# ahsouri/OI-SAT-GMI

Hardware: AMD Instinct MI355X
Metric: analysed grid-cells/s (dense Gaussian-B OI: B build + Kalman-gain solve + increment) and Kalman-gain solve TFLOP/s vs MI355X fp32 MFMA roofline (higher is better)
Workload: dtype f32; 1 GPU; config3_720x1440_1e5obs; species=NO2, obs_per_month=99898, refine=2, parallelism=one month per GPU; RCCL broadcast of the grid, gather of the fields to rank 0

## Files before the change

### include/oisat.h

```cpp
#ifndef OISAT_H
#define OISAT_H

#include <stddef.h>
#include <stdint.h>

#ifdef __cplusplus
extern "C" {
#endif

#define OISAT_F32 0
#define OISAT_F64 1

#define OISAT_OK 0
#define OISAT_EINVAL (-1)
#define OISAT_EHIP (-2)
#define OISAT_ENOMEM (-3)
#define OISAT_ENOTPD (-4)
#define OISAT_ENODEV (-5)

#define OISAT_MAX_SCALES 128

typedef struct oisat_ctx oisat_ctx;

int oisat_init(int device_id, oisat_ctx** out);
void oisat_shutdown(oisat_ctx* h);
const char* oisat_last_error(void);
const char* oisat_version(void);
int oisat_device_info(oisat_ctx* h, char* name_out, int name_cap, int* cu_count, int64_t* hbm_bytes);

int oisat_set_stream(oisat_ctx* h, void* hip_stream);
int oisat_stream_create(oisat_ctx* h);
int oisat_stream_create_masked(oisat_ctx* h, int reserve_per_xcd);
int oisat_bind_thread(oisat_ctx* h);
int oisat_wait_for(oisat_ctx* waiter, oisat_ctx* signaler);
int oisat_sync(oisat_ctx* h);
int oisat_query(oisat_ctx* h, int* busy);
int oisat_dmalloc(oisat_ctx* h, size_t bytes, void** dev_out);
int oisat_dfree(oisat_ctx* h, void* dev);
int oisat_h2d(oisat_ctx* h, void* dev_dst, const void* host_src, size_t bytes);
int oisat_d2h(oisat_ctx* h, void* host_dst, const void* dev_src, size_t bytes);
int oisat_memset(oisat_ctx* h, void* dev, int byte_value, size_t bytes);

int oisat_prof_enable(oisat_ctx* h, int on);
int oisat_prof_reset(oisat_ctx* h);
int oisat_prof_collect(oisat_ctx* h, int cap, char (*names)[64], double* total_ms, int64_t* launches);

int oisat_oi_curve(oisat_ctx* h, int dtype, const void* Sa, const void* So, int64_t n,
                   const double* scales, int nscales, double* mean_out, int64_t* count_out);

int oisat_oi_apply(oisat_ctx* h, int dtype, const void* Xa, void* Y_inout, const void* Sa,
                   const void* So, int64_t n, double scale, void* Xb, void* AK, void* inc, void* err);

int oisat_oi_fused(oisat_ctx* h, int dtype, const void* Xa, void* Y_inout, const void* Sa,
                   const void* So, int64_t n, const double* scales, int nscales, int forced_index,
                   void* Xb, void* AK, void* inc, void* err, int32_t* index_dev, double* curve_dev);

int oisat_nanmean_stack(oisat_ctx* h, int dtype, const void* stack, int k, int64_t n, int inf_to_nan, void* out);

int oisat_error_average(oisat_ctx* h, int dtype, const void* stack, int k, int64_t n, int square_input, void* out);

int oisat_month_accumulate(oisat_ctx* h, int acc_dtype, const void* vcd, const void* uncertainty, const void* ctm_vcd,
                           const void* new_amf, const void* old_amf, int f32_mask, int64_t n, const int32_t* kept, void* acc);
int oisat_month_finish(oisat_ctx* h, int acc_dtype, const void* acc, int64_t n, void* out);
int oisat_all_nan(oisat_ctx* h, int dtype, const void* x, int64_t n, int32_t* kept);
int oisat_widen(oisat_ctx* h, const float* x, int64_t n, double* out);

int oisat_affine(oisat_ctx* h, int dtype, const void* x, int64_t n, double offset, double slope, void* out);

int oisat_oi_variances(oisat_ctx* h, int dtype, const void* Xa, const void* sat_err, int64_t n,
                       double error_ctm, void* Sa_out, void* So_out);

int oisat_scaling_factor(oisat_ctx* h, int dtype, const void* posterior, const void* prior, int64_t n, void* out);

int oisat_partial_column(oisat_ctx* h, int dtype, const void* deltap, const void* profile, int64_t n, void* out);

int oisat_amf_recal(oisat_ctx* h, const double* sat_pmid, const double* sat_sw, int nzs, int ctm_dtype,
                    const void* ctm_pmid, const void* ctm_partial, int nzc, const double* tropopause, const double* vcd,
                    const double* amf, int64_t n, double* new_amf, double* vcd_out, double* ctm_vcd);

int oisat_column_sum(oisat_ctx* h, int dtype, const void* ctm_pmid, const void* ctm_partial, int nzc,
                     const double* tropopause, const double* vcd, int64_t n, void* ctm_vcd);

int oisat_ak_conv_mopitt(oisat_ctx* h, int ctm_dtype, const void* ctm_pmid, const void* ctm_profile,
                         const void* ctm_air_partial, int nzc, const double* sat_pmid,
                         const double* averaging_kernels, const double* apriori_profile, int nzs,
                         const double* aprior_column, const double* apriori_surface, const double* vcd,
                         int64_t n, double* model_vcd, double* model_xcol);
int oisat_ak_conv_gosat(oisat_ctx* h, int ctm_dtype, const void* ctm_pmid, const void* ctm_profile, int nzc,
                        const double* sat_pmid, const double* averaging_kernels,
                        const double* apriori_profile, const double* pressure_weight, int nzs,
                        const double* x_col, int64_t n, double* model_xcol);

int oisat_water_column(oisat_ctx* h, int dtype, const void* deltap, const void* profile, int64_t n, void* out);
int oisat_pwv_sum(oisat_ctx* h, int dtype, const void* partial, int nz, const double* vcd, int64_t n, void* out);

int oisat_boxfilter_symm(oisat_ctx* h, int dtype, const void* Z, int64_t Ny, int64_t Nx, int ky, int kx,
                         int variance, void* out);

int oisat_nn_query(oisat_ctx* h, const double* plon, const double* plat, int64_t P,
                   const double* tlon, const double* tlat, int64_t T, double max_dist,
                   int32_t* idx_out, double* dist_out );

int oisat_nn_query_ties(oisat_ctx* h, const double* plon, const double* plat, int64_t P,
                        const double* tlon, const double* tlat, int64_t T, double max_dist,
                        int32_t* idx_out, double* dist_out ,
                        int32_t* tie_list, int64_t* n_ties);

int oisat_gather_mask(oisat_ctx* h, int dtype, const void* values, int64_t P, int nfields,
                      const int32_t* idx, int64_t T, void* out);

int oisat_linear_interp(oisat_ctx* h, int dtype, const double* tlon, const double* tlat, int64_t T,
                        const int32_t* nn_idx, const int32_t* vertex_to_simplex, const int32_t* simplices,
                        const int32_t* neighbors, const double* transform, int64_t nsimplex,
                        const void* values, int64_t P, int nfields, void* out, const double* bounds_host);

int oisat_tri_transform(oisat_ctx* h, const double* points, int64_t P, const int32_t* simplices, int64_t nsimplex,
                        double* transform_out, int32_t* suspects, int64_t* n_suspect);

int oisat_linear_locate(oisat_ctx* h, const double* tlon, const double* tlat, int64_t T, const int32_t* nn_idx,
                        const int32_t* vertex_to_simplex, const int32_t* simplices, const int32_t* neighbors,
                        const double* transform, int64_t nsimplex, int64_t P, const double* bounds_host,
                        int32_t* amb_list, int64_t* n_amb);

int oisat_linear_interp_forced(oisat_ctx* h, int dtype, const double* tlon, const double* tlat, int64_t T,
                               const int32_t* nn_idx, const int32_t* vertex_to_simplex, const int32_t* simplices,
                               const int32_t* neighbors, const double* transform, int64_t nsimplex,
                               const void* values, int64_t P, int nfields, void* out, const double* bounds_host,
                               const int32_t* forced);

int oisat_rbf_interp(oisat_ctx* h, int dtype, const double* plon, const double* plat, int64_t P,
                     const double* tlon, const double* tlat, int64_t T, const int32_t* nn_idx, double cell,
                     int neighbors, const void* values, int nfields, void* out, int64_t* n_singular);

int oisat_rbf_interp_ties(oisat_ctx* h, int dtype, const double* plon, const double* plat, int64_t P,
                          const double* tlon, const double* tlat, int64_t T, const int32_t* nn_idx, double cell,
                          int neighbors, const void* values, int nfields, void* out, int64_t* n_singular,
                          int32_t* tie_list, int64_t* n_ties);

int oisat_rbf_interp_forced(oisat_ctx* h, int dtype, const double* plon, const double* plat, int64_t P,
                            const double* tlon, const double* tlat, int64_t T, const int32_t* targets,
                            const int32_t* ids, int64_t n, int neighbors, const void* values, int nfields, void* out,
                            int64_t* n_singular);

int oisat_rbf_check_masked(oisat_ctx* h, const double* plon, const double* plat, int64_t P, const double* tlon,
                           const double* tlat, int64_t T, const int32_t* nn_idx, double cell, int neighbors,
                           int64_t* n_singular);

int oisat_boxfilter_pick(oisat_ctx* h, int dtype, const void* Z, int64_t Ny, int64_t Nx, int nfields,
                         int ky, int kx, int variance, const int32_t* idx, int64_t T, void* out);

int oisat_flag_mask(oisat_ctx* h, int dtype, const void* x, const void* flag, int64_t n, double thresh,
                    int square, void* out);

int oisat_sqrt(oisat_ctx* h, int dtype, const void* x, int64_t n, void* out);


int oisat_cov_build(oisat_ctx* h, const double* oxyz, const double* osig, const double* ovar, int64_t m,
                    double g, float* S, int64_t ld);

int oisat_innovation(oisat_ctx* h, int dtype, const void* xb, const int64_t* cell, const double* y,
                     int64_t m, double* d_out);

int oisat_gemm_nt(oisat_ctx* h, float* C, int64_t ldc, const float* A, int64_t lda, const float* B, int64_t ldb,
                  int64_t M, int64_t N, int64_t K, int mode, int lower);

int oisat_potrf(oisat_ctx* h, float* S, int64_t m, int64_t ld, int* info_host);

int oisat_envelope(const double* lat_sorted, int64_t m, double g, int32_t* env_out);
int oisat_factor_envelope(const double* lat_sorted, int64_t m, double g, int32_t* env_out);
int oisat_factor_far(const double* lat_sorted, int64_t m, double g, const int32_t* first, int32_t* far_out);
int oisat_factor_mid(const double* lat_sorted, int64_t m, double g, const int32_t* first, const int32_t* far, int32_t* mid_out);

#define OISAT_CORR_GAUSSIAN 0
#define OISAT_CORR_GASPARI_COHN 1
int oisat_set_correlation(oisat_ctx* h, int kind);
int oisat_corr_eval(int kind, double g, const double* d2, int64_t n, double* out);
int oisat_corr_cut_chord(int kind, double g, double bits, double* chord_out);
int oisat_envelope_corr(int kind, const double* lat_sorted, int64_t m, double g, int32_t* env_out);
int oisat_factor_envelope_corr(int kind, const double* lat_sorted, int64_t m, double g, int32_t* env_out);
int oisat_factor_far_corr(int kind, const double* lat_sorted, int64_t m, double g, const int32_t* first, int32_t* far_out);
int oisat_set_factor_far(oisat_ctx* h, const int32_t* far, int64_t nb);
int oisat_factor_mid_corr(int kind, const double* lat_sorted, int64_t m, double g, const int32_t* first, const int32_t* far,
                          int32_t* mid_out);
int oisat_set_factor_mid(oisat_ctx* h, const int32_t* mid, int64_t nb);
int oisat_cov_build_env(oisat_ctx* h, const double* oxyz, const double* osig, const double* ovar, int64_t m,
                        double g, float* S, int64_t ld, const int32_t* env_dev);
int oisat_potrf_env(oisat_ctx* h, float* S, int64_t m, int64_t ld, const int32_t* first, const int32_t* env_dev,
                    int* info_host);

#define OISAT_SCHEDULE_OTHER 0
#define OISAT_SCHEDULE_ENV_DAG 1
#define OISAT_SCHEDULE_ENV_DAG_FWD 2
int oisat_cov_build_env_zeroed(oisat_ctx* h, const double* oxyz, const double* osig, const double* ovar, int64_t m,
                               double g, float* S, int64_t ld, const int32_t* first, const int32_t* env_dev,
                               const int32_t* zero_first, const int32_t* zero_first_dev, int* enveloped_out);
int oisat_cov_build_cover(const int32_t* first, const int32_t* zero_first, int64_t nb, int32_t* from_out,
                          int64_t* width_out, int64_t* zero_tiles_out);
int oisat_potrf_env_fwd(oisat_ctx* h, float* S, int64_t m, int64_t ld, const int32_t* first, const int32_t* env_dev,
                        const double* d, int* info_host, int* schedule_out);

int oisat_trsv_plan(int64_t nb, int band, int cu_count, int32_t* two_tiles_out, int32_t* grid_out);

int oisat_potrs(oisat_ctx* h, const float* L, int64_t m, int64_t ld, double* z_inout);

int oisat_cov_residual(oisat_ctx* h, const double* oxyz, const double* osig, const double* ovar, int64_t m,
                       double g, const double* d, const double* z, double* r_out, const double* olat_sorted);

int oisat_gain_solve(oisat_ctx* h, const float* L, const double* oxyz, const double* osig, const double* ovar,
                     int64_t m, int64_t ld, double g, const double* d, int refine, double* z_out,
                     double* resid_host, const double* olat_sorted );

int oisat_apply_increment(oisat_ctx* h, int dtype, const double* gxyz, const double* gsig, int64_t n,
                          const double* oxyz, const double* osig, const double* z, int64_t m, double g,
                          const void* xb, void* xa, void* inc, const double* glat, const double* olat_sorted);

int oisat_apply_increment_grid(oisat_ctx* h, int dtype, const double* gxyz, const double* gsig, int64_t ny, int64_t nx,
                               const double* oxyz, const double* osig, const double* z, int64_t m, double g,
                               const void* xb, void* xa, void* inc, const double* glat, const double* olat_sorted);

int oisat_set_obs_blocks(oisat_ctx* h, const int32_t* perm, int64_t m);

int oisat_trsm_rows(oisat_ctx* h, const float* L, int64_t m, int64_t ld, float* X, int64_t nrows, int64_t ldx);

int oisat_posterior_error(oisat_ctx* h, const float* L, int64_t m, int64_t ld, const double* gxyz,
                          const double* gsig, int64_t n, int64_t i0, int64_t i1, const double* oxyz,
                          const double* osig, double g, int64_t chunk_rows, float* err);

int oisat_gain_diag(oisat_ctx* h, const float* L, int64_t m, int64_t ld, const double* ovar, int64_t chunk_rows,
                    double* ak_out);

int oisat_dag_task_order(int nsys, const int32_t* block_rows, int wave, int32_t* tasks_out, int64_t capacity,
                         int64_t* ntasks_out, int32_t* reserve_out, int32_t* max_wave_chains_out);
int oisat_dag_task_order_env(int nb, const int32_t* first, const int32_t* far, int32_t* tasks_out, int64_t capacity,
                             int64_t* ntasks_out);

int oisat_set_task_graph(oisat_ctx* h, int mode);

int oisat_set_share(oisat_ctx* h, int wave_prio, int gemm_wg_per_cu);

int oisat_set_refine_tol(oisat_ctx* h, double tol);

int oisat_batch_create(oisat_ctx* h, int nmat, float* const* S, const int64_t* m, const int64_t* ld, float* const* tinv,
                       int* batch_id_out);
int oisat_batch_potrf(oisat_ctx* h, int batch_id, int* info_host);

int oisat_batch_set_solve(oisat_ctx* h, int batch_id, int nmat, const double* const* oxyz, const double* const* osig,
                          const double* const* ovar, const double* const* d, const double* const* olat, double* const* z,
                          double* const* work, void* const* state, const double* const* gxyz, const double* const* gsig,
                          const double* const* glat, const int64_t* n, const void* const* xb, void* const* xa,
                          void* const* inc);
int oisat_batch_set_grid(oisat_ctx* h, int batch_id, int nmat, const int64_t* nx, const int32_t* const* perm);
int oisat_batch_solve(oisat_ctx* h, int batch_id, int dtype, double g, int refine);
int oisat_batch_analyse(oisat_ctx* h, int batch_id, int dtype, double g, int refine, int* info_host);
int oisat_batch_is_task_graph(oisat_ctx* h, int batch_id, int* yes_out);
int oisat_batch_destroy(oisat_ctx* h, int batch_id);
int oisat_factor_adopt(oisat_ctx* h, const float* L, int64_t m, int64_t ld, float* tinv);

int oisat_comm_unique_id(char* id_out, int cap );
int oisat_comm_init(oisat_ctx* h, int rank, int nranks, const char* unique_id);
int oisat_comm_bcast(oisat_ctx* h, void* dev_buf, size_t bytes, int root);
int oisat_comm_gather(oisat_ctx* h, const void* send_dev, size_t bytes, void* recv_dev, int root);
int oisat_comm_destroy(oisat_ctx* h);

enum { OISAT_STATUS_NOTPD_COL = 0, OISAT_STATUS_NOTPD_BLOCKS = 1, OISAT_STATUS_TRSV_TIMEOUTS = 2, OISAT_STATUS_UNCONVERGED = 3,
       OISAT_STATUS_UNCONVERGED_MEMBER = 4, OISAT_STATUS_DAG_TIMEOUTS = 5, OISAT_STATUS_WORDS = 6 };
int oisat_solve_status_ex(oisat_ctx* h, int32_t* out, int nwords, int clear);
int oisat_solve_status(oisat_ctx* h, int* first_notpd_col, int* n_notpd_blocks, int* trsv_timeouts, int clear);

int oisat_dense_reserve(oisat_ctx* h, int64_t max_obs, int64_t diag_chunk_rows);

#ifdef __cplusplus
}
#endif
#endif
```

### oi-sat-gmi_amd/csrc/dense_chol.hip

```cpp
#include "oisat_common.h"

#include <algorithm>

namespace {

typedef float f32x16 __attribute__((ext_vector_type(16)));

constexpr int NB = 128;
constexpr int BK = 32;
constexpr int LDSW = 36;

struct BatchArgs {
    const BatchMat* mats;
    int kind;
    int b0, mid, b1;
    const int* cum = nullptr;
    int cnt = 0, total = 0;
    int prio = 0;
};

__device__ __forceinline__ void group_prio(int p) {
    if (p == 3) __builtin_amdgcn_s_setprio(3);
    else if (p == 2) __builtin_amdgcn_s_setprio(2);
    else if (p == 1) __builtin_amdgcn_s_setprio(1);
// ... 1591 lines not shown
        OISAT_LAUNCH(h, "potrf_diag", potrf_diag3_kernel, dim3(1), dim3(D3_THREADS), 0, S, ld, k0, tinv, info_dev, (int)b0,
                     (const BatchMat*)nullptr, 0);
        const int64_t rows = (mpb - b0 - 1) * NB;
        if (rows > 0) {
            float* P = S + (k0 + NB) * ld + k0;
            const int rc = launch_gemm(h, "trsm_gemm", P, ld, P, ld, tinv + b0 * NB * NB, NB, rows, NB, NB, 1, 0);
            if (rc) return rc;
        }
        return OISAT_OK;
    }
    if (b1 - b0 == 2 && kSinglePairs) {
        OISAT_LAUNCH(h, "potrf_diag", potrf_diag3_kernel, dim3(1), dim3(D3_THREADS), 0, S, ld, b0 * NB, tinv, info_dev, (int)b0,
                     (const BatchMat*)nullptr, 0);
        OISAT_LAUNCH(h, "pair_mid", pair_mid_kernel<false>, dim3(1), dim3(256), 0, S, ld, (int)mpb, (const float*)tinv, (int)b0,
                     (const BatchMat*)nullptr, 0);
        OISAT_LAUNCH(h, "potrf_diag", potrf_diag3_kernel, dim3(1), dim3(D3_THREADS), 0, S, ld, (b0 + 1) * NB, tinv, info_dev,
                     (int)(b0 + 1), (const BatchMat*)nullptr, 0);
        const int64_t rows = mpb - b0 - 2;
        if (rows > 0) {
            OISAT_LAUNCH(h, "pair_panel", pair_panel_kernel<false>, dim3((unsigned)(rows * 2)), dim3(256), 0, S, ld, (int)mpb,
                         (const float*)tinv, (int)b0, (const BatchMat*)nullptr, 0);
        }
        return OISAT_OK;
    }
    const int64_t mid = split_mid(b0, b1, kSinglePairs);
    int rc = potrf_rec(h, S, ld, mpb, b0, mid, tinv, info_dev);
    if (rc) return rc;
    {
        float* Cc = S + mid * NB * ld + mid * NB;
        const float* Aa = S + mid * NB * ld + b0 * NB;
        rc = launch_gemm(h, "syrk_gemm", Cc, ld, Aa, ld, Aa, ld, (mpb - mid) * NB, (b1 - mid) * NB, (int)((mid - b0) * NB), 0, 1);
        if (rc) return rc;
    }
    return potrf_rec(h, S, ld, mpb, mid, b1, tinv, info_dev);
}

int potrf_lookahead(oisat_ctx* h, float* S, int64_t ld, int64_t nb, float* tinv, int* info_dev, int64_t pw) {
    const int64_t np = cdiv(nb, pw);
    if (!h->aux_stream) {
        int prio_low = 0, prio_high = 0;
        HIP_TRY(hipDeviceGetStreamPriorityRange(&prio_low, &prio_high));
        const int prio = prio_low;
        HIP_TRY(hipStreamCreateWithPriority(&h->aux_stream, hipStreamNonBlocking, prio));
    }
    while ((int64_t)h->sync_events.size() < 2 * np + 2) {
        hipEvent_t ev;
        HIP_TRY(hipEventCreateWithFlags(&ev, hipEventDisableTiming));
        h->sync_events.push_back(ev);
    }
    hipStream_t s1 = h->stream, s2 = h->aux_stream;
    auto E1 = [&](int64_t q) { return h->sync_events[2 * q]; };
    auto E2 = [&](int64_t q) { return h->sync_events[2 * q + 1]; };
    hipEvent_t ev_edge = h->sync_events[2 * np];
    HIP_TRY(hipEventRecord(ev_edge, s1));
    HIP_TRY(hipStreamWaitEvent(s2, ev_edge, 0));
    auto c0 = [&](int64_t q) { return (q * pw < nb ? q * pw : nb); };
    int rc = OISAT_OK;
    auto update = [&](int64_t cb0, int64_t cb1, int64_t kb0, int64_t kb1) {
        if (cb1 <= cb0) return (int)OISAT_OK;
        float* Cc = S + cb0 * NB * ld + cb0 * NB;
        const float* Aa = S + cb0 * NB * ld + kb0 * NB;
        return launch_gemm(h, "syrk_gemm", Cc, ld, Aa, ld, Aa, ld, (nb - cb0) * NB, (cb1 - cb0) * NB, (int)((kb1 - kb0) * NB), 0, 1);
    };
    for (int64_t q = 0; q < np && rc == OISAT_OK; ++q) {
        if (q >= 2) HIP_TRY(hipStreamWaitEvent(s1, E2(q - 2), 0));
        rc = potrf_rec(h, S, ld, nb, c0(q), c0(q + 1), tinv, info_dev);
        if (rc || q + 1 == np) break;
        HIP_TRY(hipEventRecord(E1(q), s1));
        if (q >= 1) HIP_TRY(hipStreamWaitEvent(s1, E2(q - 1), 0));
        rc = update(c0(q + 1), c0(q + 2), c0(q), c0(q + 1));
        if (rc) break;
        if (q + 2 < np) {
            HIP_TRY(hipStreamWaitEvent(s2, E1(q), 0));
            h->stream = s2;
            rc = update(c0(q + 2), c0(q + 3), c0(q), c0(q + 1));
            if (rc == OISAT_OK && hipEventRecord(E2(q), s2) != hipSuccess) rc = OISAT_EHIP;
            if (rc == OISAT_OK) rc = update(c0(q + 3), nb, c0(q), c0(q + 1));
            h->stream = s1;
        }
    }
    h->stream = s1;
    if (rc) return rc;
    HIP_TRY(hipEventRecord(ev_edge, s2));
    HIP_TRY(hipStreamWaitEvent(s1, ev_edge, 0));
    return OISAT_OK;
}

constexpr size_t kCtlBytes = ((sizeof(TrsvCtl) + 15) / 16) * 16;
int status_ws(oisat_ctx* h, int** info_dev, char** trsv_base) {
    const bool fresh4 = h->ws[4] == nullptr, fresh7 = h->ws[7] == nullptr;
    int* info = (int*)oisat_ws(h, 4, 256);
    char* base = (char*)oisat_ws(h, 7, 16 + 2 * kCtlBytes);
    if (!info || !base) return OISAT_ENOMEM;
    if (fresh4) HIP_TRY(hipMemsetAsync(info, 0, 256, h->stream));
    if (fresh7) HIP_TRY(hipMemsetAsync(base, 0, 16 + 2 * kCtlBytes, h->stream));
    if (info_dev) *info_dev = info;
    if (trsv_base) *trsv_base = base;
    return OISAT_OK;
}

__global__ __launch_bounds__(256) void solve_prep_batched_kernel(const SolveMember* __restrict__ mem) {
    const SolveMember* mb = mem + blockIdx.y;
    const int64_t m = mb->m, mp = (int64_t)mb->mpb * NB;
    const int64_t stride = (int64_t)gridDim.x * blockDim.x;
    const int64_t g0 = (int64_t)blockIdx.x * blockDim.x + threadIdx.x;
    const double* src = mb->d;
    double* rhs = mb->rhs;
    unsigned long long* fwd = reinterpret_cast<unsigned long long*>(mb->fwd);
    for (int64_t i = g0; i < mp; i += stride) {
        rhs[i] = i < m ? src[i] : 0.0;
        fwd[i] = kTrsvEmpty;
    }
    if (g0 == 0) {
        mb->st->conv = 0;
        mb->st->computed = 0;
    }
}

__global__ __launch_bounds__(1024) void resid_check_batched_kernel(const SolveMember* __restrict__ mem, int k, double tol2, int final,
                                                                    int* __restrict__ info) {
    __shared__ double sr[1024], sd[1024];
    const SolveMember* mb = mem + blockIdx.x;
    SolveState* st = mb->st;
    if (st->conv != 0) return;
    const double* r = mb->rhs;
    const double* d = mb->d;
    const int64_t m = mb->m;
    double a = 0.0, b = 0.0;
    for (int64_t i = threadIdx.x; i < m; i += 1024) {
        a += r[i] * r[i];
        if (k == 0) b += d[i] * d[i];
    }
    sr[threadIdx.x] = a;
    sd[threadIdx.x] = b;
    __syncthreads();
    for (int q = 512; q > 0; q >>= 1) {
        if ((int)threadIdx.x < q) {
            sr[threadIdx.x] += sr[threadIdx.x + q];
            sd[threadIdx.x] += sd[threadIdx.x + q];
        }
        __syncthreads();
    }
    if (threadIdx.x == 0) {
        if (k == 0) st->dd = sd[0];
        st->norm[k] = sr[0];
        st->computed = k + 1;
        if (sr[0] <= tol2 * st->dd) st->conv = 1;
        else if (final && tol2 > 0.0) {
            atomicAdd(&info[kInfoUnconverged], 1);
            atomicCAS(&info[kInfoUnconvergedMember], 0, mb->which + 1);
        }
    }
}

extern "C" int oisat_trsv_plan(int64_t nb, int band, int cu_count, int32_t* two_tiles_out, int32_t* grid_out) {
    ARG_CHECK(nb >= 1 && nb <= INT32_MAX && band >= 0 && cu_count >= 0);
    const bool two = nb <= cu_count || (band > 0 && band <= cu_count / 2);
    if (two_tiles_out) *two_tiles_out = two ? 1 : 0;
    if (grid_out) *grid_out = (int32_t)(two ? std::min<int64_t>(nb, cu_count) : nb);
    return OISAT_OK;
}

static int trsv_launch_shape(const oisat_ctx* h, const ChFactor& f, int nb, int* two_out, int* grid_out) {
    int32_t two = 0, grid = 0;
    if (int rc = oisat_trsv_plan(nb, f.env != nullptr ? f.band : 0, h->cu_count, &two, &grid)) return rc;
    const char* e = getenv("OISAT_TRSV_TWO_TILES");
    if (e && *e) {
        ARG_CHECK((e[0] == '0' || e[0] == '1') && e[1] == '\0');
        two = e[0] == '1';
        grid = two && h->cu_count > 0 ? std::min(nb, h->cu_count) : nb;
    }
    e = getenv("OISAT_TRSV_MAX_WGS");
    if (e && *e) {
        char* end = nullptr;
        const long cap = strtol(e, &end, 10);
        ARG_CHECK(end != e && *end == '\0' && cap >= 1);
        if (cap < grid) grid = (int32_t)cap;
    }
    *two_out = two;
    *grid_out = grid;
    return OISAT_OK;
}

int trsv_solve(oisat_ctx* h, const ChFactor& f, double* rhs_pad, double* fwd, const SolveState* st, double* zout, int accumulate,
               bool fwd_done = false) {
    const int nb = (int)(f.mp / NB);
    const size_t ctl_bytes = kCtlBytes;
    char* base = nullptr;
    if (int rc = status_ws(h, nullptr, &base)) return rc;
    unsigned* err_total = (unsigned*)base;
    char* ctl = base + 16;
    int two = 0, grid = 0;
    if (int rc = trsv_launch_shape(h, f, nb, &two, &grid)) return rc;
    const size_t shm = sizeof(float) * NB * TLD * (two ? 2 : 1);
    if (!fwd_done) {
        OISAT_LAUNCH(h, "trsv_fwd", (trsv_pipe_kernel<0>), dim3(grid), dim3(256), shm, f.S, f.ld, (const float*)f.tinv, nb, rhs_pad, fwd,
                     (TrsvCtl*)ctl, err_total, two, st, (double*)nullptr, (int64_t)0, 0, f.env);
    }
    OISAT_LAUNCH(h, "trsv_bwd", (trsv_pipe_kernel<1>), dim3(grid), dim3(256), shm, f.S, f.ld, (const float*)f.tinv, nb, fwd, rhs_pad,
                 (TrsvCtl*)(ctl + ctl_bytes), err_total, two, st, zout, f.m, accumulate, f.env);
    return OISAT_OK;
}

SolveState* solve_state(oisat_ctx* h) {
    const bool fresh = h->ws[9] == nullptr;
    SolveState* st = (SolveState*)oisat_ws(h, 9, 256);
    if (st && fresh && hipMemsetAsync(st, 0, 256, h->stream) != hipSuccess) return nullptr;
    return st;
}

int trsm_rows_rec(oisat_ctx* h, const ChFactor& f, float* X, int64_t nrows, int64_t ldx, int64_t b0, int64_t b1) {
    if (b1 - b0 == 1) {
        float* Xb = X + b0 * NB;
        return launch_gemm(h, "trsm_rows_diag", Xb, ldx, Xb, ldx, f.tinv + b0 * NB * NB, NB, nrows, NB, NB, 1, 0);
    }
    const int64_t mid = b0 + (b1 - b0 + 1) / 2;
    int rc = trsm_rows_rec(h, f, X, nrows, ldx, b0, mid);
    if (rc) return rc;
    rc = launch_gemm(h, "trsm_rows_gemm", X + mid * NB, ldx, X + b0 * NB, ldx, f.S + mid * NB * f.ld + b0 * NB, f.ld, nrows,
                     (b1 - mid) * NB, (int)((mid - b0) * NB), 0, 0);
    if (rc) return rc;
    return trsm_rows_rec(h, f, X, nrows, ldx, mid, b1);
}

hipError_t dense_kernel_attributes() {
    static const hipError_t attr_rc = []() {
        hipError_t e = hipFuncSetAttribute((const void*)trsv_pipe_kernel<0>, hipFuncAttributeMaxDynamicSharedMemorySize,
                                    (int)(sizeof(float) * NB * TLD * 2));
        if (e == hipSuccess)
            e = hipFuncSetAttribute((const void*)trsv_pipe_kernel<1>, hipFuncAttributeMaxDynamicSharedMemorySize,
                                    (int)(sizeof(float) * NB * TLD * 2));
        if (e == hipSuccess)
            e = hipFuncSetAttribute((const void*)trsv_batched_kernel<0>, hipFuncAttributeMaxDynamicSharedMemorySize,
                                    (int)(sizeof(float) * NB * TLD));
        if (e == hipSuccess)
            e = hipFuncSetAttribute((const void*)trsv_batched_kernel<1>, hipFuncAttributeMaxDynamicSharedMemorySize,
                                    (int)(sizeof(float) * NB * TLD));
        return e;
    }();
    return attr_rc;
}

#include "dense_dag.inc"

static inline bool dag_wanted(const oisat_ctx* h, int64_t max_blocks, int nsys) {
    const int mode = h->dag_mode >= 0 ? h->dag_mode : (getenv("OISAT_DAG") ? atoi(getenv("OISAT_DAG")) : -1);
    if (mode == 0 || nsys > 1024) return false;
    return max_blocks >= (mode == 1 ? 2 : 3);
}

}

void oisat_dag_plan_release(void* plan) { dag_plan_free((DagPlan*)plan); }

extern "C" int oisat_dag_task_order(int nsys, const int32_t* block_rows, int wave, int32_t* tasks_out, int64_t capacity,
                                    int64_t* ntasks_out, int32_t* reserve_out, int32_t* max_wave_chains_out) {
    ARG_CHECK(nsys > 0 && block_rows && ntasks_out && (tasks_out || capacity == 0));
    std::vector<int> nb_of(block_rows, block_rows + nsys);
    for (int s = 0; s < nsys; ++s) ARG_CHECK(nb_of[s] >= 1 && (s == 0 || nb_of[s] <= nb_of[s - 1]));
    DagOrder order;
    dag_task_order(nb_of, wave, order);
    *ntasks_out = (int64_t)order.tasks.size();
    if (reserve_out) *reserve_out = order.reserve_chains;
    if (max_wave_chains_out) *max_wave_chains_out = order.max_wave_chains;
    if ((int64_t)order.tasks.size() > capacity) return capacity == 0 ? OISAT_OK : OISAT_EINVAL;
    memcpy(tasks_out, order.tasks.data(), sizeof(int4) * order.tasks.size());
    return OISAT_OK;
}

extern "C" int oisat_set_refine_tol(oisat_ctx* h, double tol) {
    ARG_CHECK(h != nullptr && tol >= 0.0 && tol < 1.0);
    h->refine_tol = tol;
    return OISAT_OK;
}

extern "C" int oisat_set_task_graph(oisat_ctx* h, int mode) {
    ARG_CHECK(h != nullptr && mode >= -1 && mode <= 1);
    h->dag_mode = mode;
    return OISAT_OK;
}

extern "C" int oisat_set_share(oisat_ctx* h, int wave_prio, int gemm_wg_per_cu) {
    ARG_CHECK(h != nullptr && wave_prio >= 0 && wave_prio <= 3 && gemm_wg_per_cu >= 0 && gemm_wg_per_cu <= 2);
    h->wave_prio = wave_prio;
    h->gemm_wg_per_cu = gemm_wg_per_cu;
    return OISAT_OK;
}

extern "C" int oisat_gemm_nt(oisat_ctx* h, float* C, int64_t ldc, const float* A, int64_t lda, const float* B, int64_t ldb,
                             int64_t M, int64_t N, int64_t K, int mode, int lower) {
    ARG_CHECK(h && C && A && B && M > 0 && N > 0 && K > 0);
    ARG_CHECK(M % NB == 0 && N % NB == 0 && K % BK == 0 && K < (int64_t)INT32_MAX);
    ARG_CHECK(ldc % 4 == 0 && lda % 4 == 0 && ldb % 4 == 0 && ldc >= N && lda >= K && ldb >= K);
    ARG_CHECK(((uintptr_t)C % 16) == 0 && ((uintptr_t)A % 16) == 0 && ((uintptr_t)B % 16) == 0);
    ARG_CHECK((mode == 0 || mode == 1) && (!lower || M >= N));
    return launch_gemm(h, "gemm_nt", C, ldc, A, lda, B, ldb, M, N, (int)K, mode, lower);
}

static bool fwd_in_launch_off() {
    const char* e = getenv("OISAT_FWD_IN_LAUNCH");
    return e != nullptr && atoi(e) == 0;
}

static int potrf_impl(oisat_ctx* h, float* S, int64_t m, int64_t ld, int* info_host, const int32_t* first, const int32_t* env_dev,
                      const double* fwd_d = nullptr, int* schedule_out = nullptr, const int32_t* far = nullptr, const int32_t* mid = nullptr) {
    ARG_CHECK(h && S && m > 0);
    h->factor.fwd_d = nullptr;
    if (schedule_out) *schedule_out = OISAT_SCHEDULE_OTHER;
    const int64_t mp = cdiv(m, NB) * NB;
    ARG_CHECK(ld >= mp && (ld % 4) == 0 && ((uintptr_t)S % 16) == 0);
    const int64_t mpb = mp / NB;
    float* tinv = (float*)oisat_ws(h, 3, sizeof(float) * mpb * NB * NB);
    int* info_dev = nullptr;
    if (!tinv) return OISAT_ENOMEM;
    if (int rc = status_ws(h, &info_dev, nullptr)) return rc;
    HIP_TRY(dense_kernel_attributes());
    HIP_TRY(hipMemsetAsync(info_dev, 0, sizeof(int), h->stream));
    if (mp > m) {
        OISAT_LAUNCH(h, "pad_identity", pad_identity_kernel, dim3(stream_grid((mp - m) * mp, 256)), dim3(256), 0, S, ld, m, mp);
    }
    bool lookahead = false;
    int64_t pw = 4;
    if (const char* env = getenv("OISAT_POTRF")) {
        if (strcmp(env, "recursive") == 0) lookahead = false;
        else if (strncmp(env, "lookahead", 9) == 0) {
            lookahead = mpb >= 2;
            if (env[9] == ':' && atoi(env + 10) > 0) pw = atoi(env + 10);
        }
    }
    int rc;
    if (!lookahead && !getenv("OISAT_POTRF") && dag_wanted(h, mpb, 1) && dag_fits(1, dag_slots(h)) && (!first || mpb <= kDagEnvMaxBlocks)) {
        const bool ride = fwd_d != nullptr && !fwd_in_launch_off();
        DagSingle* hit = nullptr;
        for (DagSingle& c : h->dag_cache)
            if (c.plan && c.S == S && c.tinv == tinv && c.ld == ld && c.mpb == mpb && c.enveloped == (first != nullptr) && c.fwd == ride) hit = &c;
        if (hit && first) {
            DagPlan& pl = *(DagPlan*)hit->plan;
            if (memcmp(pl.first.data(), first, sizeof(int) * (size_t)mpb) != 0 ||
                memcmp(pl.far.data(), far ? far : first, sizeof(int) * (size_t)mpb) != 0 ||
                memcmp(pl.mid.data(), mid ? mid : far ? far : first, sizeof(int) * (size_t)mpb) != 0)
                if (int rf = dag_plan_refill(pl, first, far, mid, h->stream)) return rf;
        }
        if (!hit) {
            DagSingle* slot = nullptr;
            for (DagSingle& c : h->dag_cache)
                if (!c.plan) { slot = &c; break; }
            if (!slot) {
                slot = &h->dag_cache[0];
                for (DagSingle& c : h->dag_cache)
                    if (c.stamp < slot->stamp) slot = &c;
                HIP_TRY(hipStreamSynchronize(h->stream));
                oisat_dag_plan_release(slot->plan);
                slot->plan = nullptr;
            }
            DagSolveShape shape;
            if (ride) {
                shape.refine = 0;
                shape.fwd_only = true;
            }
            slot->plan = dag_plan_create(std::vector<BatchMat>{BatchMat{S, tinv, ld, m, (int)mpb, 0}}, h->stream, shape, first, first ? far : nullptr,
                                         first ? mid : nullptr);
            if (!slot->plan) return OISAT_ENOMEM;
            slot->S = S; slot->tinv = tinv; slot->ld = ld; slot->mpb = mpb; slot->enveloped = first != nullptr; slot->fwd = ride;
            hit = slot;
        }
        hit->stamp = ++h->dag_clock;
        DagPlan& pl = *(DagPlan*)hit->plan;
        if (ride) {
            double* w = (double*)oisat_ws(h, 5, sizeof(double) * (2 + 8) * mp);
            SolveState* st = solve_state(h);
            char* base = nullptr;
            if (!w || !st) return OISAT_ENOMEM;
            if (int rs = status_ws(h, nullptr, &base)) return rs;
            OISAT_LAUNCH(h, "copy_pad", solve_prep_kernel, dim3(stream_grid(mp, 256)), dim3(256), 0, fwd_d, m, mp, w, w + mp, st);
            DagSolve sv{};
            sv.queue = pl.queue_dev;
            sv.qcap = (int)pl.qcap;
            sv.qcap0 = (int)pl.qcap0;
            sv.nsys = 1;
            sv.trsv_timeouts = (unsigned*)base;
            sv.fwd_rhs = w;
            sv.fwd_sol = w + mp;
            sv.env = first ? env_dev : nullptr;
            rc = dag_launch(h, pl, info_dev, (unsigned*)(info_dev + kInfoDagTimeouts), &sv);
            if (rc == OISAT_OK) h->factor.fwd_d = fwd_d;
        } else {
            rc = dag_launch(h, pl, info_dev, (unsigned*)(info_dev + kInfoDagTimeouts));
        }
        if (schedule_out) *schedule_out = !first ? OISAT_SCHEDULE_OTHER : ride ? OISAT_SCHEDULE_ENV_DAG_FWD : OISAT_SCHEDULE_ENV_DAG;
    } else {
        rc = lookahead ? potrf_lookahead(h, S, ld, mpb, tinv, info_dev, pw) : potrf_rec(h, S, ld, mpb, 0, mpb, tinv, info_dev);
    }
    if (rc) {
        h->factor.fwd_d = nullptr;
        return rc;
    }
    h->factor.S = S;
    h->factor.m = m;
    h->factor.mp = mp;
    h->factor.ld = ld;
    h->factor.tinv = tinv;
    h->factor.env = env_dev;
    h->factor.band = 0;
    if (first && env_dev)
        for (int64_t b = 0; b < mpb; ++b) h->factor.band = std::max(h->factor.band, (int)(b - first[b]) + 1);
    if (info_host) {
        int* pin = (int*)oisat_pinned(h, 64);
        if (!pin) return OISAT_ENOMEM;
        HIP_TRY(hipMemcpyAsync(pin, info_dev, 8 * sizeof(int), hipMemcpyDeviceToHost, h->stream));
        HIP_TRY(hipStreamSynchronize(h->stream));
        *info_host = *pin;
        if (pin[kInfoDagTimeouts] != 0) {
            HIP_TRY(hipMemsetAsync(info_dev + kInfoDagTimeouts, 0, sizeof(int), h->stream));
            oisat_set_error("potrf: the task-graph factorization timed out (a workgroup gave up waiting): the factor is incomplete");
            return OISAT_EHIP;
        }
        if (*pin != 0) {
            HIP_TRY(hipMemsetAsync(info_dev + 1, 0, 2 * sizeof(int), h->stream));
            oisat_set_error("potrf: matrix not positive definite at column %d", *pin);
            return OISAT_ENOTPD;
        }
    }
    return OISAT_OK;
}

extern "C" int oisat_potrf(oisat_ctx* h, float* S, int64_t m, int64_t ld, int* info_host) {
    return potrf_impl(h, S, m, ld, info_host, nullptr, nullptr);
}

bool oisat_envelope_off() {
    const char* e = getenv("OISAT_ENVELOPE");
    return e != nullptr && atoi(e) == 0;
}

static bool envelope_table_ok(const int32_t* first, int64_t nb) {
    for (int64_t i = 0; i < nb; ++i)
        if (first[i] < 0 || first[i] > (i > 0 ? i - 1 : 0) || (i > 0 && first[i] < first[i - 1])) return false;
    return true;
}

constexpr double kFactorCutBits = 28.0;
constexpr double kFactorMinKstepsPerRow = 1500.0;

static void envelope_table(int kind, const double* lat_sorted, int64_t m, double g, double bits, int32_t* env_out) {
    const int64_t nb = cdiv(m, NB);
    const double angle = g > 0.0 ? lat_window_deg(kind, g, bits) : 1e9;
    int64_t k = 0;
    for (int64_t i = 0; i < nb; ++i) {
        const double lo = lat_sorted[i * NB] - angle;
        while (k < i && lat_sorted[std::min((k + 1) * NB, m) - 1] < lo) ++k;
        env_out[i] = (int32_t)std::min<int64_t>(k, i > 0 ? i - 1 : 0);
    }
    for (int64_t b = 0, j = 0; b < nb; ++b) {
        while (j + 1 < nb && env_out[j + 1] <= b) ++j;
        env_out[nb + b] = (int32_t)j;
    }
}

static int64_t envelope_ksteps(const int32_t* first, int64_t nb) {
    int64_t k = 0;
    for (int64_t i = 0; i < nb; ++i)
        for (int64_t j = first[i]; j <= i; ++j) k += j - std::max(first[i], first[j]);
    return k;
}

static bool corr_kind_ok(int kind) { return kind == OISAT_CORR_GAUSSIAN || kind == OISAT_CORR_GASPARI_COHN; }

extern "C" int oisat_envelope_corr(int kind, const double* lat_sorted, int64_t m, double g, int32_t* env_out) {
    ARG_CHECK(corr_kind_ok(kind) && lat_sorted && env_out && m > 0 && g >= 0.0);
    for (int64_t i = 1; i < m; ++i) ARG_CHECK(lat_sorted[i] >= lat_sorted[i - 1]);
    envelope_table(kind, lat_sorted, m, g, kCutBits, env_out);
    return OISAT_OK;
}

extern "C" int oisat_envelope(const double* lat_sorted, int64_t m, double g, int32_t* env_out) {
    return oisat_envelope_corr(OISAT_CORR_GAUSSIAN, lat_sorted, m, g, env_out);
}

extern "C" int oisat_factor_envelope_corr(int kind, const double* lat_sorted, int64_t m, double g, int32_t* env_out) {
    ARG_CHECK(corr_kind_ok(kind) && lat_sorted && env_out && m > 0 && g >= 0.0);
    for (int64_t i = 1; i < m; ++i) ARG_CHECK(lat_sorted[i] >= lat_sorted[i - 1]);
    double bits = kFactorCutBits;
    bool forced = false;
    const char* e = getenv("OISAT_FACTOR_CUT_BITS");
    if (e && *e) {
        char* end = nullptr;
        bits = strtod(e, &end);
        ARG_CHECK(end != e && *end == '\0' && bits >= 1.0 && bits <= kCutBits);
        forced = true;
    }
    const int64_t nb = cdiv(m, NB);
    if (kind == OISAT_CORR_GASPARI_COHN && !forced) bits = kCutBits;
    envelope_table(kind, lat_sorted, m, g, bits, env_out);
    if (kind == OISAT_CORR_GAUSSIAN && !forced && (double)envelope_ksteps(env_out, nb) <= kFactorMinKstepsPerRow * (double)nb)
        envelope_table(kind, lat_sorted, m, g, kCutBits, env_out);
    return OISAT_OK;
}

extern "C" int oisat_factor_envelope(const double* lat_sorted, int64_t m, double g, int32_t* env_out) {
    return oisat_factor_envelope_corr(OISAT_CORR_GAUSSIAN, lat_sorted, m, g, env_out);
}

constexpr double kFactorFarBits = 18.0;

extern "C" int oisat_factor_far_corr(int kind, const double* lat_sorted, int64_t m, double g, const int32_t* first, int32_t* far_out) {
    ARG_CHECK(corr_kind_ok(kind) && lat_sorted && first && far_out && m > 0 && g >= 0.0);
    for (int64_t i = 1; i < m; ++i) ARG_CHECK(lat_sorted[i] >= lat_sorted[i - 1]);
    const int64_t nb = cdiv(m, NB);
    ARG_CHECK(envelope_table_ok(first, nb));
    double bits = kFactorFarBits;
    bool on = false;
    const char* e = getenv("OISAT_FACTOR_FAR_BITS");
    if (e && *e) {
        char* end = nullptr;
        bits = strtod(e, &end);
        ARG_CHECK(end != e && *end == '\0' && bits >= 0.0 && bits <= kCutBits);
        on = bits >= 1.0;
        ARG_CHECK(on || bits == 0.0);
    } else {
        const char* c = getenv("OISAT_FACTOR_CUT_BITS");
        if (!(c && *c) && kind == OISAT_CORR_GAUSSIAN) {
            std::vector<int32_t> narrow(2 * (size_t)nb);
            envelope_table(kind, lat_sorted, m, g, kFactorCutBits, narrow.data());
            on = (double)envelope_ksteps(narrow.data(), nb) > kFactorMinKstepsPerRow * (double)nb;
        }
    }
    if (on && !oisat_envelope_off()) {
        std::vector<int32_t> t(2 * (size_t)nb);
        envelope_table(kind, lat_sorted, m, g, bits, t.data());
        for (int64_t i = 0; i < nb; ++i) far_out[i] = std::min<int32_t>(std::max(t[i], first[i]), (int32_t)i);
    } else {
        for (int64_t i = 0; i < nb; ++i) far_out[i] = first[i];
    }
    return OISAT_OK;
}

extern "C" int oisat_factor_far(const double* lat_sorted, int64_t m, double g, const int32_t* first, int32_t* far_out) {
    return oisat_factor_far_corr(OISAT_CORR_GAUSSIAN, lat_sorted, m, g, first, far_out);
}

extern "C" int oisat_set_factor_far(oisat_ctx* h, const int32_t* far, int64_t nb) {
    ARG_CHECK(h != nullptr && nb >= 0 && (far != nullptr || nb == 0));
    h->factor_far.assign(far, far + nb);
    return OISAT_OK;
}

static bool far_table_ok(const std::vector<int32_t>& far, const int32_t* first, int64_t nb) {
    if (far.empty()) return true;
    if ((int64_t)far.size() != nb) return false;
    for (int64_t i = 0; i < nb; ++i)
        if (far[i] < first[i] || far[i] > i) return false;
    return true;
}

constexpr double kFactorMidBits = 8.0;

extern "C" int oisat_factor_mid_corr(int kind, const double* lat_sorted, int64_t m, double g, const int32_t* first, const int32_t* far,
                                     int32_t* mid_out) {
    ARG_CHECK(corr_kind_ok(kind) && lat_sorted && first && far && mid_out && m > 0 && g >= 0.0);
    for (int64_t i = 1; i < m; ++i) ARG_CHECK(lat_sorted[i] >= lat_sorted[i - 1]);
    const int64_t nb = cdiv(m, NB);
    ARG_CHECK(envelope_table_ok(first, nb));
    for (int64_t i = 0; i < nb; ++i) ARG_CHECK(far[i] >= first[i] && far[i] <= i);
    double bits = kFactorMidBits;
    bool on = false;
    const char* e = getenv("OISAT_FACTOR_MID_BITS");
    if (e && *e) {
        char* end = nullptr;
        bits = strtod(e, &end);
        ARG_CHECK(end != e && *end == '\0' && bits >= 0.0 && bits <= kCutBits);
        on = bits >= 1.0;
        ARG_CHECK(on || bits == 0.0);
    } else {
        const char* c = getenv("OISAT_FACTOR_CUT_BITS");
        if (!(c && *c) && kind == OISAT_CORR_GAUSSIAN) {
            std::vector<int32_t> narrow(2 * (size_t)nb);
            envelope_table(kind, lat_sorted, m, g, kFactorCutBits, narrow.data());
            on = (double)envelope_ksteps(narrow.data(), nb) > kFactorMinKstepsPerRow * (double)nb;
        }
    }
    if (on && !oisat_envelope_off()) {
        std::vector<int32_t> t(2 * (size_t)nb);
        envelope_table(kind, lat_sorted, m, g, bits, t.data());
        for (int64_t i = 0; i < nb; ++i) mid_out[i] = std::min<int32_t>(std::max(t[i], far[i]), (int32_t)i);
    } else {
        for (int64_t i = 0; i < nb; ++i) mid_out[i] = far[i];
    }
    return OISAT_OK;
}

extern "C" int oisat_factor_mid(const double* lat_sorted, int64_t m, double g, const int32_t* first, const int32_t* far, int32_t* mid_out) {
    return oisat_factor_mid_corr(OISAT_CORR_GAUSSIAN, lat_sorted, m, g, first, far, mid_out);
}

extern "C" int oisat_set_factor_mid(oisat_ctx* h, const int32_t* mid, int64_t nb) {
    ARG_CHECK(h != nullptr && nb >= 0 && (mid != nullptr || nb == 0));
    h->factor_mid.assign(mid, mid + nb);
    return OISAT_OK;
}

static bool mid_table_ok(const std::vector<int32_t>& mid, const std::vector<int32_t>& far, const int32_t* first, int64_t nb) {
    if (mid.empty()) return true;
    if ((int64_t)mid.size() != nb || !far_table_ok(far, first, nb)) return false;
    for (int64_t i = 0; i < nb; ++i)
        if (mid[i] < (far.empty() ? first[i] : far[i]) || mid[i] > i) return false;
    return true;
}

extern "C" int oisat_dag_task_order_env(int nb, const int32_t* first, const int32_t* far, int32_t* tasks_out, int64_t capacity,
                                        int64_t* ntasks_out) {
    ARG_CHECK(nb >= 1 && nb <= kDagEnvMaxBlocks && first && ntasks_out && (tasks_out || capacity == 0));
    ARG_CHECK(envelope_table_ok(first, nb));
    if (far)
        for (int i = 0; i < nb; ++i) ARG_CHECK(far[i] >= first[i] && far[i] <= i);
    DagOrder order;
    dag_task_order(std::vector<int>{nb}, 0, order, first, far);
    *ntasks_out = (int64_t)order.tasks.size();
    if ((int64_t)order.tasks.size() > capacity) return capacity == 0 ? OISAT_OK : OISAT_EINVAL;
    memcpy(tasks_out, order.tasks.data(), sizeof(int4) * order.tasks.size());
    return OISAT_OK;
}

extern "C" int oisat_potrf_env(oisat_ctx* h, float* S, int64_t m, int64_t ld, const int32_t* first, const int32_t* env_dev,
                               int* info_host) {
    ARG_CHECK(h != nullptr);
    std::vector<int32_t> far, mid;
    far.swap(h->factor_far);
    mid.swap(h->factor_mid);
    ARG_CHECK(first && env_dev && m > 0);
    ARG_CHECK(envelope_table_ok(first, cdiv(m, NB)) && far_table_ok(far, first, cdiv(m, NB)) &&
              mid_table_ok(mid, far, first, cdiv(m, NB)));
    if (oisat_envelope_off()) return potrf_impl(h, S, m, ld, info_host, nullptr, nullptr);
    return potrf_impl(h, S, m, ld, info_host, first, env_dev, nullptr, nullptr, far.empty() ? nullptr : far.data(),
                      mid.empty() ? nullptr : mid.data());
}

extern "C" int oisat_potrf_env_fwd(oisat_ctx* h, float* S, int64_t m, int64_t ld, const int32_t* first, const int32_t* env_dev,
                                   const double* d, int* info_host, int* schedule_out) {
    ARG_CHECK(h != nullptr);
    std::vector<int32_t> far, mid;
    far.swap(h->factor_far);
    mid.swap(h->factor_mid);
    ARG_CHECK(first && env_dev && d && m > 0);
    ARG_CHECK(envelope_table_ok(first, cdiv(m, NB)) && far_table_ok(far, first, cdiv(m, NB)) &&
              mid_table_ok(mid, far, first, cdiv(m, NB)));
    if (oisat_envelope_off()) return potrf_impl(h, S, m, ld, info_host, nullptr, nullptr, d, schedule_out);
    return potrf_impl(h, S, m, ld, info_host, first, env_dev, d, schedule_out, far.empty() ? nullptr : far.data(),
                      mid.empty() ? nullptr : mid.data());
}

extern "C" int oisat_potrs(oisat_ctx* h, const float* L, int64_t m, int64_t ld, double* z_inout) {
    ARG_CHECK(h && L && z_inout && m > 0);
    ARG_CHECK(h->factor.S == L && h->factor.m == m && h->factor.ld == ld);
    h->factor.fwd_d = nullptr;
    double* w = (double*)oisat_ws(h, 5, sizeof(double) * (2 + 8) * h->factor.mp);
    if (!w) return OISAT_ENOMEM;
    double* rhs = w;
    double* fwd = w + h->factor.mp;
    OISAT_LAUNCH(h, "copy_pad", solve_prep_kernel, dim3(stream_grid(h->factor.mp, 256)), dim3(256), 0, (const double*)z_inout, m,
                 h->factor.mp, rhs, fwd, (SolveState*)nullptr);
    return trsv_solve(h, h->factor, rhs, fwd, nullptr, z_inout, 0);
}

int oisat_cov_residual_if(oisat_ctx* h, const double* oxyz, const double* osig, const double* ovar, int64_t m, double g,
                          const double* d, const double* z, double* r_out, const double* olat_sorted, const int* converged_dev,
                          const int* perm);
const int* oisat_take_obs_perm(oisat_ctx* h, int64_t m);

extern "C" int oisat_gain_solve(oisat_ctx* h, const float* L, const double* oxyz, const double* osig, const double* ovar, int64_t m,
                                int64_t ld, double g, const double* d, int refine, double* z_out, double* resid_host,
                                const double* olat_sorted) {
    ARG_CHECK(h != nullptr);
    const int* perm = oisat_take_obs_perm(h, m);
    const bool fwd_done = h->factor.fwd_d != nullptr && h->factor.fwd_d == d;
    h->factor.fwd_d = nullptr;
    ARG_CHECK(L && oxyz && osig && ovar && d && z_out && m > 0 && refine >= 0 && refine <= 8);
    ARG_CHECK(h->factor.S == L && h->factor.m == m && h->factor.ld == ld);
    const double tol = h->refine_tol;
    const int64_t mp = h->factor.mp;
    double* w = (double*)oisat_ws(h, 5, sizeof(double) * (2 + 8) * mp);
    SolveState* st = solve_state(h);
    if (!w || !st) return OISAT_ENOMEM;
    double* rhs = w;
    double* fwd = w + mp;
    if (!fwd_done) {
        OISAT_LAUNCH(h, "copy_pad", solve_prep_kernel, dim3(stream_grid(mp, 256)), dim3(256), 0, d, m, mp, rhs, fwd, st);
    }
    int rc = trsv_solve(h, h->factor, rhs, fwd, nullptr, z_out, 0, fwd_done);
    if (rc) return rc;
    int* info_dev = nullptr;
    if (int rs = status_ws(h, &info_dev, nullptr)) return rs;
    for (int it = 0; it <= refine && (refine > 0 || resid_host); ++it) {
        rc = oisat_cov_residual_if(h, oxyz, osig, ovar, m, g, d, z_out, rhs, olat_sorted, &st->conv, perm);
        if (rc) return rc;
        OISAT_LAUNCH(h, "resid_check", resid_check_kernel, dim3(1), dim3(1024), 0, (const double*)rhs, d, m, it, tol * tol, st,
                     it == refine && refine > 0 ? 1 : 0, info_dev);
        if (it == refine) break;
        rc = trsv_solve(h, h->factor, rhs, fwd, st, z_out, 1);
        if (rc) return rc;
    }
    if (resid_host) {
        char* pin = (char*)oisat_pinned(h, 512);
        if (!pin) return OISAT_ENOMEM;
        HIP_TRY(hipMemcpyAsync(pin, st, sizeof(SolveState), hipMemcpyDeviceToHost, h->stream));
        HIP_TRY(hipMemcpyAsync(pin + 256, h->ws[7], sizeof(unsigned), hipMemcpyDeviceToHost, h->stream));
        HIP_TRY(hipStreamSynchronize(h->stream));
        const SolveState* hs = (const SolveState*)pin;
        const double dn = hs->dd > 0.0 ? sqrt(hs->dd) : 1.0;
        for (int it = 0; it <= refine; ++it) {
            const int k = it < hs->computed ? it : hs->computed - 1;
            resid_host[it] = k >= 0 ? sqrt(hs->norm[k]) / dn : 0.0;
        }
        const unsigned gave_up = *(const unsigned*)(pin + 256);
        if (gave_up != 0) {
            HIP_TRY(hipMemsetAsync(h->ws[7], 0, 16, h->stream));
            oisat_set_error("triangular solve: %u workgroup(s) gave up waiting for a predecessor (bounded spin)", gave_up);
            return OISAT_EHIP;
        }
    }
    return OISAT_OK;
}

extern "C" int oisat_trsm_rows(oisat_ctx* h, const float* L, int64_t m, int64_t ld, float* X, int64_t nrows, int64_t ldx) {
    ARG_CHECK(h && L && X && m > 0 && nrows > 0);
    ARG_CHECK(h->factor.S == L && h->factor.m == m && h->factor.ld == ld);
    ARG_CHECK(nrows % NB == 0 && ldx >= h->factor.mp && ldx % 4 == 0 && ((uintptr_t)X % 16) == 0);
    return trsm_rows_rec(h, h->factor, X, nrows, ldx, 0, h->factor.mp / NB);
}

extern "C" int oisat_posterior_error(oisat_ctx* h, const float* L, int64_t m, int64_t ld, const double* gxyz, const double* gsig,
                                     int64_t n, int64_t i0, int64_t i1, const double* oxyz, const double* osig, double g,
                                     int64_t chunk_rows, float* err) {
    ARG_CHECK(h && L && gxyz && gsig && oxyz && osig && err && m > 0 && n > 0 && 0 <= i0 && i0 < i1 && i1 <= n);
    ARG_CHECK(h->factor.S == L && h->factor.m == m && h->factor.ld == ld);
    const int64_t mp = h->factor.mp;
    if (chunk_rows <= 0) chunk_rows = 4096;
    chunk_rows = cdiv(chunk_rows, NB) * NB;
    float* X = (float*)oisat_ws(h, 6, sizeof(float) * chunk_rows * mp + sizeof(double) * chunk_rows);
    if (!X) return OISAT_ENOMEM;
    double* ss = (double*)(X + chunk_rows * mp);
    const float g2 = h->corr == OISAT_CORR_GASPARI_COHN ? (float)(kGcZ2PerG * g) : (float)(g * 1.4426950408889634);
    for (int64_t c0 = i0; c0 < i1; c0 += chunk_rows) {
        const int64_t live = (i1 - c0 < chunk_rows) ? i1 - c0 : chunk_rows;
        const int64_t nrows = cdiv(live, NB) * NB;
        if (h->corr == OISAT_CORR_GASPARI_COHN) {
            OISAT_LAUNCH(h, "cross_cov_rows", cross_cov_rows_kernel<OISAT_CORR_GASPARI_COHN>, dim3((unsigned)(mp / 64), (unsigned)(nrows / 64)),
                         dim3(256), 0, gxyz, gsig, n, c0, live, oxyz, osig, m, mp, g2, X, mp);
        } else {
            OISAT_LAUNCH(h, "cross_cov_rows", cross_cov_rows_kernel<OISAT_CORR_GAUSSIAN>, dim3((unsigned)(mp / 64), (unsigned)(nrows / 64)),
                         dim3(256), 0, gxyz, gsig, n, c0, live, oxyz, osig, m, mp, g2, X, mp);
        }
        if (nrows > live) HIP_TRY(hipMemsetAsync(X + live * mp, 0, sizeof(float) * (nrows - live) * mp, h->stream));
        const int rc = trsm_rows_rec(h, h->factor, X, nrows, mp, 0, mp / NB);
        if (rc) return rc;
        OISAT_LAUNCH(h, "row_sumsq", row_sumsq_kernel, dim3((unsigned)cdiv(nrows * 64, 256)), dim3(256), 0, (const float*)X, nrows, mp,
                     mp, ss);
        OISAT_LAUNCH(h, "post_err", post_err_kernel, dim3((unsigned)cdiv(live, 256)), dim3(256), 0, gsig, c0, live, n,
                     (const double*)ss, err + (c0 - i0));
    }
    return OISAT_OK;
}

extern "C" int oisat_gain_diag(oisat_ctx* h, const float* L, int64_t m, int64_t ld, const double* ovar, int64_t chunk_rows,
                               double* ak_out) {
    ARG_CHECK(h && L && ovar && ak_out && m > 0);
    ARG_CHECK(h->factor.S == L && h->factor.m == m && h->factor.ld == ld);
    const int64_t mp = h->factor.mp;
    if (chunk_rows <= 0) chunk_rows = 4096;
    chunk_rows = cdiv(chunk_rows, NB) * NB;
    float* X = (float*)oisat_ws(h, 6, sizeof(float) * chunk_rows * mp + sizeof(double) * chunk_rows);
    if (!X) return OISAT_ENOMEM;
    double* ss = (double*)(X + chunk_rows * mp);
    for (int64_t a0 = 0; a0 < m; a0 += chunk_rows) {
        const int64_t live = (m - a0 < chunk_rows) ? m - a0 : chunk_rows;
        const int64_t nrows = cdiv(live, NB) * NB;
        OISAT_LAUNCH(h, "identity_rows", identity_rows_kernel, dim3(stream_grid(nrows * mp, 256)), dim3(256), 0, X, mp, a0, nrows, mp);
        const int rc = trsm_rows_rec(h, h->factor, X, nrows, mp, 0, mp / NB);
        if (rc) return rc;
        OISAT_LAUNCH(h, "row_sumsq", row_sumsq_kernel, dim3((unsigned)cdiv(nrows * 64, 256)), dim3(256), 0, (const float*)X, nrows, mp,
                     mp, ss);
        OISAT_LAUNCH(h, "gain_diag", gain_diag_kernel, dim3((unsigned)cdiv(live, 256)), dim3(256), 0, ovar, a0, live, m,
                     (const double*)ss, ak_out);
    }
    return OISAT_OK;
}

extern "C" int oisat_solve_status_ex(oisat_ctx* h, int32_t* out, int nwords, int clear) {
    ARG_CHECK(h != nullptr && (out != nullptr || nwords == 0) && nwords >= 0 && nwords <= OISAT_STATUS_WORDS);
    int* info = nullptr;
    char* base = nullptr;
    if (int rc = status_ws(h, &info, &base)) return rc;
    int* pin = (int*)oisat_pinned(h, 256);
    if (!pin) return OISAT_ENOMEM;
    HIP_TRY(hipMemcpyAsync(pin, info, 8 * sizeof(int), hipMemcpyDeviceToHost, h->stream));
    HIP_TRY(hipMemcpyAsync(pin + 8, base, sizeof(int), hipMemcpyDeviceToHost, h->stream));
    if (clear) {
        HIP_TRY(hipMemsetAsync(info + 1, 0, 2 * sizeof(int), h->stream));
        HIP_TRY(hipMemsetAsync(info + kInfoUnconverged, 0, 3 * sizeof(int), h->stream));
        HIP_TRY(hipMemsetAsync(base, 0, 16, h->stream));
    }
    HIP_TRY(hipStreamSynchronize(h->stream));
    const int32_t words[OISAT_STATUS_WORDS] = {pin[1], pin[2], pin[8], pin[kInfoUnconverged], pin[kInfoUnconvergedMember] - 1,
                                               pin[kInfoDagTimeouts]};
    for (int i = 0; i < nwords; ++i) out[i] = words[i];
    return OISAT_OK;
}

extern "C" int oisat_solve_status(oisat_ctx* h, int* first_notpd_col, int* n_notpd_blocks, int* trsv_timeouts, int clear) {
    int32_t w[OISAT_STATUS_WORDS];
    if (int rc = oisat_solve_status_ex(h, w, OISAT_STATUS_WORDS, clear)) return rc;
    if (first_notpd_col) *first_notpd_col = w[OISAT_STATUS_NOTPD_COL];
    if (n_notpd_blocks) *n_notpd_blocks = w[OISAT_STATUS_NOTPD_BLOCKS];
    if (trsv_timeouts) *trsv_timeouts = w[OISAT_STATUS_TRSV_TIMEOUTS] + w[OISAT_STATUS_DAG_TIMEOUTS] + w[OISAT_STATUS_UNCONVERGED];
    return OISAT_OK;
}

extern "C" int oisat_dense_reserve(oisat_ctx* h, int64_t max_obs, int64_t diag_chunk_rows) {
    ARG_CHECK(h != nullptr && max_obs > 0 && diag_chunk_rows >= 0);
    const int64_t mp = cdiv(max_obs, NB) * NB;
    if (!oisat_ws(h, 3, sizeof(float) * mp * NB)) return OISAT_ENOMEM;
    if (int rc = status_ws(h, nullptr, nullptr)) return rc;
    if (!oisat_ws(h, 5, sizeof(double) * (2 + 8) * mp)) return OISAT_ENOMEM;
    if (!solve_state(h)) return OISAT_ENOMEM;
    size_t s6 = sizeof(double) * (max_obs + 16);
    if (diag_chunk_rows > 0) {
        const int64_t ch = cdiv(diag_chunk_rows, NB) * NB;
        const size_t x = sizeof(float) * ch * mp + sizeof(double) * ch;
        if (x > s6) s6 = x;
    }
    if (!oisat_ws(h, 6, s6)) return OISAT_ENOMEM;
    if (!oisat_pinned(h, 4096)) return OISAT_ENOMEM;
    return OISAT_OK;
}

extern "C" int oisat_batch_create(oisat_ctx* h, int nmat, float* const* S, const int64_t* m, const int64_t* ld, float* const* tinv,
                                  int* batch_id_out) {
    ARG_CHECK(h && S && m && ld && tinv && batch_id_out && nmat > 0 && nmat <= 65535);
    ChBatch* bt = new ChBatch();
    bt->order.resize(nmat);
    for (int i = 0; i < nmat; ++i) bt->order[i] = i;
    for (int i = 0; i < nmat; ++i) {
        const int64_t mp = cdiv(m[i], NB) * NB;
        if (!(S[i] && tinv[i] && m[i] > 0 && ld[i] >= mp && (ld[i] % 4) == 0 && ((uintptr_t)S[i] % 16) == 0 && ((uintptr_t)tinv[i] % 16) == 0 &&
              mp / NB < (int64_t)INT32_MAX)) {
            delete bt;
            oisat_set_error("oisat_batch_create: matrix %d: bad pointer, size or leading dimension", i);
            return OISAT_EINVAL;
        }
    }
    std::stable_sort(bt->order.begin(), bt->order.end(), [&](int a, int b) { return cdiv(m[a], NB) > cdiv(m[b], NB); });
    bt->table.resize(nmat);
    for (int i = 0; i < nmat; ++i) {
        const int k = bt->order[i];
        bt->table[i] = BatchMat{S[k], tinv[k], ld[k], m[k], (int)cdiv(m[k], NB), 0};
    }
    bt->max_mpb = bt->table[0].mpb;
    bt->pairs = kLeafPairsMin > 0 && nmat >= kLeafPairsMin;
    if (hipMalloc(&bt->table_dev, sizeof(BatchMat) * nmat) != hipSuccess) {
        delete bt;
        oisat_set_error("oisat_batch_create: hipMalloc of the table failed");
        return OISAT_ENOMEM;
    }
    if (hipMemcpy(bt->table_dev, bt->table.data(), sizeof(BatchMat) * nmat, hipMemcpyHostToDevice) != hipSuccess) {
        (void)hipFree(bt->table_dev);
        delete bt;
        oisat_set_error("oisat_batch_create: upload of the table failed");
        return OISAT_EHIP;
    }
    {
        std::vector<int> host;
        build_cum_tables(bt, host);
        if (hipMalloc(&bt->cum_dev, sizeof(int) * host.size()) != hipSuccess ||
            hipMemcpy(bt->cum_dev, host.data(), sizeof(int) * host.size(), hipMemcpyHostToDevice) != hipSuccess) {
            if (bt->cum_dev) (void)hipFree(bt->cum_dev);
            (void)hipFree(bt->table_dev);
            delete bt;
            oisat_set_error("oisat_batch_create: tile-enumeration tables failed");
            return OISAT_ENOMEM;
        }
    }
    bool want_dag = dag_wanted(h, bt->max_mpb, nmat);
    if (want_dag) {
        std::vector<int> nb_of(nmat);
        for (int i = 0; i < nmat; ++i) nb_of[i] = bt->table[i].mpb;
        DagOrder probe;
        dag_task_order(nb_of, 0, probe);
        want_dag = dag_fits(probe.max_wave_chains, dag_slots(h));
    }
    if (want_dag) {
        bt->dag = dag_plan_create(bt->table, h->stream);
        if (bt->dag && hipStreamSynchronize(h->stream) != hipSuccess) {
            oisat_dag_plan_release(bt->dag);
            bt->dag = nullptr;
        }
        if (!bt->dag) {
            (void)hipFree(bt->cum_dev);
            (void)hipFree(bt->table_dev);
            delete bt;
            return OISAT_ENOMEM;
        }
    }
    int id = -1;
    for (size_t i = 0; i < h->batches.size(); ++i)
        if (!h->batches[i]) { id = (int)i; break; }
    if (id < 0) { h->batches.push_back(nullptr); id = (int)h->batches.size() - 1; }
    h->batches[id] = bt;
    *batch_id_out = id;
    return OISAT_OK;
}
// ... 271 lines not shown
```

### oi-sat-gmi_amd/csrc/dense_dag.inc

```
constexpr int DAG_CHAIN = 0, DAG_TILE = 1, DAG_SUB = 2, DAG_PRE = 3;
constexpr int DAG_FWD = 5, DAG_BWD = 6, DAG_RES = 7, DAG_INC = 8;
constexpr int DAG_STATE_HDR = 64;
constexpr int DAG_ST_FWD = 2;
constexpr int DAG_ST_BWD = 11;
constexpr int DAG_ST_RES = 20;
constexpr int DAG_ST_INC = 29;
constexpr int DAG_INC_DECIDED = 1 << 20;
constexpr int DAG_MAX_REFINE = 8;
constexpr unsigned kDagSpinMax = 1u << 24;
constexpr int DAG_CU_KEYS = 16 * 256;

struct DagSys {
    float* S;
    float* tinv;
    int64_t ld;
    int* state;
    int nb;
    int which;
    const int* mid;
};

struct DagCtl {
    int ticket, error, gone, pad;
    int sys_done, pad2[3];
    struct { int head, tail, avail, pad; } q[2];
    int cu_arrivals[DAG_CU_KEYS];
    int cu_role[DAG_CU_KEYS];
};

struct DagLane {
    int lane, wid, wr, wc, rl, lc, frow, fh, sw, arow, brow;
    int flags;
    unsigned spin;
};

__device__ __forceinline__ bool dag_wait_ge(const int* p, int v, DagCtl* ctl, unsigned spin_max) {
    unsigned spins = 0;
    while (__hip_atomic_load(p, __ATOMIC_RELAXED, __HIP_MEMORY_SCOPE_AGENT) < v) {
        __builtin_amdgcn_s_sleep(2);
        if ((++spins & 255u) == 0u &&
            (spins > spin_max || __hip_atomic_load(&ctl->error, __ATOMIC_RELAXED, __HIP_MEMORY_SCOPE_AGENT) != 0)) {
            __hip_atomic_store(&ctl->error, 1, __ATOMIC_RELAXED, __HIP_MEMORY_SCOPE_AGENT);
            return false;
        }
    }
    return true;
}

__device__ __forceinline__ void dag_drop_l1() { asm volatile("buffer_inv sc1" ::: "memory"); }

__device__ __forceinline__ bool dag_join(bool ok_thread0, int* s_flag) {
    if (threadIdx.x == 0) {
        *s_flag = ok_thread0 ? 1 : 0;
        asm volatile("buffer_inv sc1\n\ts_waitcnt vmcnt(0)" ::: "memory");
    }
    __syncthreads();
    return *s_flag != 0;
}

__device__ __forceinline__ void dag_publish(int* p, int v) {
    asm volatile("s_waitcnt vmcnt(0)" ::: "memory");
    __syncthreads();
    if (threadIdx.x == 0) __hip_atomic_store(p, v, __ATOMIC_RELAXED, __HIP_MEMORY_SCOPE_AGENT);
}

#define DAG_MFMA4(A0, A1, B0, B1, c)                                                            \
    acc00 = __builtin_amdgcn_mfma_f32_32x32x2f32(A0.c, B0.c, acc00, 0, 0, 0);                   \
    acc01 = __builtin_amdgcn_mfma_f32_32x32x2f32(A0.c, B1.c, acc01, 0, 0, 0);                   \
    acc10 = __builtin_amdgcn_mfma_f32_32x32x2f32(A1.c, B0.c, acc10, 0, 0, 0);                   \
    acc11 = __builtin_amdgcn_mfma_f32_32x32x2f32(A1.c, B1.c, acc11, 0, 0, 0);
#define DAG_MFMA16(A0, A1, B0, B1)                                                              \
    DAG_MFMA4(A0, A1, B0, B1, x) DAG_MFMA4(A0, A1, B0, B1, y) DAG_MFMA4(A0, A1, B0, B1, z) DAG_MFMA4(A0, A1, B0, B1, w)

__device__ __forceinline__ void dag_seg(float* __restrict__ lds, const DagLane& L, const float* Ad, int64_t lda, const float* Bd, int64_t ldb,
                                        int nkt, f32x16& acc00, f32x16& acc01, f32x16& acc10, f32x16& acc11) {
    typedef __attribute__((address_space(1))) const void* gptr_t;
    typedef __attribute__((address_space(3))) void* lptr_t;
    constexpr int IMG = NB * BK;
#define DAG_DMA(buf, k0)                                                                                           \
    do {                                                                                                           \
        _Pragma("unroll") for (int i = 0; i < 4; ++i) {                                                            \
            __builtin_amdgcn_global_load_lds((gptr_t)(Ad + (int64_t)(8 * i) * lda + (k0)),                         \
                                             (lptr_t)(lds + ((buf) * 2 + 0) * IMG + (L.wid * 32 + 8 * i) * BK), 16, 0, 0); \
            __builtin_amdgcn_global_load_lds((gptr_t)(Bd + (int64_t)(8 * i) * ldb + (k0)),                         \
                                             (lptr_t)(lds + ((buf) * 2 + 1) * IMG + (L.wid * 32 + 8 * i) * BK), 16, 0, 0); \
        }                                                                                                          \
    } while (0)
#define DAG_FRAG(A0, A1, B0, B1, buf, s)                                                                               \
    do {                                                                                                           \
        A0 = *reinterpret_cast<const float4*>(lds + ((buf) * 2 + 0) * IMG + L.arow + 4 * ((2 * (s) + L.fh) ^ L.sw));            \
        A1 = *reinterpret_cast<const float4*>(lds + ((buf) * 2 + 0) * IMG + L.arow + 32 * BK + 4 * ((2 * (s) + L.fh) ^ L.sw));  \
        B0 = *reinterpret_cast<const float4*>(lds + ((buf) * 2 + 1) * IMG + L.brow + 4 * ((2 * (s) + L.fh) ^ L.sw));            \
        B1 = *reinterpret_cast<const float4*>(lds + ((buf) * 2 + 1) * IMG + L.brow + 32 * BK + 4 * ((2 * (s) + L.fh) ^ L.sw));  \
    } while (0)
    float4 fa0, fa1, fb0, fb1, ga0, ga1, gb0, gb1;
    DAG_DMA(0, 0);
    asm volatile("s_waitcnt vmcnt(0)" ::: "memory");
    __syncthreads();
    DAG_FRAG(fa0, fa1, fb0, fb1, 0, 0);
    for (int kt = 0; kt < nkt; ++kt) {
        const int cur = kt & 1;
        const bool more = kt + 1 < nkt;
        if (more) DAG_DMA(cur ^ 1, (kt + 1) * BK);
        DAG_FRAG(ga0, ga1, gb0, gb1, cur, 1);
        DAG_MFMA16(fa0, fa1, fb0, fb1)
        DAG_FRAG(fa0, fa1, fb0, fb1, cur, 2);
        DAG_MFMA16(ga0, ga1, gb0, gb1)
        DAG_FRAG(ga0, ga1, gb0, gb1, cur, 3);
        DAG_MFMA16(fa0, fa1, fb0, fb1)
        asm volatile("s_waitcnt vmcnt(0)" ::: "memory");
        __syncthreads();
        if (more) DAG_FRAG(fa0, fa1, fb0, fb1, cur ^ 1, 0);
        DAG_MFMA16(ga0, ga1, gb0, gb1)
    }
#undef DAG_DMA
#undef DAG_FRAG
}

typedef __attribute__((ext_vector_type(8))) __bf16 dag_bf16x8;
typedef __attribute__((ext_vector_type(4))) unsigned dag_u32x4;
__device__ __forceinline__ unsigned dag_pk_bf16(float lo, float hi) {
    unsigned r;
    asm("v_cvt_pk_bf16_f32 %0, %1, %2" : "=v"(r) : "v"(lo), "v"(hi));
    return r;
}
__device__ __forceinline__ dag_bf16x8 dag_pack8(const float4& a, const float4& b) {
    const dag_u32x4 u = {dag_pk_bf16(a.x, a.y), dag_pk_bf16(a.z, a.w), dag_pk_bf16(b.x, b.y), dag_pk_bf16(b.z, b.w)};
    return __builtin_bit_cast(dag_bf16x8, u);
}
__device__ __forceinline__ void dag_seg_bf16(float* __restrict__ lds, const DagLane& L, const float* Ad, int64_t lda, const float* Bd, int64_t ldb,
                                             int nkt, f32x16& acc00, f32x16& acc01, f32x16& acc10, f32x16& acc11) {
    typedef __attribute__((address_space(1))) const void* gptr_t;
    typedef __attribute__((address_space(3))) void* lptr_t;
    constexpr int IMG = NB * BK;
#define DAG_DMA(buf, k0)                                                                                           \
    do {                                                                                                           \
        _Pragma("unroll") for (int i = 0; i < 4; ++i) {                                                            \
            __builtin_amdgcn_global_load_lds((gptr_t)(Ad + (int64_t)(8 * i) * lda + (k0)),                         \
                                             (lptr_t)(lds + ((buf) * 2 + 0) * IMG + (L.wid * 32 + 8 * i) * BK), 16, 0, 0); \
            __builtin_amdgcn_global_load_lds((gptr_t)(Bd + (int64_t)(8 * i) * ldb + (k0)),                         \
                                             (lptr_t)(lds + ((buf) * 2 + 1) * IMG + (L.wid * 32 + 8 * i) * BK), 16, 0, 0); \
        }                                                                                                          \
    } while (0)
#define DAG_RD8(lo, hi, buf, op, row, c)                                                                                              \
    do {                                                                                                                              \
        lo = *reinterpret_cast<const float4*>(lds + ((buf) * 2 + (op)) * IMG + (row) + 4 * ((4 * (c) + 2 * L.fh) ^ L.sw));            \
        hi = *reinterpret_cast<const float4*>(lds + ((buf) * 2 + (op)) * IMG + (row) + 4 * ((4 * (c) + 2 * L.fh + 1) ^ L.sw));        \
    } while (0)
#define DAG_CHUNK(buf, c)                                                                                          \
    do {                                                                                                           \
        float4 a0l, a0h, a1l, a1h, b0l, b0h, b1l, b1h;                                                             \
        DAG_RD8(a0l, a0h, buf, 0, L.arow, c);                                                                      \
        DAG_RD8(a1l, a1h, buf, 0, L.arow + 32 * BK, c);                                                            \
        DAG_RD8(b0l, b0h, buf, 1, L.brow, c);                                                                      \
        DAG_RD8(b1l, b1h, buf, 1, L.brow + 32 * BK, c);                                                            \
        const dag_bf16x8 a0 = dag_pack8(a0l, a0h), a1 = dag_pack8(a1l, a1h);                                       \
        const dag_bf16x8 b0 = dag_pack8(b0l, b0h), b1 = dag_pack8(b1l, b1h);                                       \
        acc00 = __builtin_amdgcn_mfma_f32_32x32x16_bf16(a0, b0, acc00, 0, 0, 0);                                   \
        acc01 = __builtin_amdgcn_mfma_f32_32x32x16_bf16(a0, b1, acc01, 0, 0, 0);                                   \
        acc10 = __builtin_amdgcn_mfma_f32_32x32x16_bf16(a1, b0, acc10, 0, 0, 0);                                   \
        acc11 = __builtin_amdgcn_mfma_f32_32x32x16_bf16(a1, b1, acc11, 0, 0, 0);                                   \
    } while (0)
    DAG_DMA(0, 0);
    asm volatile("s_waitcnt vmcnt(0)" ::: "memory");
    __syncthreads();
    for (int kt = 0; kt < nkt; ++kt) {
        const int cur = kt & 1;
        if (kt + 1 < nkt) DAG_DMA(cur ^ 1, (kt + 1) * BK);
        DAG_CHUNK(cur, 0);
        DAG_CHUNK(cur, 1);
        asm volatile("s_waitcnt vmcnt(0)" ::: "memory");
        __syncthreads();
    }
#undef DAG_CHUNK
}

__device__ __forceinline__ unsigned dag_pk_bf16_lo(float x, float y, unsigned hi ) {
    return dag_pk_bf16(x - __builtin_bit_cast(float, hi << 16), y - __builtin_bit_cast(float, hi & 0xffff0000u));
}
__device__ __forceinline__ void dag_split8(const float4& a, const float4& b, dag_bf16x8& hi, dag_bf16x8& lo) {
    const dag_u32x4 h = {dag_pk_bf16(a.x, a.y), dag_pk_bf16(a.z, a.w), dag_pk_bf16(b.x, b.y), dag_pk_bf16(b.z, b.w)};
    const dag_u32x4 l = {dag_pk_bf16_lo(a.x, a.y, h.x), dag_pk_bf16_lo(a.z, a.w, h.y), dag_pk_bf16_lo(b.x, b.y, h.z), dag_pk_bf16_lo(b.z, b.w, h.w)};
    hi = __builtin_bit_cast(dag_bf16x8, h);
    lo = __builtin_bit_cast(dag_bf16x8, l);
}
__device__ __forceinline__ void dag_seg_bf16x2(float* __restrict__ lds, const DagLane& L, const float* Ad, int64_t lda, const float* Bd, int64_t ldb,
                                               int nkt, f32x16& acc00, f32x16& acc01, f32x16& acc10, f32x16& acc11) {
    typedef __attribute__((address_space(1))) const void* gptr_t;
    typedef __attribute__((address_space(3))) void* lptr_t;
    constexpr int IMG = NB * BK;
#define DAG_SPLIT(H, LO, buf, op, row, c)                                                                          \
    do {                                                                                                           \
        float4 rl, rh;                                                                                             \
        DAG_RD8(rl, rh, buf, op, row, c);                                                                          \
        dag_split8(rl, rh, H, LO);                                                                                 \
    } while (0)
#define DAG_CHUNK(buf, c)                                                                                          \
    do {                                                                                                           \
        dag_bf16x8 a0, a0l, a1, a1l, b0, b0l, b1, b1l;                                                             \
        DAG_SPLIT(a0, a0l, buf, 0, L.arow, c);                                                                     \
        DAG_SPLIT(a1, a1l, buf, 0, L.arow + 32 * BK, c);                                                           \
        DAG_SPLIT(b0, b0l, buf, 1, L.brow, c);                                                                     \
        DAG_SPLIT(b1, b1l, buf, 1, L.brow + 32 * BK, c);                                                           \
        acc00 = __builtin_amdgcn_mfma_f32_32x32x16_bf16(a0l, b0, acc00, 0, 0, 0);                                  \
        acc01 = __builtin_amdgcn_mfma_f32_32x32x16_bf16(a0l, b1, acc01, 0, 0, 0);                                  \
        acc10 = __builtin_amdgcn_mfma_f32_32x32x16_bf16(a1l, b0, acc10, 0, 0, 0);                                  \
        acc11 = __builtin_amdgcn_mfma_f32_32x32x16_bf16(a1l, b1, acc11, 0, 0, 0);                                  \
        acc00 = __builtin_amdgcn_mfma_f32_32x32x16_bf16(a0, b0l, acc00, 0, 0, 0);                                  \
        acc01 = __builtin_amdgcn_mfma_f32_32x32x16_bf16(a0, b1l, acc01, 0, 0, 0);                                  \
        acc10 = __builtin_amdgcn_mfma_f32_32x32x16_bf16(a1, b0l, acc10, 0, 0, 0);                                  \
        acc11 = __builtin_amdgcn_mfma_f32_32x32x16_bf16(a1, b1l, acc11, 0, 0, 0);                                  \
        acc00 = __builtin_amdgcn_mfma_f32_32x32x16_bf16(a0, b0, acc00, 0, 0, 0);                                   \
        acc01 = __builtin_amdgcn_mfma_f32_32x32x16_bf16(a0, b1, acc01, 0, 0, 0);                                   \
        acc10 = __builtin_amdgcn_mfma_f32_32x32x16_bf16(a1, b0, acc10, 0, 0, 0);                                   \
        acc11 = __builtin_amdgcn_mfma_f32_32x32x16_bf16(a1, b1, acc11, 0, 0, 0);                                   \
    } while (0)
    DAG_DMA(0, 0);
    asm volatile("s_waitcnt vmcnt(0)" ::: "memory");
    __syncthreads();
    for (int kt = 0; kt < nkt; ++kt) {
        const int cur = kt & 1;
        if (kt + 1 < nkt) DAG_DMA(cur ^ 1, (kt + 1) * BK);
        DAG_CHUNK(cur, 0);
        DAG_CHUNK(cur, 1);
        asm volatile("s_waitcnt vmcnt(0)" ::: "memory");
        __syncthreads();
    }
#undef DAG_DMA
#undef DAG_RD8
#undef DAG_SPLIT
#undef DAG_CHUNK
}

__device__ __forceinline__ void dag_acc_to_image(float* __restrict__ lds, const DagLane& L, const f32x16& acc00, const f32x16& acc01,
                                                 const f32x16& acc10, const f32x16& acc11) {
    constexpr int IMG = NB * BK;
    const int ch = L.frow >> 2, w = L.frow & 3;
#define DAG_PUT(ACC, i, j)                                                                              \
    _Pragma("unroll") for (int e = 0; e < 16; ++e) {                                                    \
        const int r = L.wr * 64 + (i) * 32 + (e & 3) + 8 * (e >> 2) + 4 * L.fh;                         \
        lds[(L.wc * 2 + (j)) * IMG + r * BK + 4 * (ch ^ (r & 7)) + w] = ACC[e];                         \
    }
    DAG_PUT(acc00, 0, 0)
    DAG_PUT(acc01, 0, 1)
    DAG_PUT(acc10, 1, 0)
    DAG_PUT(acc11, 1, 1)
#undef DAG_PUT
}

__device__ __forceinline__ void dag_self_product(const float* __restrict__ lds, const DagLane& L, f32x16& acc00, f32x16& acc01, f32x16& acc10,
                                                 f32x16& acc11) {
    constexpr int IMG = NB * BK;
#pragma unroll
    for (int s = 0; s < 4; ++s) {
#pragma unroll
        for (int g = 0; g < 4; ++g) {
            const float* img = lds + s * IMG;
            const float4 a0 = *reinterpret_cast<const float4*>(img + L.arow + 4 * ((2 * g + L.fh) ^ L.sw));
            const float4 a1 = *reinterpret_cast<const float4*>(img + L.arow + 32 * BK + 4 * ((2 * g + L.fh) ^ L.sw));
            const float4 b0 = *reinterpret_cast<const float4*>(img + L.brow + 4 * ((2 * g + L.fh) ^ L.sw));
            const float4 b1 = *reinterpret_cast<const float4*>(img + L.brow + 32 * BK + 4 * ((2 * g + L.fh) ^ L.sw));
            DAG_MFMA16(a0, a1, b0, b1)
        }
    }
}

template <bool SUB>
__device__ __forceinline__ void dag_epilogue(float* Cg , int64_t ldc, const DagLane& L, const f32x16& acc00,
                                             const f32x16& acc01, const f32x16& acc10, const f32x16& acc11) {
    const __amdgpu_buffer_rsrc_t crs = __builtin_amdgcn_make_buffer_rsrc((void*)Cg, (short)0, (int)(64 * ldc * 4), 0x00020000);
    const int cvoff = (int)(((4 * L.fh) * ldc + L.frow) * 4);
#define DAG_SOFF(i, j, e) (int)((((i) * 32 + ((e) & 3) + 8 * ((e) >> 2)) * ldc + (j) * 32) * 4)
#define DAG_EPI(ACC, i, j)                                                                                              \
    do {                                                                                                                \
        float pre[16];                                                                                                  \
        if (SUB) {                                                                                                      \
            _Pragma("unroll") for (int e = 0; e < 16; ++e)                                                              \
                pre[e] = __builtin_bit_cast(float, __builtin_amdgcn_raw_buffer_load_b32(crs, cvoff, DAG_SOFF(i, j, e), 16)); \
        }                                                                                                               \
        _Pragma("unroll") for (int e = 0; e < 16; ++e) {                                                                \
            const float o = SUB ? pre[e] - ACC[e] : ACC[e];                                                             \
            __builtin_amdgcn_raw_buffer_store_b32(__builtin_bit_cast(unsigned, o), crs, cvoff, DAG_SOFF(i, j, e), 16);  \
        }                                                                                                               \
    } while (0)
    DAG_EPI(acc00, 0, 0);
    DAG_EPI(acc01, 0, 1);
    DAG_EPI(acc10, 1, 0);
    DAG_EPI(acc11, 1, 1);
#undef DAG_EPI
#undef DAG_SOFF
}

__device__ __forceinline__ const float* dag_src(const float* tile0, int64_t ld, const DagLane& L) {
    return tile0 + (int64_t)(L.wid * 32 + L.rl) * ld + 4 * L.lc;
}

template <bool FAR>
__device__ __forceinline__ bool dag_tile_task(const DagSys& sy, int kind, int k0, int kfar, int i, int j, DagCtl* ctl, float* lds, const DagLane& L,
                                              int* s_flag, int* s_kav, long long* tr ) {
    const int t = threadIdx.x;
    const int kend = kind == DAG_PRE ? j - 1 : j;
    int* const st = sy.state;
    const int* rowfin_i = st + DAG_STATE_HDR + i;
    const int* rowfin_j = st + DAG_STATE_HDR + j;
    const float* Arow = sy.S + (int64_t)i * NB * sy.ld;
    const float* Brow = sy.S + (int64_t)j * NB * sy.ld;
    f32x16 acc00 = {0}, acc01 = {0}, acc10 = {0}, acc11 = {0};
    int kmid = kfar;
    if (FAR && sy.mid) {
        kmid = sy.mid[i];
        kmid = kmid < kfar ? kfar : kmid;
        kmid = kmid > kend ? (kend > kfar ? kend : kfar) : kmid;
    }
    int k = k0;
    while (k < kend) {
        bool ok = true;
        if (t == 0) {
            const long long w0 = tr ? wall_clock64() : 0;
            ok = dag_wait_ge(rowfin_i, k + 1, ctl, L.spin) && (i == j || dag_wait_ge(rowfin_j, k + 1, ctl, L.spin));
            if (tr) tr[2] += wall_clock64() - w0;
            int a = __hip_atomic_load(rowfin_i, __ATOMIC_RELAXED, __HIP_MEMORY_SCOPE_AGENT);
            const int b = i == j ? a : __hip_atomic_load(rowfin_j, __ATOMIC_RELAXED, __HIP_MEMORY_SCOPE_AGENT);
            a = a < b ? a : b;
            *s_kav = a < kend ? a : kend;
        }
        if (!dag_join(ok, s_flag)) return false;
        int kav = *s_kav;
        if (FAR && k < kfar) {
            kav = kav < kfar ? kav : kfar;
            dag_seg_bf16(lds, L, dag_src(Arow + (int64_t)k * NB, sy.ld, L), sy.ld, dag_src(Brow + (int64_t)k * NB, sy.ld, L), sy.ld,
                         (kav - k) * (NB / BK), acc00, acc01, acc10, acc11);
        } else if (FAR && k < kmid) {
            kav = kav < kmid ? kav : kmid;
            dag_seg_bf16x2(lds, L, dag_src(Arow + (int64_t)k * NB, sy.ld, L), sy.ld, dag_src(Brow + (int64_t)k * NB, sy.ld, L), sy.ld,
                           (kav - k) * (NB / BK), acc00, acc01, acc10, acc11);
        } else {
            dag_seg(lds, L, dag_src(Arow + (int64_t)k * NB, sy.ld, L), sy.ld, dag_src(Brow + (int64_t)k * NB, sy.ld, L), sy.ld, (kav - k) * (NB / BK),
                    acc00, acc01, acc10, acc11);
        }
        k = kav;
        __syncthreads();
    }
    float* Ct = sy.S + (int64_t)i * NB * sy.ld + (int64_t)j * NB;
    float* Cq = Ct + (int64_t)(L.wr * 64) * sy.ld + L.wc * 64;
    if (kind != DAG_TILE) {
        dag_epilogue<true>(Cq, sy.ld, L, acc00, acc01, acc10, acc11);
        asm volatile("s_waitcnt vmcnt(0)" ::: "memory");
        __syncthreads();
        if (t == 0) {
            asm volatile("buffer_inv sc1\n\ts_waitcnt vmcnt(0)" ::: "memory");
            __hip_atomic_store(st + DAG_STATE_HDR + (kind == DAG_PRE ? sy.nb : 2 * sy.nb) + j, 1, __ATOMIC_RELAXED, __HIP_MEMORY_SCOPE_AGENT);
        }
        return true;
    }
    if (kend > k0) {
        dag_epilogue<true>(Cq, sy.ld, L, acc00, acc01, acc10, acc11);
        asm volatile("s_waitcnt vmcnt(0)" ::: "memory");
    }
    bool ok = true;
    if (t == 0) {
        const long long w0 = tr ? wall_clock64() : 0;
        ok = dag_wait_ge(st, j + 1, ctl, L.spin);
        if (tr) { tr[2] += wall_clock64() - w0; tr[3] = wall_clock64(); }
    }
    if (!dag_join(ok, s_flag)) return false;
    acc00 = f32x16{0}; acc01 = f32x16{0}; acc10 = f32x16{0}; acc11 = f32x16{0};
    dag_seg(lds, L, dag_src(Ct, sy.ld, L), sy.ld, dag_src(sy.tinv + (int64_t)j * NB * NB, NB, L), NB, NB / BK, acc00, acc01, acc10, acc11);
    if (t == 0) dag_drop_l1();
    dag_epilogue<false>(Cq, sy.ld, L, acc00, acc01, acc10, acc11);
    dag_publish(st + DAG_STATE_HDR + i, j + 1);
    return true;
}

__device__ __forceinline__ void dag_chain_diag(const DagSys& sy, int j, int* info, float* lds, const DagLane& L, const struct DagSolve* sv,
                                               struct DagCtl* ctl);
__device__ __forceinline__ void dag_chain_diag_body(const DagSys& sy, int j, int* info, float* lds, const DagLane& L, bool* announced) {
    float* Pp = lds;
    float* Xr = Pp + 2 * D3_PBUF;
    float* dinvb = Xr + 7 * D3_TILE;
    float* stage = dinvb + 2 * D3_TILE;
    int64_t ldj = sy.ld;
    int lrj = L.lane & 15, lgj = L.lane >> 4;
    asm volatile("" : "+s"(ldj), "+v"(lrj), "+v"(lgj));
    gfloat* Sb = (gfloat*)(sy.S + (int64_t)j * NB * sy.ld + (int64_t)j * NB);
    gfloat* Tg = (gfloat*)(sy.tinv + (int64_t)j * NB * NB);
    if (L.wid == 0) d3_diagonal_wave<true>(Sb, ldj, Pp, dinvb, stage, info, j * NB, L.lane, lrj, lgj, sy.which);
    else if (L.wid == 1) d3_worker_wave<1, true>(Sb, ldj, Tg, Pp, Xr, dinvb, stage, lrj, lgj);
    else if (L.wid == 2) d3_worker_wave<2, true>(Sb, ldj, Tg, Pp, Xr, dinvb, stage, lrj, lgj);
    else d3_worker_wave<3, true>(Sb, ldj, Tg, Pp, Xr, dinvb, stage, lrj, lgj);
    *announced = true;
#ifdef OISAT_TEST_HOOKS
    if ((L.flags & 128) && j >= 3) {
        asm volatile("s_waitcnt vmcnt(0)" ::: "memory");
        __syncthreads();
        *announced = false;
        return;
    }
#endif
    dag_publish(sy.state, j + 1);
}

__device__ __forceinline__ bool dag_chain_panel(const DagSys& sy, int j, DagCtl* ctl, float* lds, const DagLane& L, int* s_flag, long long* ctr) {
    const int t = threadIdx.x;
    int* const st = sy.state;
    float* Sjj = sy.S + (int64_t)j * NB * sy.ld + (int64_t)j * NB;
    f32x16 acc00 = {0}, acc01 = {0}, acc10 = {0}, acc11 = {0};
    float* Pt = Sjj + (int64_t)NB * sy.ld;
    dag_seg(lds, L, dag_src(Pt, sy.ld, L), sy.ld, dag_src(sy.tinv + (int64_t)j * NB * NB, NB, L), NB, NB / BK, acc00, acc01, acc10, acc11);
    if (t == 0) dag_drop_l1();
    dag_epilogue<false>(Pt + (int64_t)(L.wr * 64) * sy.ld + L.wc * 64, sy.ld, L, acc00, acc01, acc10, acc11);
    dag_acc_to_image(lds, L, acc00, acc01, acc10, acc11);
    dag_publish(st + DAG_STATE_HDR + j + 1, j + 1);
    if (ctr && t == 0) ctr[8 * j + 3] = wall_clock64();
    acc00 = f32x16{0}; acc01 = f32x16{0}; acc10 = f32x16{0}; acc11 = f32x16{0};
    dag_self_product(lds, L, acc00, acc01, acc10, acc11);
    if (ctr && t == 0) ctr[8 * j + 4] = wall_clock64();
    {
        bool ok = true;
        if (t == 0 && j >= 1) ok = dag_wait_ge(st + DAG_STATE_HDR + sy.nb + j + 1, 1, ctl, L.spin);
        if (ctr && t == 0) ctr[8 * j + 5] = wall_clock64();
        if (!dag_join(ok, s_flag)) return false;
    }
    dag_epilogue<true>(Sjj + (int64_t)NB * sy.ld + NB + (int64_t)(L.wr * 64) * sy.ld + L.wc * 64, sy.ld, L, acc00, acc01, acc10, acc11);
    asm volatile("s_waitcnt vmcnt(0)" ::: "memory");
    __syncthreads();
    return true;
}

__device__ __forceinline__ bool dag_chain_task(const DagSys& sy, DagCtl* ctl, int* info, float* lds, const DagLane& L, int* s_flag,
                                               long long* ctr , const struct DagSolve* sv) {
    const int t = threadIdx.x;
    __builtin_amdgcn_s_setprio(3);
    for (int j = 0; j < sy.nb; ++j) {
        if (ctr && t == 0) ctr[8 * j + 0] = wall_clock64();
        dag_chain_diag(sy, j, info, lds, L, sv, ctl);
        if (ctr && t == 0) ctr[8 * j + 1] = wall_clock64();
        if (j + 1 == sy.nb) break;
        bool ok = true;
        if (t == 0 && j >= 1) ok = dag_wait_ge(sy.state + DAG_STATE_HDR + 2 * sy.nb + j, 1, ctl, L.spin);
        if (ctr && t == 0) ctr[8 * j + 2] = wall_clock64();
        if (!dag_join(ok, s_flag)) return false;
        if (!dag_chain_panel(sy, j, ctl, lds, L, s_flag, ctr)) return false;
    }
    __builtin_amdgcn_s_setprio(0);
    return true;
}

struct DagSolve {
    const SolveMember* mem;
    unsigned long long* queue;
    double g, g2, win_deg, cut_chord, tol2;
    int refine, dtype, cells, blocks;
    int nsys, qcap, qcap0;
    unsigned* trsv_timeouts;
    double* fwd_rhs;
    double* fwd_sol;
    const int* env;
};

__device__ __forceinline__ int dag_ld(const int* p) { return __hip_atomic_load(p, __ATOMIC_RELAXED, __HIP_MEMORY_SCOPE_AGENT); }
__device__ __forceinline__ void dag_st(int* p, int v) { __hip_atomic_store(p, v, __ATOMIC_RELAXED, __HIP_MEMORY_SCOPE_AGENT); }

__device__ __forceinline__ int dag_queue_of(int kind) { return kind >= DAG_RES ? 1 : 0; }
__device__ __forceinline__ void dag_queue_write(const DagSolve& sv, DagCtl* ctl, int qi, int slot, int kind, int sys, int a, int b) {
    if (slot >= (qi ? sv.qcap - sv.qcap0 : sv.qcap0)) {
        dag_st(&ctl->error, 1);
        return;
    }
    unsigned long long* e = sv.queue + 2 * (int64_t)((qi ? sv.qcap0 : 0) + slot);
    __hip_atomic_store(e + 1, (unsigned long long)(unsigned)a | ((unsigned long long)(unsigned)b << 32), __ATOMIC_RELAXED, __HIP_MEMORY_SCOPE_AGENT);
    asm volatile("s_waitcnt vmcnt(0)" ::: "memory");
    __hip_atomic_store(e, (unsigned long long)(unsigned)kind | ((unsigned long long)(unsigned)sys << 32), __ATOMIC_RELAXED, __HIP_MEMORY_SCOPE_AGENT);
}
__device__ __forceinline__ void dag_push_one(const DagSolve& sv, DagCtl* ctl, int kind, int sys, int a, int b) {
    const int qi = dag_queue_of(kind);
    const int slot = __hip_atomic_fetch_add(&ctl->q[qi].tail, 1, __ATOMIC_RELAXED, __HIP_MEMORY_SCOPE_AGENT);
    dag_queue_write(sv, ctl, qi, slot, kind, sys, a, b);
    asm volatile("s_waitcnt vmcnt(0)" ::: "memory");
    __hip_atomic_fetch_add(&ctl->q[qi].avail, 1, __ATOMIC_RELAXED, __HIP_MEMORY_SCOPE_AGENT);
}
__device__ __forceinline__ void dag_push_many(const DagSolve& sv, DagCtl* ctl, int kind, int sys, int a0, int n, int b, int* s_base) {
    const int qi = dag_queue_of(kind);
    __syncthreads();
    if (threadIdx.x == 0) *s_base = __hip_atomic_fetch_add(&ctl->q[qi].tail, n, __ATOMIC_RELAXED, __HIP_MEMORY_SCOPE_AGENT);
    __syncthreads();
    const int base = *s_base;
    for (int i = threadIdx.x; i < n; i += 256) dag_queue_write(sv, ctl, qi, base + i, kind, sys, a0 + i, b);
    asm volatile("s_waitcnt vmcnt(0)" ::: "memory");
    __syncthreads();
    if (threadIdx.x == 0) __hip_atomic_fetch_add(&ctl->q[qi].avail, n, __ATOMIC_RELAXED, __HIP_MEMORY_SCOPE_AGENT);
}
__device__ __forceinline__ bool dag_queue_pop(const DagSolve& sv, DagCtl* ctl, int qi, int4* task_out, int* slot_out, long long* tm ) {
    const long long c0 = tm ? wall_clock64() : 0;
    bool some = __hip_atomic_fetch_add(&ctl->q[qi].avail, 0, __ATOMIC_RELAXED, __HIP_MEMORY_SCOPE_AGENT) > 0;
    if (some && __hip_atomic_fetch_add(&ctl->q[qi].avail, -1, __ATOMIC_RELAXED, __HIP_MEMORY_SCOPE_AGENT) <= 0) {
        __hip_atomic_fetch_add(&ctl->q[qi].avail, 1, __ATOMIC_RELAXED, __HIP_MEMORY_SCOPE_AGENT);
        some = false;
    }
    if (!some) {
        if (tm) tm[0] += wall_clock64() - c0;
        return false;
    }
    int h = __hip_atomic_fetch_add(&ctl->q[qi].head, 1, __ATOMIC_RELAXED, __HIP_MEMORY_SCOPE_AGENT);
    const long long c1 = tm ? wall_clock64() : 0;
    if (tm) tm[1] += c1 - c0;
    if (h >= (qi ? sv.qcap - sv.qcap0 : sv.qcap0)) return false;
    h += qi ? sv.qcap0 : 0;
    unsigned long long w0;
    unsigned spins = 0;
    while (((w0 = __hip_atomic_load(&sv.queue[2 * (int64_t)h], __ATOMIC_RELAXED, __HIP_MEMORY_SCOPE_AGENT)) & 0xffffffffull) == 0ull) {
        __builtin_amdgcn_s_sleep(1);
        if (++spins > (1u << 22)) {
            dag_st(&ctl->error, 1);
            return false;
        }
    }
    const unsigned long long w1 = __hip_atomic_load(&sv.queue[2 * (int64_t)h + 1], __ATOMIC_RELAXED, __HIP_MEMORY_SCOPE_AGENT);
    *task_out = int4{(int)(w0 & 0xffffffffull), (int)(w0 >> 32), (int)(w1 & 0xffffffffull), (int)(w1 >> 32)};
    *slot_out = h;
    if (tm) tm[2] += wall_clock64() - c1;
    return true;
}

__device__ __forceinline__ int dag_inc_patches(const SolveMember& mb, int cells) {
    if (mb.nx > 0) return (int)(((mb.nx + 31) / 32) * (((mb.n / mb.nx) + 8 * cells - 1) / (8 * cells)));
    return (int)((mb.n + 256 * cells - 1) / (256 * cells));
}

__device__ __forceinline__ void dag_chain_diag(const DagSys& sy, int j, int* info, float* lds, const DagLane& L, const DagSolve* sv, DagCtl* ctl) {
    bool announced = false;
    dag_chain_diag_body(sy, j, info, lds, L, &announced);
    if (sv != nullptr && announced && threadIdx.x == 0) dag_push_one(*sv, ctl, DAG_FWD, sy.which, j, 0);
}

__device__ __forceinline__ void dag_task_acquire() {
    if (threadIdx.x == 0) asm volatile("buffer_inv sc1\n\ts_waitcnt vmcnt(0)" ::: "memory");
    __syncthreads();
}

__device__ __forceinline__ void dag_inc_account(int* word, int add, int npatch, DagCtl* ctl) {
    const int v = __hip_atomic_fetch_add(word, add, __ATOMIC_RELAXED, __HIP_MEMORY_SCOPE_AGENT) + add;
    if (v == DAG_INC_DECIDED + npatch) __hip_atomic_fetch_add(&ctl->sys_done, 1, __ATOMIC_RELAXED, __HIP_MEMORY_SCOPE_AGENT);
}
__device__ __forceinline__ bool dag_push_increment(const DagSys& sy, const SolveMember& mb, int sys, int g, bool final, const DagSolve& sv, DagCtl* ctl,
                                                   int* s_base, unsigned spin_max) {
    const int npatch = dag_inc_patches(mb, sv.cells);
    if (g >= 2) {
        __syncthreads();
        if (threadIdx.x == 0) {
            unsigned spins = 0;
            int ok = 1;
            while ((__hip_atomic_fetch_add(sy.state + DAG_ST_INC + g - 1, 0, __ATOMIC_RELAXED, __HIP_MEMORY_SCOPE_AGENT) & (DAG_INC_DECIDED - 1)) < npatch) {
                __builtin_amdgcn_s_sleep(8);
                if (++spins > spin_max || dag_ld(&ctl->error) != 0) {
                    dag_st(&ctl->error, 1);
                    ok = 0;
                    break;
                }
            }
            *s_base = ok;
        }
        __syncthreads();
        const bool ok = *s_base != 0;
        __syncthreads();
        if (!ok) return false;
    }
    dag_push_many(sv, ctl, DAG_INC, sys, 0, npatch, g, s_base);
    if (final && threadIdx.x == 0) dag_inc_account(sy.state + DAG_ST_INC + g, DAG_INC_DECIDED, npatch, ctl);
    return true;
}

__device__ __forceinline__ bool dag_after_sweeps(const DagSys& sy, const SolveMember& mb, int sys, int round, const DagSolve& sv, DagCtl* ctl, int* s_base,
                                                 unsigned spin_max) {
    const bool final = sv.refine == 0 || round == sv.refine;
    if (final || round >= 1)
        if (!dag_push_increment(sy, mb, sys, round, final, sv, ctl, s_base, spin_max)) return false;
    if (sv.refine > 0) dag_push_many(sv, ctl, DAG_RES, sys, 0, (int)((mb.m + 63) / 64), round, s_base);
    return true;
}

template <int TRANSPOSE>
__device__ __forceinline__ bool dag_sweep_task(const DagSys& sy, const SolveMember& mb, int sys, int tk, int round, const DagSolve& sv, DagCtl* ctl,
                                               float* lds, int* s_kav, unsigned spin_max) {
    const int t = threadIdx.x;
    int* const st = sy.state;
    const int nb = sy.nb;
    dag_task_acquire();
    __builtin_amdgcn_s_setprio(2);
    float* tile = lds;
    double* vec = reinterpret_cast<double*>(lds + NB * TLD);
    double* part = vec + NB;
    unsigned* s_ok = reinterpret_cast<unsigned*>(part + NB);
    if (t == 0) *s_ok = 1u;
    __syncthreads();
    double* in = TRANSPOSE ? mb.fwd : mb.rhs;
    double* out = TRANSPOSE ? mb.rhs : mb.fwd;
    if (!trsv_row<TRANSPOSE, true>(mb.S, mb.ld, mb.tinv, nb, tk, 0, in, out, reinterpret_cast<TrsvCtl*>(ctl), sv.trsv_timeouts, 0,
                                   TRANSPOSE ? mb.z : (double*)nullptr, mb.m, round > 0 ? 1 : 0, tile, vec, part, s_ok)) {
        __builtin_amdgcn_s_setprio(0);
        return false;
    }
    __builtin_amdgcn_s_setprio(0);
    asm volatile("s_waitcnt vmcnt(0)" ::: "memory");
    __syncthreads();
    if (t == 0) {
        const int done = __hip_atomic_fetch_add(st + (TRANSPOSE ? DAG_ST_BWD : DAG_ST_FWD) + round, 1, __ATOMIC_RELAXED, __HIP_MEMORY_SCOPE_AGENT);
        *s_kav = done == nb - 1 ? 1 : 0;
    }
    __syncthreads();
    const bool last = *s_kav != 0;
    __syncthreads();
    if (last) {
        if (!TRANSPOSE) dag_push_many(sv, ctl, DAG_BWD, sys, 0, nb, round, s_kav);
        else if (!dag_after_sweeps(sy, mb, sys, round, sv, ctl, s_kav, spin_max)) return false;
    }
    return true;
}

__device__ __forceinline__ bool dag_fwd_row_task(const DagSys& sy, int row, const DagSolve& sv, DagCtl* ctl, float* lds) {
    dag_task_acquire();
    __builtin_amdgcn_s_setprio(2);
    float* tile = lds;
    double* vec = reinterpret_cast<double*>(lds + NB * TLD);
    double* part = vec + NB;
    unsigned* s_ok = reinterpret_cast<unsigned*>(part + NB);
    if (threadIdx.x == 0) *s_ok = 1u;
    __syncthreads();
    int step0 = 0;
    if (sv.env != nullptr) {
        step0 = sv.env[row];
        step0 = step0 < 0 ? 0 : (step0 > row ? row : step0);
    }
    const bool ok = trsv_row<0, true>(sy.S, sy.ld, sy.tinv, sy.nb, row, step0, sv.fwd_rhs, sv.fwd_sol, reinterpret_cast<TrsvCtl*>(ctl),
                                      sv.trsv_timeouts, 0, (double*)nullptr, (int64_t)0, 0, tile, vec, part, s_ok);
    __builtin_amdgcn_s_setprio(0);
    if (!ok) return false;
    asm volatile("s_waitcnt vmcnt(0)" ::: "memory");
    __syncthreads();
    if (threadIdx.x == 0 &&
        __hip_atomic_fetch_add(sy.state + DAG_ST_FWD, 1, __ATOMIC_RELAXED, __HIP_MEMORY_SCOPE_AGENT) == sy.nb - 1)
        __hip_atomic_fetch_add(&ctl->sys_done, 1, __ATOMIC_RELAXED, __HIP_MEMORY_SCOPE_AGENT);
    return true;
}

__device__ __forceinline__ bool dag_res_task(const DagSys& sy, const SolveMember& mb, int sys, int c, int e, const DagSolve& sv, DagCtl* ctl, int* info,
                                             float* lds, int* s_kav, unsigned spin_max) {
    const int t = threadIdx.x;
    int* const st = sy.state;
    dag_task_acquire();
    __builtin_amdgcn_s_setprio(1);
    const SolveLds W = solve_lds_carve(lds);
    if (sv.blocks)
        resid_compact_block<OISAT_CORR_GAUSSIAN, true>(mb.oxyz, mb.osig, mb.ovar, mb.m, sv.g, mb.d, mb.z, mb.rhs, mb.olat, sv.win_deg, mb.perm, sv.cut_chord, (int64_t)c, W);
    else
        resid_rows_block<OISAT_CORR_GAUSSIAN, true>(mb.oxyz, mb.osig, mb.ovar, mb.m, sv.g, mb.d, mb.z, mb.rhs, sv.win_deg < 180.0 ? mb.olat : (const double*)nullptr,
                               sv.win_deg, (double*)nullptr, 1, 0, (int64_t)c, W);
    __builtin_amdgcn_s_setprio(0);
    asm volatile("s_waitcnt vmcnt(0)" ::: "memory");
    __syncthreads();
    const int nres = (int)((mb.m + 63) / 64);
    if (t == 0) *s_kav = __hip_atomic_fetch_add(st + DAG_ST_RES + e, 1, __ATOMIC_RELAXED, __HIP_MEMORY_SCOPE_AGENT) == nres - 1 ? 1 : 0;
    __syncthreads();
    const bool last = *s_kav != 0;
    __syncthreads();
    if (!last) return true;
    dag_task_acquire();
    double* sr = reinterpret_cast<double*>(lds) + 4096;
    double* sd = sr + 1024;
    const double* r = mb.rhs;
    const double* d = mb.d;
    const int64_t m = mb.m;
#pragma unroll
    for (int q = 0; q < 4; ++q) {
        double a = 0.0, b = 0.0;
        for (int64_t i = t + 256 * q; i < m; i += 1024) {
            a += r[i] * r[i];
            if (e == 0) b += d[i] * d[i];
        }
        sr[t + 256 * q] = a;
        sd[t + 256 * q] = b;
    }
    __syncthreads();
    for (int w = 512; w > 0; w >>= 1) {
        for (int i = t; i < w; i += 256) {
            sr[i] += sr[i + w];
            sd[i] += sd[i + w];
        }
        __syncthreads();
    }
    if (t == 0) {
        SolveState* ss = mb.st;
        double dd;
        if (e == 0) {
            dd = sd[0];
            __hip_atomic_store(&ss->dd, dd, __ATOMIC_RELAXED, __HIP_MEMORY_SCOPE_AGENT);
        } else {
            dd = __hip_atomic_load(&ss->dd, __ATOMIC_RELAXED, __HIP_MEMORY_SCOPE_AGENT);
        }
        __hip_atomic_store(&ss->norm[e], sr[0], __ATOMIC_RELAXED, __HIP_MEMORY_SCOPE_AGENT);
        dag_st(&ss->computed, e + 1);
        const bool conv = sr[0] <= sv.tol2 * dd;
        if (conv) dag_st(&ss->conv, 1);
        else if (e == sv.refine && sv.tol2 > 0.0) {
            atomicAdd(&info[kInfoUnconverged], 1);
            atomicCAS(&info[kInfoUnconvergedMember], 0, mb.which + 1);
        }
        *s_kav = conv ? 1 : 0;
    }
    __syncthreads();
    const bool conv = *s_kav != 0;
    __syncthreads();
    if (e < sv.refine) {
        if (conv && e == 0) {
            if (!dag_push_increment(sy, mb, sys, 0, true, sv, ctl, s_kav, spin_max)) return false;
        } else if (conv) {
            if (t == 0) dag_inc_account(st + DAG_ST_INC + e, DAG_INC_DECIDED, dag_inc_patches(mb, sv.cells), ctl);
        } else {
            dag_push_many(sv, ctl, DAG_FWD, sys, 0, sy.nb, e + 1, s_kav);
        }
    }
    return true;
}

template <typename T>
__device__ __forceinline__ bool dag_inc_task(const DagSys& sy, const SolveMember& mb, int blk, int gen, const DagSolve& sv, DagCtl* ctl, float* lds) {
    dag_task_acquire();
    __builtin_amdgcn_s_setprio(1);
    const SolveLds W = solve_lds_carve(lds);
    const bool windowed = sv.win_deg < 180.0;
    const double* glat = windowed ? mb.glat : (const double*)nullptr;
    const double* olat = windowed ? mb.olat : (const double*)nullptr;
    if (sv.cells == 1)
        increment_patch<OISAT_CORR_GAUSSIAN, T, 1>(mb.gxyz, mb.gsig, mb.n, mb.oxyz, mb.osig, mb.z, mb.m, sv.g2, (const T*)mb.xb, (T*)mb.xa, (T*)mb.inc, glat, olat,
                              sv.win_deg, mb.nx, sv.cut_chord, (int64_t)blk, W);
    else
        increment_patch<OISAT_CORR_GAUSSIAN, T, 2>(mb.gxyz, mb.gsig, mb.n, mb.oxyz, mb.osig, mb.z, mb.m, sv.g2, (const T*)mb.xb, (T*)mb.xa, (T*)mb.inc, glat, olat,
                              sv.win_deg, mb.nx, sv.cut_chord, (int64_t)blk, W);
    __builtin_amdgcn_s_setprio(0);
    __syncthreads();
    asm volatile("s_waitcnt vmcnt(0)" ::: "memory");
    __syncthreads();
    if (threadIdx.x == 0) dag_inc_account(sy.state + DAG_ST_INC + gen, 1, dag_inc_patches(mb, sv.cells), ctl);
    return true;
}

__device__ __forceinline__ void dag_lane_coords(DagLane& L, int t) {
    L.lane = t & 63;
    L.wid = __builtin_amdgcn_readfirstlane(t >> 6);
    L.wr = L.wid >> 1;
    L.wc = L.wid & 1;
    L.rl = L.lane >> 3;
    L.lc = (L.lane & 7) ^ L.rl;
    L.frow = L.lane & 31;
    L.fh = L.lane >> 5;
    L.sw = L.frow & 7;
    L.arow = (L.wr * 64 + L.frow) * BK;
    L.brow = (L.wc * 64 + L.frow) * BK;
}

constexpr int DAG_SOLVE_NONE = 0, DAG_SOLVE_ALL = 1, DAG_SOLVE_FWD = 2;
constexpr unsigned kDagFwdStayers = 16;
constexpr int kDagLdsFloats = 2 * 2 * NB * BK;
constexpr int kDagSolveLdsFloats = NB * TLD + 4 * NB + 16;
static_assert(kDagSolveLdsFloats >= kDagLdsFloats && (size_t)kDagSolveLdsFloats * 4 >= 32768 + 2 * 1024 * sizeof(double) &&
              kSolveLdsBytes <= 32768, "solve tasks' LDS fits");
template <int SOLVE>
__global__ __launch_bounds__(256, 2) void potrf_dag_kernel(const DagSys* __restrict__ systems, const int4* __restrict__ tasks, int ntasks,
                                                           DagCtl* __restrict__ ctl, int* __restrict__ info, unsigned* __restrict__ err_total,
                                                           int* __restrict__ state_all, int state_words, int reserve_chains, int flags,
                                                           long long* __restrict__ trace, int chain_rows_total, const DagSolve sv) {
    __shared__ __attribute__((aligned(16))) float lds[SOLVE ? kDagSolveLdsFloats : kDagLdsFloats];
    __shared__ int s_ticket, s_flag, s_kav;
    static_assert(2 * D3_PBUF + 7 * D3_TILE + 2 * D3_TILE + 16 * D3_SLD <= 2 * 2 * NB * BK, "diagonal-block LDS fits into the GEMM image");
    const int t = threadIdx.x;
    DagLane L;
    L.lane = t & 63;
    L.wid = __builtin_amdgcn_readfirstlane(t >> 6);
    L.wr = L.wid >> 1;
    L.wc = L.wid & 1;
    L.rl = L.lane >> 3;
    L.lc = (L.lane & 7) ^ L.rl;
    L.frow = L.lane & 31;
    L.fh = L.lane >> 5;
    L.sw = L.frow & 7;
    L.arow = (L.wr * 64 + L.frow) * BK;
    L.brow = (L.wc * 64 + L.frow) * BK;
    L.flags = flags;
    L.spin = kDagSpinMax;
#ifdef OISAT_TEST_HOOKS
    if (flags & 256) L.spin = 4096u;
#endif
    int cu_key = -1, first_on_cu = 1;
    if (reserve_chains > 0 || SOLVE == DAG_SOLVE_ALL) {
        if (t == 0) {
            unsigned xcc, hw;
            asm volatile("s_getreg_b32 %0, hwreg(HW_REG_XCC_ID)" : "=s"(xcc));
            asm volatile("s_getreg_b32 %0, hwreg(HW_REG_HW_ID)" : "=s"(hw));
            const int key = (int)(((xcc & 15u) << 8) | ((hw >> 8) & 255u));
            const int arrived = __hip_atomic_fetch_add(&ctl->cu_arrivals[key], 1, __ATOMIC_RELAXED, __HIP_MEMORY_SCOPE_AGENT);
            s_ticket = key;
            s_flag = arrived;
            if (arrived >= 1 && reserve_chains > 0) {
                unsigned spins = 0;
                while (__hip_atomic_load(&ctl->cu_role[key], __ATOMIC_RELAXED, __HIP_MEMORY_SCOPE_AGENT) == 0 && ++spins < 4096u)
                    __builtin_amdgcn_s_sleep(2);
                spins = 0;
                while (__hip_atomic_load(&ctl->ticket, __ATOMIC_RELAXED, __HIP_MEMORY_SCOPE_AGENT) < reserve_chains && ++spins < 4096u)
                    __builtin_amdgcn_s_sleep(2);
                s_kav = __hip_atomic_load(&ctl->cu_role[key], __ATOMIC_RELAXED, __HIP_MEMORY_SCOPE_AGENT);
            } else {
                s_kav = 0;
            }
        }
        __syncthreads();
        cu_key = s_ticket;
        first_on_cu = s_flag == 0;
    }
    const bool second_on_cu = !first_on_cu;
    bool leave_now = reserve_chains > 0 && !first_on_cu && s_kav == 2;
    __syncthreads();
    __shared__ int4 s_task;
    bool tickets_gone = false;
    unsigned idle = 0;
    long long wg_claim = 0, wg_first = 0, wg_tasks = 0, wg_n = 0;
    long long wg_pop[3] = {0, 0, 0};
    while (!leave_now) {
        __syncthreads();
        if (t == 0) {
            const long long c0 = trace ? wall_clock64() : 0;
            if (trace && wg_first == 0) wg_first = c0;
            int slot = -1;
            s_flag = 0;
            if (SOLVE && (dag_queue_pop(sv, ctl, 0, &s_task, &slot, trace && SOLVE == DAG_SOLVE_ALL ? wg_pop : (long long*)nullptr) ||
                          (SOLVE == DAG_SOLVE_ALL && (second_on_cu || tickets_gone) && dag_queue_pop(sv, ctl, 1, &s_task, &slot, trace ? wg_pop : (long long*)nullptr)))) {
                s_flag = 1;
                s_ticket = ntasks + slot;
            } else if (!tickets_gone) {
                s_ticket = __hip_atomic_fetch_add(&ctl->ticket, 1, __ATOMIC_RELAXED, __HIP_MEMORY_SCOPE_AGENT);
            } else {
                s_ticket = ntasks;
            }
            if (trace) wg_claim += wall_clock64() - c0;
        }
        __syncthreads();
        const int tk = s_ticket;
        const bool ready_task = SOLVE && s_flag != 0;
        if (cu_key >= 0 && first_on_cu) {
            if (t == 0)
                __hip_atomic_store(&ctl->cu_role[cu_key], !ready_task && tk < reserve_chains ? 2 : 1, __ATOMIC_RELAXED, __HIP_MEMORY_SCOPE_AGENT);
            cu_key = -1;
        }
        if (!ready_task && tk >= ntasks) {
            if (!SOLVE) break;
            if (SOLVE == DAG_SOLVE_FWD && blockIdx.x >= kDagFwdStayers) break;
            tickets_gone = true;
            __syncthreads();
            if (t == 0) {
                const bool done = __hip_atomic_fetch_add(&ctl->sys_done, 0, __ATOMIC_RELAXED, __HIP_MEMORY_SCOPE_AGENT) >= sv.nsys;
                bool bad = dag_ld(&ctl->error) != 0;
                if (!done && !bad && ++idle > L.spin) {
                    dag_st(&ctl->error, 1);
                    bad = true;
                }
                s_flag = done || bad ? 1 : 0;
            }
            __syncthreads();
            if (s_flag != 0) break;
            __builtin_amdgcn_s_sleep(SOLVE == DAG_SOLVE_FWD ? 64 : 8);
            continue;
        }
        idle = 0;
        int4 task = ready_task ? s_task : tasks[tk];
        task.x = __builtin_amdgcn_readfirstlane(task.x);
        task.y = __builtin_amdgcn_readfirstlane(task.y);
        task.z = __builtin_amdgcn_readfirstlane(task.z);
        task.w = __builtin_amdgcn_readfirstlane(task.w);
        const DagSys sy = systems[task.y];
        long long* tr = trace ? trace + 4 * (int64_t)tk : nullptr;
        if (tr && t == 0) {
            tr[0] = wall_clock64();
            tr[2] = 0;
            tr[3] = ready_task ? ((long long)task.x | ((long long)task.w << 4) | ((long long)task.y << 8) | ((long long)task.z << 24)) : 0;
        }
        bool ok;
        if constexpr (SOLVE == DAG_SOLVE_FWD) {
            int tt = t;
            asm volatile("" : "+v"(tt));
            dag_lane_coords(L, tt);
            if (ready_task) ok = dag_fwd_row_task(sy, task.z, sv, ctl, lds);
            else if ((task.x & 255) == DAG_CHAIN)
                ok = dag_chain_task(sy, ctl, info, lds, L, &s_flag, trace ? trace + 4 * (int64_t)(ntasks + sv.qcap) + 8 * (int64_t)task.z : nullptr, &sv);
            else ok = dag_tile_task<true>(sy, task.x & 255, (task.x >> 8) & 1023, task.x >> 18, task.z, task.w, ctl, lds, L, &s_flag, &s_kav, tr);
        } else if (ready_task) {
            const SolveMember mb = sv.mem[task.y];
            if (task.x == DAG_FWD) ok = dag_sweep_task<0>(sy, mb, task.y, task.z, task.w, sv, ctl, lds, &s_kav, L.spin);
            else if (task.x == DAG_BWD) ok = dag_sweep_task<1>(sy, mb, task.y, task.z, task.w, sv, ctl, lds, &s_kav, L.spin);
            else if (task.x == DAG_RES) ok = dag_res_task(sy, mb, task.y, task.z, task.w, sv, ctl, info, lds, &s_kav, L.spin);
            else if (sv.dtype == OISAT_F32) ok = dag_inc_task<float>(sy, mb, task.z, task.w, sv, ctl, lds);
            else ok = dag_inc_task<double>(sy, mb, task.z, task.w, sv, ctl, lds);
        } else if ((task.x & 255) == DAG_CHAIN) {
            ok = dag_chain_task(sy, ctl, info, lds, L, &s_flag, trace ? trace + 4 * (int64_t)(ntasks + (SOLVE ? sv.qcap : 0)) + 8 * (int64_t)task.z : nullptr,
                                SOLVE ? &sv : (const DagSolve*)nullptr);
        } else {
            ok = dag_tile_task<SOLVE != DAG_SOLVE_ALL>(sy, task.x & 255, (task.x >> 8) & 1023, task.x >> 18, task.z, task.w, ctl, lds, L, &s_flag,
                                                       &s_kav, tr);
        }
        if (tr && t == 0) {
            tr[1] = wall_clock64();
            wg_tasks += tr[1] - tr[0];
            ++wg_n;
        }
        if (!ok) break;
    }
    if (trace && t == 0) {
        long long* w = trace + 4 * (int64_t)(ntasks + (SOLVE ? sv.qcap : 0)) + 8 * (int64_t)chain_rows_total + 8 * (int64_t)blockIdx.x;
        w[0] = wg_first; w[1] = wg_claim; w[2] = wg_tasks; w[3] = wg_n; w[4] = wall_clock64(); w[5] = 0; w[6] = wg_pop[0] + wg_pop[1]; w[7] = wg_pop[2];
    }
    __syncthreads();
    if (t == 0) {
        asm volatile("s_waitcnt vmcnt(0)" ::: "memory");
        const int gone = __hip_atomic_fetch_add(&ctl->gone, 1, __ATOMIC_RELAXED, __HIP_MEMORY_SCOPE_AGENT);
        s_flag = gone == (int)gridDim.x - 1 ? 1 : 0;
    }
    __syncthreads();
    if (s_flag) {
        for (int w = t; w < state_words; w += 256) __hip_atomic_store(&state_all[w], 0, __ATOMIC_RELAXED, __HIP_MEMORY_SCOPE_AGENT);
        if (reserve_chains > 0 || SOLVE == DAG_SOLVE_ALL)
            for (int w = t; w < DAG_CU_KEYS; w += 256) {
                __hip_atomic_store(&ctl->cu_arrivals[w], 0, __ATOMIC_RELAXED, __HIP_MEMORY_SCOPE_AGENT);
                __hip_atomic_store(&ctl->cu_role[w], 0, __ATOMIC_RELAXED, __HIP_MEMORY_SCOPE_AGENT);
            }
        if (SOLVE) {
            for (int w = t; w < 2 * sv.qcap; w += 256) __hip_atomic_store(&sv.queue[w], 0ull, __ATOMIC_RELAXED, __HIP_MEMORY_SCOPE_AGENT);
        }
        __syncthreads();
        if (t == 0) {
            if (__hip_atomic_load(&ctl->error, __ATOMIC_RELAXED, __HIP_MEMORY_SCOPE_AGENT) != 0) atomicAdd(err_total, 1u);
            for (int qi = 0; qi < 2; ++qi) {
                __hip_atomic_store(&ctl->q[qi].head, 0, __ATOMIC_RELAXED, __HIP_MEMORY_SCOPE_AGENT);
                __hip_atomic_store(&ctl->q[qi].tail, 0, __ATOMIC_RELAXED, __HIP_MEMORY_SCOPE_AGENT);
                __hip_atomic_store(&ctl->q[qi].avail, 0, __ATOMIC_RELAXED, __HIP_MEMORY_SCOPE_AGENT);
            }
            __hip_atomic_store(&ctl->sys_done, 0, __ATOMIC_RELAXED, __HIP_MEMORY_SCOPE_AGENT);
            __hip_atomic_store(&ctl->ticket, 0, __ATOMIC_RELAXED, __HIP_MEMORY_SCOPE_AGENT);
            __hip_atomic_store(&ctl->error, 0, __ATOMIC_RELAXED, __HIP_MEMORY_SCOPE_AGENT);
            __hip_atomic_store(&ctl->gone, 0, __ATOMIC_RELAXED, __HIP_MEMORY_SCOPE_AGENT);
        }
    }
}
#undef DAG_MFMA4
#undef DAG_MFMA16

struct DagPlan {
    DagSys* sys_dev = nullptr;
    int4* tasks_dev = nullptr;
    int* state_dev = nullptr;
    DagCtl* ctl_dev = nullptr;
    int ntasks = 0, nsys = 0, state_words = 0, chain_rows = 0;
    int reserve_chains = 0;
    int max_wave_chains = 0;
    int solve_refine = -1;
    bool fwd_only = false;
    int64_t qcap = 0, qcap0 = 0;
    unsigned long long* queue_dev = nullptr;
    std::vector<DagSys> sys_host;
    std::vector<int4> tasks_host;
    std::vector<int> first;
    std::vector<int> far;
    std::vector<int> mid;
    int* mid_dev = nullptr;
    size_t tasks_cap = 0;
    long long* trace_dev = nullptr;
};

void dag_plan_free(DagPlan* p) {
    if (!p) return;
    if (p->sys_dev) (void)hipFree(p->sys_dev);
    if (p->tasks_dev) (void)hipFree(p->tasks_dev);
    if (p->state_dev) (void)hipFree(p->state_dev);
    if (p->ctl_dev) (void)hipFree(p->ctl_dev);
    if (p->queue_dev) (void)hipFree(p->queue_dev);
    if (p->mid_dev) (void)hipFree(p->mid_dev);
    if (p->trace_dev) (void)hipFree(p->trace_dev);
    delete p;
}

struct DagOrder {
    std::vector<int4> tasks;
    int chain_rows = 0, reserve_chains = 0, max_wave_chains = 0;
};
constexpr int kDagWave = 8;
constexpr double kDagEnvLead = 0.15;
constexpr double kDagEnvLeadFar = 0.2;
constexpr int kDagWave0Max = 64;
constexpr int kDagEnvMaxBlocks = 1024;
void dag_task_order(const std::vector<int>& nb_of, int wave_arg, DagOrder& out, const int* first = nullptr, const int* far = nullptr) {
    const int nsys = (int)nb_of.size();
    const int wave = wave_arg > 0 ? wave_arg : kDagWave;
    int nbig = 0;
    while (nbig < nsys && nbig < kDagWave0Max && 2 * nb_of[nbig] >= nb_of[0]) ++nbig;
    std::vector<std::pair<int, int>> waves;
    if (nbig == nsys) {
        waves.push_back({0, nsys});
    } else {
        std::vector<std::pair<int, int>> small_waves, big_pairs;
        for (int w0 = nbig; w0 < nsys; w0 += wave) small_waves.push_back({w0, w0 + wave < nsys ? w0 + wave : nsys});
        for (int b0 = 0; b0 < nbig; b0 += 2) big_pairs.push_back({b0, b0 + 2 < nbig ? b0 + 2 : nbig});
        const int k = (int)small_waves.size(), G = (int)big_pairs.size();
        int g = 0;
        for (int w = 0; w <= k; ++w) {
            while (g < G) {
                int at = (int)((double)g * (double)k / (double)G + 0.5);
                if (at != w) break;
                waves.push_back(big_pairs[g++]);
            }
            if (w < k) waves.push_back(small_waves[w]);
        }
    }
    std::vector<int4>& tasks = out.tasks;
    tasks.clear();
    bool any_far = false;
    for (int i = 0; first && far && i < nb_of[0]; ++i) any_far = any_far || far[i] > first[i];
    const double env_lead = any_far ? kDagEnvLeadFar : kDagEnvLead;
    int chain_rows = 0;
    int max_wave_chains = 0, second = 0;
    struct Item { double key; int4 task; };
    std::vector<Item> items;
    for (const std::pair<int, int>& wv : waves) {
        const int w0 = wv.first, w1 = wv.second;
        for (int s = w0; s < w1; ++s) {
            tasks.push_back(int4{DAG_CHAIN, s, chain_rows, 0});
            chain_rows += nb_of[s];
        }
        if (w1 - w0 > max_wave_chains) { second = max_wave_chains; max_wave_chains = w1 - w0; }
        else if (w1 - w0 > second) second = w1 - w0;
        items.clear();
        for (int s = w0; s < w1; ++s) {
            const int nb = nb_of[s];
            for (int j = 0; j < nb; ++j) {
                const double key = (double)j / (double)nb;
                auto ekey = [&](int i, int jj) { return ((double)jj - env_lead * (double)(jj - first[i])) / (double)nb; };
                auto word = [&](int kind, int i, int kend) {
                    if (!first) return kind;
                    const int k0 = first[i];
                    int kfar = far ? far[i] : k0;
                    kfar = kfar < k0 ? k0 : kfar;
                    kfar = kfar > kend ? (kend > k0 ? kend : k0) : kfar;
                    return kind | k0 << 8 | kfar << 18;
                };
                if (j >= 2) items.push_back(Item{(first ? ekey(j, j - 1) : (double)(j - 1) / (double)nb) - 1e-9, int4{word(DAG_PRE, j, j - 1), s, j, j}});
                if (j >= 1 && j + 1 < nb) items.push_back(Item{first ? ekey(j + 1, j) : key, int4{word(DAG_SUB, j + 1, j), s, j + 1, j}});
                for (int i = j + 2; i < nb && (!first || first[i] <= j); ++i)
                    items.push_back(Item{first ? ekey(i, j) : key, int4{word(DAG_TILE, i, j), s, i, j}});
            }
        }
        std::stable_sort(items.begin(), items.end(), [](const Item& a, const Item& b) { return a.key < b.key; });
        for (const Item& it : items) tasks.push_back(it.task);
    }
    out.chain_rows = chain_rows;
    out.max_wave_chains = max_wave_chains + (waves.size() > 1 ? (second > 0 ? second : max_wave_chains) : 0);
    {
        int n = 0;
        const int first_w0 = waves[0].first, first_w1 = waves[0].second;
        while (first_w0 + n < first_w1 && n < 4 && nb_of[first_w0 + n] >= 8) ++n;
        out.reserve_chains = n;
    }
}

struct DagSolveShape {
    int refine = -1;
    std::vector<int> nres, ninc;
    bool fwd_only = false;
};
static inline void dag_queue_entries(const std::vector<int>& nb_of, const DagSolveShape& sh, int64_t* sweep_rows, int64_t* valu_tasks) {
    *sweep_rows = *valu_tasks = 0;
    for (size_t s = 0; s < nb_of.size(); ++s) {
        if (sh.fwd_only) {
            *sweep_rows += nb_of[s];
            continue;
        }
        *sweep_rows += (int64_t)(sh.refine + 1) * 2 * nb_of[s];
        *valu_tasks += (int64_t)(sh.refine + 1) * ((sh.refine > 0 ? sh.nres[s] : 0) + sh.ninc[s]);
    }
}

static inline bool dag_fits(int max_wave_chains, int slots) { return 4 * max_wave_chains <= slots; }
static inline int dag_slots(const oisat_ctx* h) { return 2 * (h->cu_count > 0 ? h->cu_count : 256); }

static hipError_t dag_plan_mid(DagPlan& p, const int* mid, hipStream_t stream) {
    const size_t nb = p.first.size();
    p.mid.assign(mid ? mid : p.far.data(), (mid ? mid : p.far.data()) + nb);
    bool any = false;
    for (size_t i = 0; i < nb; ++i) any = any || p.mid[i] > p.far[i];
    const int* want = any ? p.mid_dev : nullptr;
    if (any)
        if (hipError_t e = hipMemcpyAsync(p.mid_dev, p.mid.data(), sizeof(int) * nb, hipMemcpyHostToDevice, stream)) return e;
    if (p.sys_host[0].mid == want) return hipSuccess;
    p.sys_host[0].mid = want;
    return hipMemcpyAsync(p.sys_dev, p.sys_host.data(), sizeof(DagSys), hipMemcpyHostToDevice, stream);
}

DagPlan* dag_plan_create(const std::vector<BatchMat>& table, hipStream_t stream, const DagSolveShape& shape = DagSolveShape(),
                         const int* first = nullptr, const int* far = nullptr, const int* mid = nullptr) {
    DagPlan* p = new DagPlan();
    const int nsys = (int)table.size();
    p->nsys = nsys;
    p->sys_host.resize(nsys);
    std::vector<int> state_off(nsys);
    int words = 0;
    for (int s = 0; s < nsys; ++s) {
        state_off[s] = words;
        words += DAG_STATE_HDR + 3 * table[s].mpb;
        words = (words + 31) / 32 * 32;
    }
    p->state_words = words;
    DagOrder order;
    {
        std::vector<int> nb_of(nsys);
        for (int s = 0; s < nsys; ++s) nb_of[s] = table[s].mpb;
        dag_task_order(nb_of, 0, order, nsys == 1 ? first : nullptr, nsys == 1 && first ? far : nullptr);
        if (first && nsys == 1) {
            p->first.assign(first, first + nb_of[0]);
            p->far.assign(far ? far : first, (far ? far : first) + nb_of[0]);
        }
        if (shape.refine >= 0) {
            int64_t rows = 0, valu = 0;
            dag_queue_entries(nb_of, shape, &rows, &valu);
            p->qcap0 = rows;
            p->qcap = rows + valu;
        }
    }
    p->solve_refine = shape.refine;
    p->fwd_only = shape.fwd_only;
    std::vector<int4>& tasks = order.tasks;
    p->max_wave_chains = order.max_wave_chains;
    p->chain_rows = order.chain_rows;
    p->reserve_chains = order.reserve_chains;
    p->ntasks = (int)tasks.size();
    p->tasks_host = tasks;
    p->tasks_cap = tasks.size();
    if (!p->first.empty()) {
        const size_t nb = (size_t)table[0].mpb;
        p->tasks_cap = 1 + 2 * nb + nb * (nb + 1) / 2;
    }
    bool ok = hipMalloc((void**)&p->sys_dev, sizeof(DagSys) * nsys) == hipSuccess &&
              hipMalloc((void**)&p->tasks_dev, sizeof(int4) * p->tasks_cap) == hipSuccess &&
              hipMalloc((void**)&p->state_dev, sizeof(int) * words) == hipSuccess &&
              hipMalloc((void**)&p->ctl_dev, sizeof(DagCtl)) == hipSuccess &&
              (p->first.empty() || hipMalloc((void**)&p->mid_dev, sizeof(int) * p->first.size()) == hipSuccess) &&
              (p->qcap == 0 || (p->qcap < (int64_t)INT32_MAX / 4 && hipMalloc((void**)&p->queue_dev, 16 * (size_t)p->qcap) == hipSuccess));
    if (ok && p->qcap > 0) ok = hipMemsetAsync(p->queue_dev, 0, 16 * (size_t)p->qcap, stream) == hipSuccess;
    if (ok) {
        for (int s = 0; s < nsys; ++s)
            p->sys_host[s] = DagSys{table[s].S, table[s].tinv, table[s].ld, p->state_dev + state_off[s], table[s].mpb, s};
        ok = hipMemcpy(p->sys_dev, p->sys_host.data(), sizeof(DagSys) * nsys, hipMemcpyHostToDevice) == hipSuccess &&
             hipMemcpy(p->tasks_dev, tasks.data(), sizeof(int4) * tasks.size(), hipMemcpyHostToDevice) == hipSuccess &&
             hipMemsetAsync(p->state_dev, 0, sizeof(int) * words, stream) == hipSuccess &&
             hipMemsetAsync(p->ctl_dev, 0, sizeof(DagCtl), stream) == hipSuccess;
        if (ok && !p->first.empty()) ok = dag_plan_mid(*p, mid, stream) == hipSuccess;
    }
    if (!ok) {
        dag_plan_free(p);
        oisat_set_error("task-graph factorization: allocation or upload of the plan failed");
        return nullptr;
    }
    return p;
}

int dag_plan_refill(DagPlan& p, const int* first, const int* far, const int* mid, hipStream_t stream) {
    const int nb = p.sys_host[0].nb;
    DagOrder order;
    dag_task_order(std::vector<int>{nb}, 0, order, first, far);
    if (order.tasks.size() > p.tasks_cap) {
        oisat_set_error("task-graph factorization: %zu tickets do not fit the plan's %zu", order.tasks.size(), p.tasks_cap);
        return OISAT_EINVAL;
    }
    HIP_TRY(hipStreamSynchronize(stream));
    p.tasks_host = order.tasks;
    p.ntasks = (int)order.tasks.size();
    p.first.assign(first, first + nb);
    p.far.assign(far ? far : first, (far ? far : first) + nb);
    p.max_wave_chains = order.max_wave_chains;
    p.chain_rows = order.chain_rows;
    p.reserve_chains = order.reserve_chains;
    if (p.trace_dev) { (void)hipFree(p.trace_dev); p.trace_dev = nullptr; }
    HIP_TRY(hipMemcpyAsync(p.tasks_dev, p.tasks_host.data(), sizeof(int4) * p.tasks_host.size(), hipMemcpyHostToDevice, stream));
    HIP_TRY(dag_plan_mid(p, mid, stream));
    return OISAT_OK;
}

int dag_launch(oisat_ctx* h, DagPlan& p, int* info_dev, unsigned* dag_timeouts, const DagSolve* solve = nullptr) {
    const int slots = dag_slots(h);
    if (!dag_fits(p.max_wave_chains, slots)) {
        oisat_set_error("task-graph factorization: %d chains of one wave on %d resident workgroups would not drain", p.max_wave_chains, slots);
        return OISAT_EINVAL;
    }
    if ((solve != nullptr) != (p.solve_refine >= 0) || (solve && solve->refine != p.solve_refine)) {
        oisat_set_error("task-graph launch: plan and solve arguments do not belong together");
        return OISAT_EINVAL;
    }
    const int grid = p.ntasks < slots ? p.ntasks : slots;
    const char* trace_file = getenv("OISAT_DAG_TRACE");
    const size_t trace_words = 4 * ((size_t)p.ntasks + (size_t)p.qcap) + 8 * (size_t)p.chain_rows + 8 * (size_t)grid;
    if (trace_file && !p.trace_dev) HIP_TRY(hipMalloc((void**)&p.trace_dev, sizeof(long long) * trace_words));
    if (trace_file) HIP_TRY(hipMemsetAsync(p.trace_dev, 0, sizeof(long long) * trace_words, h->stream));
    int flags = 0;
#ifdef OISAT_TEST_HOOKS
    if (getenv("OISAT_DAG_FLAGS")) flags = atoi(getenv("OISAT_DAG_FLAGS"));
#endif
    if (p.fwd_only && (p.nsys != 1 || !solve || !solve->fwd_rhs || !solve->fwd_sol || solve->nsys != 1)) {
        oisat_set_error("task-graph launch: the forward-sweep plan takes one system and its two work vectors");
        return OISAT_EINVAL;
    }
    if (solve) {
        if (solve->queue != p.queue_dev || solve->qcap != (int)p.qcap || solve->qcap0 != (int)p.qcap0) {
            oisat_set_error("task-graph launch: the solve arguments carry another plan's ready queue");
            return OISAT_EINVAL;
        }
        if (p.fwd_only) {
            OISAT_LAUNCH(h, "potrf_dag", potrf_dag_kernel<DAG_SOLVE_FWD>, dim3((unsigned)grid), dim3(256), 0, (const DagSys*)p.sys_dev,
                         (const int4*)p.tasks_dev, p.ntasks, p.ctl_dev, info_dev, dag_timeouts, p.state_dev, p.state_words, p.reserve_chains, flags,
                         trace_file ? p.trace_dev : (long long*)nullptr, p.chain_rows, *solve);
        } else {
            OISAT_LAUNCH(h, "analyse_dag", potrf_dag_kernel<DAG_SOLVE_ALL>, dim3((unsigned)grid), dim3(256), 0, (const DagSys*)p.sys_dev,
                         (const int4*)p.tasks_dev, p.ntasks, p.ctl_dev, info_dev, dag_timeouts, p.state_dev, p.state_words, p.reserve_chains, flags,
                         trace_file ? p.trace_dev : (long long*)nullptr, p.chain_rows, *solve);
        }
    } else {
        OISAT_LAUNCH(h, "potrf_dag", potrf_dag_kernel<DAG_SOLVE_NONE>, dim3((unsigned)grid), dim3(256), 0, (const DagSys*)p.sys_dev,
                     (const int4*)p.tasks_dev, p.ntasks, p.ctl_dev, info_dev, dag_timeouts, p.state_dev, p.state_words, p.reserve_chains, flags,
                     trace_file ? p.trace_dev : (long long*)nullptr, p.chain_rows, DagSolve{});
    }
    if (trace_file) {
        std::vector<long long> host(trace_words);
        HIP_TRY(hipStreamSynchronize(h->stream));
        HIP_TRY(hipMemcpy(host.data(), p.trace_dev, sizeof(long long) * trace_words, hipMemcpyDeviceToHost));
        if (FILE* f = fopen(trace_file, "wb")) {
            const int hdr[2] = {p.ntasks + (int)p.qcap, p.chain_rows + grid};
            fwrite(hdr, sizeof(int), 2, f);
            fwrite(p.tasks_host.data(), sizeof(int4), p.tasks_host.size(), f);
            {
                const std::vector<int4> pad((size_t)p.qcap, int4{-1, 0, 0, 0});
                fwrite(pad.data(), sizeof(int4), pad.size(), f);
            }
            fwrite(host.data(), sizeof(long long), host.size(), f);
            fclose(f);
        }
    }
    return OISAT_OK;
}
```

### oi-sat-gmi_amd/csrc/oisat_common.h

```cpp
#pragma once

#include <hip/hip_runtime.h>

#include <cmath>
#include <cstdarg>
#include <cstdint>
#include <cstdio>
#include <cstring>
#include <string>
#include <vector>

#include "../../include/oisat.h"

constexpr int kWave = 64;

void oisat_set_error(const char* fmt, ...);

struct ProfRec {
    char name[64];
    double total_ms = 0.0;
    int64_t launches = 0;
};

struct ProfPending {
    int rec;
    hipEvent_t a, b;
};

struct ChFactor {
    const float* S = nullptr;
    int64_t m = 0, mp = 0, ld = 0;
    float* tinv = nullptr;
    const int* env = nullptr;
    int band = 0;
    const double* fwd_d = nullptr;
};

struct BatchMat {
    float* S;
    float* tinv;
    int64_t ld;
    int64_t m;
    int mpb;
    int pad;
};

struct SolveState {
    double dd;
    double norm[12];
    int conv;
    int computed;
};

struct SolveMember {
    const float* S;
    const float* tinv;
    int64_t ld, m;
    int mpb, nx;
    const double *oxyz, *osig, *ovar, *d, *olat;
    double *z, *rhs, *fwd;
    SolveState* st;
    const double *gxyz, *gsig, *glat;
    int64_t n;
    const void* xb;
    void* xa;
    void* inc;
    const int* perm;
    int which;
};

struct ChBatch {
    BatchMat* table_dev = nullptr;
    int* cum_dev = nullptr;
    std::vector<int> cum_off, cum_cnt, cum_total;
    std::vector<long long> cum_key;
    std::vector<BatchMat> table;
    std::vector<int> order;
    int max_mpb = 0;
    SolveMember* solve_dev = nullptr;
    std::vector<SolveMember> solve_host;
    int64_t max_patches = 0;
    int* ord_dev = nullptr;
    void* ctl_dev = nullptr;
    int ord_total = 0;
    int64_t max_m = 0, max_n = 0, max_mp = 0;
    bool pairs = false;
    void* dag = nullptr;
    void* dag_solve = nullptr;
    int dag_solve_refine = -1, dag_solve_cells = 0;
};

struct DagSingle {
    void* plan = nullptr;
    const float* S = nullptr;
    const float* tinv = nullptr;
    int64_t ld = 0, mpb = 0;
    bool enveloped = false;
    bool fwd = false;
    uint64_t stamp = 0;
};

struct oisat_ctx {
    int device = 0;
    hipStream_t stream = nullptr;
    int cu_count = 0;
    size_t hbm_bytes = 0;
    char name[128] = {0};
    bool prof = false;
    std::vector<ProfRec> recs;
    std::vector<ProfPending> pending;
    std::vector<hipEvent_t> free_events;
    void* ws[10] = {nullptr, nullptr, nullptr, nullptr, nullptr, nullptr, nullptr, nullptr, nullptr, nullptr};
    size_t ws_bytes[10] = {0, 0, 0, 0, 0, 0, 0, 0, 0, 0};
    double scales_host[OISAT_MAX_SCALES] = {0};
    int scales_n = 0;
    const void* scales_dev = nullptr;
    ChFactor factor;
    bool small_tiles = true;
    double refine_tol = 1e-6;
    int corr = 0;
    int wave_prio = 0;
    int gemm_wg_per_cu = 0;
    hipStream_t own_stream = nullptr;
    hipStream_t aux_stream = nullptr;
    std::vector<hipEvent_t> sync_events;
    void* comm = nullptr;
    int comm_rank = 0, comm_size = 1;
    hipEvent_t signal_event = nullptr;
    std::vector<ChBatch*> batches;
    const int* obs_perm = nullptr;
    int64_t obs_perm_m = 0;
    std::vector<int32_t> factor_far;
    std::vector<int32_t> factor_mid;
    int dag_mode = -1;
    DagSingle dag_cache[8];
    uint64_t dag_clock = 0;
    void* pinned = nullptr;
    size_t pinned_bytes = 0;
    hipStream_t xfer_streams[4] = {nullptr, nullptr, nullptr, nullptr};
};

#define HIP_TRY(expr)                                                                          \
    do {                                                                                       \
        hipError_t _e = (expr);                                                                \
        if (_e != hipSuccess) {                                                                \
            oisat_set_error("%s failed: %s (%s:%d)", #expr, hipGetErrorString(_e), __FILE__, __LINE__); \
            return OISAT_EHIP;                                                                 \
        }                                                                                      \
    } while (0)

#define ARG_CHECK(cond)                                                                        \
    do {                                                                                       \
        if (!(cond)) {                                                                         \
            oisat_set_error("invalid argument: %s (%s:%d)", #cond, __FILE__, __LINE__);        \
            return OISAT_EINVAL;                                                               \
        }                                                                                      \
    } while (0)

void* oisat_ws(oisat_ctx* h, int slot, size_t bytes);
void* oisat_pinned(oisat_ctx* h, size_t bytes);
bool oisat_envelope_off();
void oisat_dag_plan_release(void* plan);

int oisat_prof_begin(oisat_ctx* h, const char* name);
void oisat_prof_end(oisat_ctx* h, int pending);

#define OISAT_LAUNCH(h, NAME, kernel, grid, block, shmem, ...)                                 \
    do {                                                                                       \
        int _p = (h)->prof ? oisat_prof_begin((h), NAME) : -1;                                 \
        hipLaunchKernelGGL(kernel, grid, block, shmem, (h)->stream, __VA_ARGS__);              \
        if (_p >= 0) oisat_prof_end((h), _p);                                                  \
        hipError_t _le = hipGetLastError();                                                    \
        if (_le != hipSuccess) {                                                               \
            oisat_set_error("launch of %s failed: %s", NAME, hipGetErrorString(_le));          \
            return OISAT_EHIP;                                                                 \
        }                                                                                      \
    } while (0)

static inline int64_t cdiv(int64_t a, int64_t b) { return (a + b - 1) / b; }

static inline int stream_grid(int64_t work_items, int per_block) {
    int64_t g = cdiv(work_items, per_block);
    if (g < 1) g = 1;
    if (g > 2048) g = 2048;
    return (int)g;
}

template <typename T>
__device__ __forceinline__ T nan_of();
template <>
__device__ __forceinline__ float nan_of<float>() { return __builtin_nanf(""); }
template <>
__device__ __forceinline__ double nan_of<double>() { return __builtin_nan(""); }
```

### oi-sat-gmi_amd/csrc/oisat_core.hip

```cpp
#include "oisat_common.h"
#include <thread>

static thread_local char g_err[512] = "";

void oisat_set_error(const char* fmt, ...) {
    va_list ap;
    va_start(ap, fmt);
    vsnprintf(g_err, sizeof(g_err), fmt, ap);
    va_end(ap);
}

extern "C" const char* oisat_last_error(void) { return g_err; }
extern "C" const char* oisat_version(void) { return "oisat-hip 0.1 (gfx950)"; }

extern "C" int oisat_init(int device_id, oisat_ctx** out) {
    ARG_CHECK(out != nullptr);
    *out = nullptr;
    int ndev = 0;
    hipError_t e = hipGetDeviceCount(&ndev);
    if (e != hipSuccess || ndev <= 0) {
        oisat_set_error("no HIP device visible (%s)", e == hipSuccess ? "count = 0" : hipGetErrorString(e));
        return OISAT_ENODEV;
    }
    ARG_CHECK(device_id >= 0 && device_id < ndev);
    HIP_TRY(hipSetDevice(device_id));
    hipDeviceProp_t prop;
    HIP_TRY(hipGetDeviceProperties(&prop, device_id));
    if (strncmp(prop.gcnArchName, "gfx950", 6) != 0) {
        oisat_set_error("device %d is %s; this library is built for gfx950 (MI355X) only", device_id, prop.gcnArchName);
        return OISAT_ENODEV;
    }
    oisat_ctx* h = new oisat_ctx();
    h->device = device_id;
    h->cu_count = prop.multiProcessorCount;
    h->hbm_bytes = prop.totalGlobalMem;
    snprintf(h->name, sizeof(h->name), "%s (%s)", prop.name, prop.gcnArchName);
    *out = h;
    return OISAT_OK;
}

extern "C" int oisat_comm_destroy(oisat_ctx* h);

extern "C" void oisat_shutdown(oisat_ctx* h) {
    if (!h) return;
    (void)hipSetDevice(h->device);
    if (h->comm) (void)oisat_comm_destroy(h);
    (void)hipDeviceSynchronize();
    for (auto& p : h->pending) {
        (void)hipEventDestroy(p.a);
        (void)hipEventDestroy(p.b);
    }
    for (auto ev : h->free_events) (void)hipEventDestroy(ev);
    for (int i = 0; i < 10; ++i)
        if (h->ws[i]) (void)hipFree(h->ws[i]);
    if (h->pinned) (void)hipHostFree(h->pinned);
    if (h->own_stream) (void)hipStreamDestroy(h->own_stream);
    if (h->aux_stream) (void)hipStreamDestroy(h->aux_stream);
    for (hipStream_t& xs : h->xfer_streams)
        if (xs) (void)hipStreamDestroy(xs);
    for (auto ev : h->sync_events) (void)hipEventDestroy(ev);
    if (h->signal_event) (void)hipEventDestroy(h->signal_event);
    for (auto* b : h->batches)
        if (b) {
            if (b->table_dev) (void)hipFree(b->table_dev);
            if (b->cum_dev) (void)hipFree(b->cum_dev);
            if (b->solve_dev) (void)hipFree(b->solve_dev);
            if (b->ord_dev) (void)hipFree(b->ord_dev);
            if (b->ctl_dev) (void)hipFree(b->ctl_dev);
            oisat_dag_plan_release(b->dag);
            delete b;
        }
    for (DagSingle& c : h->dag_cache) oisat_dag_plan_release(c.plan);
    delete h;
}

extern "C" int oisat_device_info(oisat_ctx* h, char* name_out, int name_cap, int* cu_count, int64_t* hbm_bytes) {
    ARG_CHECK(h != nullptr);
    if (name_out && name_cap > 0) snprintf(name_out, name_cap, "%s", h->name);
    if (cu_count) *cu_count = h->cu_count;
    if (hbm_bytes) *hbm_bytes = (int64_t)h->hbm_bytes;
    return OISAT_OK;
}

extern "C" int oisat_set_stream(oisat_ctx* h, void* hip_stream) {
    ARG_CHECK(h != nullptr);
    h->stream = (hipStream_t)hip_stream;
    return OISAT_OK;
}

extern "C" int oisat_stream_create(oisat_ctx* h) {
    ARG_CHECK(h != nullptr);
    if (!h->own_stream) HIP_TRY(hipStreamCreateWithFlags(&h->own_stream, hipStreamNonBlocking));
    h->stream = h->own_stream;
    return OISAT_OK;
}

extern "C" int oisat_stream_create_masked(oisat_ctx* h, int reserve_per_xcd) {
    ARG_CHECK(h != nullptr && reserve_per_xcd >= 0 && h->own_stream == nullptr);
    const int ncu = h->cu_count > 0 ? h->cu_count : 256;
    ARG_CHECK(8 * reserve_per_xcd < ncu);
    if (reserve_per_xcd == 0) return oisat_stream_create(h);
    std::vector<uint32_t> mask((ncu + 31) / 32, 0xffffffffu);
    for (int b = ncu - 8 * reserve_per_xcd; b < (int)mask.size() * 32; ++b) mask[b / 32] &= ~(1u << (b % 32));
    HIP_TRY(hipExtStreamCreateWithCUMask(&h->own_stream, (uint32_t)mask.size(), mask.data()));
    h->stream = h->own_stream;
    h->cu_count = ncu - 8 * reserve_per_xcd;
    return OISAT_OK;
}

extern "C" int oisat_bind_thread(oisat_ctx* h) {
    ARG_CHECK(h != nullptr);
    HIP_TRY(hipSetDevice(h->device));
    return OISAT_OK;
}

extern "C" int oisat_wait_for(oisat_ctx* waiter, oisat_ctx* signaler) {
    ARG_CHECK(waiter != nullptr && signaler != nullptr);
    if (waiter->stream == signaler->stream) return OISAT_OK;
    if (!signaler->signal_event) HIP_TRY(hipEventCreateWithFlags(&signaler->signal_event, hipEventDisableTiming));
    HIP_TRY(hipEventRecord(signaler->signal_event, signaler->stream));
    HIP_TRY(hipStreamWaitEvent(waiter->stream, signaler->signal_event, 0));
    return OISAT_OK;
}

extern "C" int oisat_sync(oisat_ctx* h) {
    ARG_CHECK(h != nullptr);
    HIP_TRY(hipStreamSynchronize(h->stream));
    return OISAT_OK;
}

extern "C" int oisat_query(oisat_ctx* h, int* busy) {
    ARG_CHECK(h != nullptr && busy != nullptr);
    const hipError_t e = hipStreamQuery(h->stream);
    if (e != hipSuccess && e != hipErrorNotReady) {
        oisat_set_error("hipStreamQuery failed: %s", hipGetErrorString(e));
        return OISAT_EHIP;
    }
    *busy = e == hipErrorNotReady ? 1 : 0;
    return OISAT_OK;
}

extern "C" int oisat_dmalloc(oisat_ctx* h, size_t bytes, void** dev_out) {
    ARG_CHECK(h != nullptr && dev_out != nullptr);
    *dev_out = nullptr;
    if (bytes == 0) bytes = 16;
    hipError_t e = hipMalloc(dev_out, bytes);
    if (e != hipSuccess) {
        oisat_set_error("hipMalloc(%zu) failed: %s", bytes, hipGetErrorString(e));
        return OISAT_ENOMEM;
    }
    return OISAT_OK;
}

extern "C" int oisat_dfree(oisat_ctx* h, void* dev) {
    ARG_CHECK(h != nullptr);
    if (dev) HIP_TRY(hipFree(dev));
    return OISAT_OK;
}

extern "C" int oisat_h2d(oisat_ctx* h, void* dev_dst, const void* host_src, size_t bytes) {
    ARG_CHECK(h != nullptr && (bytes == 0 || (dev_dst && host_src)));
    if (bytes) HIP_TRY(hipMemcpyAsync(dev_dst, host_src, bytes, hipMemcpyHostToDevice, h->stream));
    return OISAT_OK;
}

constexpr size_t kSlicedReadback = (size_t)48 << 20;

extern "C" int oisat_d2h(oisat_ctx* h, void* host_dst, const void* dev_src, size_t bytes) {
    ARG_CHECK(h != nullptr && (bytes == 0 || (host_dst && dev_src)));
    if (bytes < kSlicedReadback) {
        if (bytes) HIP_TRY(hipMemcpyAsync(host_dst, dev_src, bytes, hipMemcpyDeviceToHost, h->stream));
        HIP_TRY(hipStreamSynchronize(h->stream));
        return OISAT_OK;
    }
    HIP_TRY(hipStreamSynchronize(h->stream));
    constexpr int T = 4;
    for (int t = 0; t < T; ++t)
        if (!h->xfer_streams[t]) HIP_TRY(hipStreamCreateWithFlags(&h->xfer_streams[t], hipStreamNonBlocking));
    const size_t slice = ((bytes / T) + 4095) & ~(size_t)4095;
    hipError_t rc[T];
    std::thread th[T];
    for (int t = 0; t < T; ++t) {
        rc[t] = hipSuccess;
        const size_t off = (size_t)t * slice;
        if (off >= bytes) continue;
        const size_t len = bytes - off < slice ? bytes - off : slice;
        auto copy_slice = [=, &rc]() {
            hipError_t e = hipSetDevice(h->device);
            if (e == hipSuccess) e = hipMemcpyAsync((char*)host_dst + off, (const char*)dev_src + off, len, hipMemcpyDeviceToHost, h->xfer_streams[t]);
            if (e == hipSuccess) e = hipStreamSynchronize(h->xfer_streams[t]);
            rc[t] = e;
        };
        try {
            th[t] = std::thread(copy_slice);
        } catch (...) {
            copy_slice();
        }
    }
    for (int t = 0; t < T; ++t)
        if (th[t].joinable()) th[t].join();
    for (int t = 0; t < T; ++t) HIP_TRY(rc[t]);
    return OISAT_OK;
}

extern "C" int oisat_memset(oisat_ctx* h, void* dev, int byte_value, size_t bytes) {
    ARG_CHECK(h != nullptr && (bytes == 0 || dev));
    if (bytes) HIP_TRY(hipMemsetAsync(dev, byte_value, bytes, h->stream));
    return OISAT_OK;
}

void* oisat_ws(oisat_ctx* h, int slot, size_t bytes) {
    if (bytes == 0) bytes = 16;
    if (h->ws_bytes[slot] >= bytes) return h->ws[slot];
    if (h->ws[slot]) {
        (void)hipStreamSynchronize(h->stream);
        (void)hipFree(h->ws[slot]);
        h->ws[slot] = nullptr;
        h->ws_bytes[slot] = 0;
    }
    size_t want = bytes + bytes / 8;
    hipError_t e = hipMalloc(&h->ws[slot], want);
    if (e != hipSuccess) {
        want = bytes;
        e = hipMalloc(&h->ws[slot], want);
    }
    if (e != hipSuccess) {
        oisat_set_error("workspace hipMalloc(%zu) failed: %s", want, hipGetErrorString(e));
        h->ws[slot] = nullptr;
        return nullptr;
    }
    h->ws_bytes[slot] = want;
    return h->ws[slot];
}

void* oisat_pinned(oisat_ctx* h, size_t bytes) {
    if (h->pinned_bytes >= bytes) return h->pinned;
    if (h->pinned) (void)hipHostFree(h->pinned);
    h->pinned = nullptr;
    h->pinned_bytes = 0;
    size_t want = bytes < 65536 ? 65536 : bytes;
    if (hipHostMalloc(&h->pinned, want, hipHostMallocDefault) != hipSuccess) {
        oisat_set_error("hipHostMalloc(%zu) failed", want);
        h->pinned = nullptr;
        return nullptr;
    }
    h->pinned_bytes = want;
    return h->pinned;
}

static hipEvent_t take_event(oisat_ctx* h) {
    if (!h->free_events.empty()) {
        hipEvent_t e = h->free_events.back();
        h->free_events.pop_back();
        return e;
    }
    hipEvent_t e = nullptr;
    (void)hipEventCreate(&e);
    return e;
}

int oisat_prof_begin(oisat_ctx* h, const char* name) {
    int rec = -1;
    for (size_t i = 0; i < h->recs.size(); ++i)
        if (strncmp(h->recs[i].name, name, 63) == 0) { rec = (int)i; break; }
    if (rec < 0) {
        ProfRec r;
        snprintf(r.name, sizeof(r.name), "%s", name);
        h->recs.push_back(r);
        rec = (int)h->recs.size() - 1;
    }
    ProfPending p;
    p.rec = rec;
    p.a = take_event(h);
    p.b = take_event(h);
    if (!p.a || !p.b) return -1;
    (void)hipEventRecord(p.a, h->stream);
    h->pending.push_back(p);
    return (int)h->pending.size() - 1;
}

void oisat_prof_end(oisat_ctx* h, int pending) { (void)hipEventRecord(h->pending[pending].b, h->stream); }

static void prof_drain(oisat_ctx* h) {
    (void)hipStreamSynchronize(h->stream);
    for (auto& p : h->pending) {
        float ms = 0.f;
        if (hipEventElapsedTime(&ms, p.a, p.b) == hipSuccess) {
            h->recs[p.rec].total_ms += ms;
            h->recs[p.rec].launches += 1;
        }
        h->free_events.push_back(p.a);
        h->free_events.push_back(p.b);
    }
    h->pending.clear();
}

extern "C" int oisat_prof_enable(oisat_ctx* h, int on) {
    ARG_CHECK(h != nullptr);
    if (!on && h->prof) prof_drain(h);
    h->prof = on != 0;
    return OISAT_OK;
}

extern "C" int oisat_prof_reset(oisat_ctx* h) {
    ARG_CHECK(h != nullptr);
    prof_drain(h);
    h->recs.clear();
    return OISAT_OK;
}

extern "C" int oisat_prof_collect(oisat_ctx* h, int cap, char (*names)[64], double* total_ms, int64_t* launches) {
    ARG_CHECK(h != nullptr);
    prof_drain(h);
    int n = (int)h->recs.size();
    for (int i = 0; i < n && i < cap; ++i) {
        if (names) memcpy(names[i], h->recs[i].name, 64);
        if (total_ms) total_ms[i] = h->recs[i].total_ms;
        if (launches) launches[i] = h->recs[i].launches;
    }
    return n;
}
```

### oi-sat-gmi_amd/oisatgmi/_hip.py

```python
from __future__ import annotations

import collections
import ctypes as C
import os
import sys
import threading

import numpy as np

F32, F64 = 0, 1
MAX_SCALES = 128

_c_ctx = C.c_void_p
_i64 = C.c_int64
_ptr = C.c_void_p

SIGNATURES = {
    "oisat_init": (C.c_int, [C.c_int, C.POINTER(_c_ctx)]),
    "oisat_shutdown": (None, [_c_ctx]),
    "oisat_last_error": (C.c_char_p, []),
    "oisat_version": (C.c_char_p, []),
    "oisat_device_info": (C.c_int, [_c_ctx, C.c_char_p, C.c_int, C.POINTER(C.c_int), C.POINTER(_i64)]),
    "oisat_set_stream": (C.c_int, [_c_ctx, _ptr]),
    "oisat_stream_create": (C.c_int, [_c_ctx]),
    "oisat_bind_thread": (C.c_int, [_c_ctx]),
    "oisat_wait_for": (C.c_int, [_c_ctx, _c_ctx]),
    "oisat_query": (C.c_int, [_c_ctx, C.POINTER(C.c_int)]),
    "oisat_stream_create_masked": (C.c_int, [_c_ctx, C.c_int]),
    "oisat_set_share": (C.c_int, [_c_ctx, C.c_int, C.c_int]),
    "oisat_set_refine_tol": (C.c_int, [_c_ctx, C.c_double]),
    "oisat_sync": (C.c_int, [_c_ctx]),
    "oisat_dmalloc": (C.c_int, [_c_ctx, C.c_size_t, C.POINTER(_ptr)]),
    "oisat_dfree": (C.c_int, [_c_ctx, _ptr]),
    "oisat_h2d": (C.c_int, [_c_ctx, _ptr, _ptr, C.c_size_t]),
    "oisat_d2h": (C.c_int, [_c_ctx, _ptr, _ptr, C.c_size_t]),
    "oisat_memset": (C.c_int, [_c_ctx, _ptr, C.c_int, C.c_size_t]),
    "oisat_prof_enable": (C.c_int, [_c_ctx, C.c_int]),
    "oisat_prof_reset": (C.c_int, [_c_ctx]),
    "oisat_prof_collect": (C.c_int, [_c_ctx, C.c_int, _ptr, C.POINTER(C.c_double), C.POINTER(_i64)]),
    "oisat_oi_curve": (C.c_int, [_c_ctx, C.c_int, _ptr, _ptr, _i64, C.POINTER(C.c_double), C.c_int,
                                 C.POINTER(C.c_double), C.POINTER(_i64)]),
    "oisat_oi_apply": (C.c_int, [_c_ctx, C.c_int, _ptr, _ptr, _ptr, _ptr, _i64, C.c_double, _ptr, _ptr, _ptr, _ptr]),
    "oisat_oi_fused": (C.c_int, [_c_ctx, C.c_int, _ptr, _ptr, _ptr, _ptr, _i64, C.POINTER(C.c_double), C.c_int, C.c_int,
                                 _ptr, _ptr, _ptr, _ptr, _ptr, _ptr]),
    "oisat_nanmean_stack": (C.c_int, [_c_ctx, C.c_int, _ptr, C.c_int, _i64, C.c_int, _ptr]),
    "oisat_error_average": (C.c_int, [_c_ctx, C.c_int, _ptr, C.c_int, _i64, C.c_int, _ptr]),
    "oisat_month_accumulate": (C.c_int, [_c_ctx, C.c_int, _ptr, _ptr, _ptr, _ptr, _ptr, C.c_int, _i64, _ptr, _ptr]),
    "oisat_month_finish": (C.c_int, [_c_ctx, C.c_int, _ptr, _i64, _ptr]),
    "oisat_all_nan": (C.c_int, [_c_ctx, C.c_int, _ptr, _i64, _ptr]),
    "oisat_widen": (C.c_int, [_c_ctx, _ptr, _i64, _ptr]),
    "oisat_affine": (C.c_int, [_c_ctx, C.c_int, _ptr, _i64, C.c_double, C.c_double, _ptr]),
    "oisat_oi_variances": (C.c_int, [_c_ctx, C.c_int, _ptr, _ptr, _i64, C.c_double, _ptr, _ptr]),
    "oisat_scaling_factor": (C.c_int, [_c_ctx, C.c_int, _ptr, _ptr, _i64, _ptr]),
    "oisat_partial_column": (C.c_int, [_c_ctx, C.c_int, _ptr, _ptr, _i64, _ptr]),
    "oisat_amf_recal": (C.c_int, [_c_ctx, _ptr, _ptr, C.c_int, C.c_int, _ptr, _ptr, C.c_int, _ptr, _ptr, _ptr, _i64, _ptr, _ptr,
                                  _ptr]),
    "oisat_column_sum": (C.c_int, [_c_ctx, C.c_int, _ptr, _ptr, C.c_int, _ptr, _ptr, _i64, _ptr]),
    "oisat_ak_conv_mopitt": (C.c_int, [_c_ctx, C.c_int, _ptr, _ptr, _ptr, C.c_int, _ptr, _ptr, _ptr, C.c_int, _ptr, _ptr, _ptr, _i64,
                                       _ptr, _ptr]),
    "oisat_ak_conv_gosat": (C.c_int, [_c_ctx, C.c_int, _ptr, _ptr, C.c_int, _ptr, _ptr, _ptr, _ptr, C.c_int, _ptr, _i64, _ptr]),
    "oisat_water_column": (C.c_int, [_c_ctx, C.c_int, _ptr, _ptr, _i64, _ptr]),
    "oisat_pwv_sum": (C.c_int, [_c_ctx, C.c_int, _ptr, C.c_int, _ptr, _i64, _ptr]),
    "oisat_boxfilter_symm": (C.c_int, [_c_ctx, C.c_int, _ptr, _i64, _i64, C.c_int, C.c_int, C.c_int, _ptr]),
    "oisat_nn_query": (C.c_int, [_c_ctx, _ptr, _ptr, _i64, _ptr, _ptr, _i64, C.c_double, _ptr, _ptr]),
    "oisat_nn_query_ties": (C.c_int, [_c_ctx, _ptr, _ptr, _i64, _ptr, _ptr, _i64, C.c_double, _ptr, _ptr, _ptr,
                                      C.POINTER(C.c_int64)]),
    "oisat_gather_mask": (C.c_int, [_c_ctx, C.c_int, _ptr, _i64, C.c_int, _ptr, _i64, _ptr]),
    "oisat_linear_interp": (C.c_int, [_c_ctx, C.c_int, _ptr, _ptr, _i64, _ptr, _ptr, _ptr, _ptr, _ptr, _i64, _ptr, _i64,
                                      C.c_int, _ptr, C.POINTER(C.c_double)]),
    "oisat_linear_locate": (C.c_int, [_c_ctx, _ptr, _ptr, _i64, _ptr, _ptr, _ptr, _ptr, _ptr, _i64, _i64, C.POINTER(C.c_double),
                                      _ptr, C.POINTER(C.c_int64)]),
    "oisat_linear_interp_forced": (C.c_int, [_c_ctx, C.c_int, _ptr, _ptr, _i64, _ptr, _ptr, _ptr, _ptr, _ptr, _i64, _ptr, _i64,
                                             C.c_int, _ptr, C.POINTER(C.c_double), _ptr]),
    "oisat_rbf_interp": (C.c_int, [_c_ctx, C.c_int, _ptr, _ptr, _i64, _ptr, _ptr, _i64, _ptr, C.c_double, C.c_int, _ptr, C.c_int,
                                   _ptr, C.POINTER(C.c_int64)]),
    "oisat_tri_transform": (C.c_int, [_c_ctx, _ptr, _i64, _ptr, _i64, _ptr, _ptr, C.POINTER(C.c_int64)]),
    "oisat_rbf_interp_ties": (C.c_int, [_c_ctx, C.c_int, _ptr, _ptr, _i64, _ptr, _ptr, _i64, _ptr, C.c_double, C.c_int, _ptr, C.c_int,
                                        _ptr, C.POINTER(C.c_int64), _ptr, C.POINTER(C.c_int64)]),
    "oisat_rbf_interp_forced": (C.c_int, [_c_ctx, C.c_int, _ptr, _ptr, _i64, _ptr, _ptr, _i64, _ptr, _ptr, _i64, C.c_int, _ptr,
                                          C.c_int, _ptr, C.POINTER(C.c_int64)]),
    "oisat_rbf_check_masked": (C.c_int, [_c_ctx, _ptr, _ptr, _i64, _ptr, _ptr, _i64, _ptr, C.c_double, C.c_int, C.POINTER(_i64)]),
    "oisat_boxfilter_pick": (C.c_int, [_c_ctx, C.c_int, _ptr, _i64, _i64, C.c_int, C.c_int, C.c_int, C.c_int,
                                       _ptr, _i64, _ptr]),
    "oisat_flag_mask": (C.c_int, [_c_ctx, C.c_int, _ptr, _ptr, _i64, C.c_double, C.c_int, _ptr]),
    "oisat_sqrt": (C.c_int, [_c_ctx, C.c_int, _ptr, _i64, _ptr]),
    "oisat_cov_build": (C.c_int, [_c_ctx, _ptr, _ptr, _ptr, _i64, C.c_double, _ptr, _i64]),
    "oisat_innovation": (C.c_int, [_c_ctx, C.c_int, _ptr, _ptr, _ptr, _i64, _ptr]),
    "oisat_gemm_nt": (C.c_int, [_c_ctx, _ptr, _i64, _ptr, _i64, _ptr, _i64, _i64, _i64, _i64, C.c_int, C.c_int]),
    "oisat_potrf": (C.c_int, [_c_ctx, _ptr, _i64, _i64, C.POINTER(C.c_int)]),
    "oisat_envelope": (C.c_int, [_ptr, _i64, C.c_double, _ptr]),
    "oisat_factor_envelope": (C.c_int, [_ptr, _i64, C.c_double, _ptr]),
    "oisat_factor_far": (C.c_int, [_ptr, _i64, C.c_double, _ptr, _ptr]),
    "oisat_set_factor_far": (C.c_int, [_ptr, _ptr, _i64]),
    "oisat_factor_mid": (C.c_int, [_ptr, _i64, C.c_double, _ptr, _ptr, _ptr]),
    "oisat_set_factor_mid": (C.c_int, [_ptr, _ptr, _i64]),
    "oisat_set_correlation": (C.c_int, [_c_ctx, C.c_int]),
    "oisat_corr_eval": (C.c_int, [C.c_int, C.c_double, _ptr, _i64, _ptr]),
    "oisat_corr_cut_chord": (C.c_int, [C.c_int, C.c_double, C.c_double, C.POINTER(C.c_double)]),
    "oisat_envelope_corr": (C.c_int, [C.c_int, _ptr, _i64, C.c_double, _ptr]),
    "oisat_factor_envelope_corr": (C.c_int, [C.c_int, _ptr, _i64, C.c_double, _ptr]),
    "oisat_factor_far_corr": (C.c_int, [C.c_int, _ptr, _i64, C.c_double, _ptr, _ptr]),
    "oisat_factor_mid_corr": (C.c_int, [C.c_int, _ptr, _i64, C.c_double, _ptr, _ptr, _ptr]),
    "oisat_dag_task_order_env": (C.c_int, [C.c_int, _ptr, _ptr, _ptr, _i64, C.POINTER(_i64)]),
    "oisat_cov_build_env": (C.c_int, [_c_ctx, _ptr, _ptr, _ptr, _i64, C.c_double, _ptr, _i64, _ptr]),
    "oisat_potrf_env": (C.c_int, [_c_ctx, _ptr, _i64, _i64, _ptr, _ptr, C.POINTER(C.c_int)]),
    "oisat_cov_build_env_zeroed": (C.c_int, [_c_ctx, _ptr, _ptr, _ptr, _i64, C.c_double, _ptr, _i64, _ptr, _ptr, _ptr, _ptr,
                                             C.POINTER(C.c_int)]),
    "oisat_cov_build_cover": (C.c_int, [_ptr, _ptr, _i64, _ptr, C.POINTER(C.c_int64), C.POINTER(C.c_int64)]),
    "oisat_potrf_env_fwd": (C.c_int, [_c_ctx, _ptr, _i64, _i64, _ptr, _ptr, _ptr, C.POINTER(C.c_int), C.POINTER(C.c_int)]),
    "oisat_trsv_plan": (C.c_int, [_i64, C.c_int, C.c_int, C.POINTER(C.c_int32), C.POINTER(C.c_int32)]),
    "oisat_potrs": (C.c_int, [_c_ctx, _ptr, _i64, _i64, _ptr]),
    "oisat_cov_residual": (C.c_int, [_c_ctx, _ptr, _ptr, _ptr, _i64, C.c_double, _ptr, _ptr, _ptr, _ptr]),
    "oisat_gain_solve": (C.c_int, [_c_ctx, _ptr, _ptr, _ptr, _ptr, _i64, _i64, C.c_double, _ptr, C.c_int, _ptr,
                                   C.POINTER(C.c_double), _ptr]),
    "oisat_trsm_rows": (C.c_int, [_c_ctx, _ptr, _i64, _i64, _ptr, _i64, _i64]),
    "oisat_posterior_error": (C.c_int, [_c_ctx, _ptr, _i64, _i64, _ptr, _ptr, _i64, _i64, _i64, _ptr, _ptr, C.c_double, _i64, _ptr]),
    "oisat_gain_diag": (C.c_int, [_c_ctx, _ptr, _i64, _i64, _ptr, _i64, _ptr]),
    "oisat_apply_increment": (C.c_int, [_c_ctx, C.c_int, _ptr, _ptr, _i64, _ptr, _ptr, _ptr, _i64, C.c_double, _ptr,
                                        _ptr, _ptr, _ptr, _ptr]),
    "oisat_apply_increment_grid": (C.c_int, [_c_ctx, C.c_int, _ptr, _ptr, _i64, _i64, _ptr, _ptr, _ptr, _i64, C.c_double, _ptr,
                                             _ptr, _ptr, _ptr, _ptr]),
    "oisat_batch_create": (C.c_int, [_c_ctx, C.c_int, C.POINTER(_ptr), C.POINTER(_i64), C.POINTER(_i64), C.POINTER(_ptr),
                                     C.POINTER(C.c_int)]),
    "oisat_batch_potrf": (C.c_int, [_c_ctx, C.c_int, C.POINTER(C.c_int)]),
    "oisat_batch_set_solve": (C.c_int, [_c_ctx, C.c_int, C.c_int] + [C.POINTER(_ptr)] * 11 + [C.POINTER(_i64)] + [C.POINTER(_ptr)] * 3),
    "oisat_set_task_graph": (C.c_int, [_c_ctx, C.c_int]),
    "oisat_dag_task_order": (C.c_int, [C.c_int, _ptr, C.c_int, _ptr, _i64, C.POINTER(_i64), C.POINTER(C.c_int), C.POINTER(C.c_int)]),
    "oisat_batch_set_grid": (C.c_int, [_c_ctx, C.c_int, C.c_int, C.POINTER(_i64), C.POINTER(_ptr)]),
    "oisat_set_obs_blocks": (C.c_int, [_c_ctx, _ptr, _i64]),
    "oisat_batch_solve": (C.c_int, [_c_ctx, C.c_int, C.c_int, C.c_double, C.c_int]),
    "oisat_batch_analyse": (C.c_int, [_c_ctx, C.c_int, C.c_int, C.c_double, C.c_int, C.POINTER(C.c_int)]),
    "oisat_batch_is_task_graph": (C.c_int, [_c_ctx, C.c_int, C.POINTER(C.c_int)]),
    "oisat_batch_destroy": (C.c_int, [_c_ctx, C.c_int]),
    "oisat_factor_adopt": (C.c_int, [_c_ctx, _ptr, _i64, _i64, _ptr]),
    "oisat_comm_unique_id": (C.c_int, [C.c_char_p, C.c_int]),
    "oisat_comm_init": (C.c_int, [_c_ctx, C.c_int, C.c_int, C.c_char_p]),
    "oisat_comm_bcast": (C.c_int, [_c_ctx, _ptr, C.c_size_t, C.c_int]),
    "oisat_comm_gather": (C.c_int, [_c_ctx, _ptr, C.c_size_t, _ptr, C.c_int]),
    "oisat_comm_destroy": (C.c_int, [_c_ctx]),
    "oisat_solve_status": (C.c_int, [_c_ctx, C.POINTER(C.c_int), C.POINTER(C.c_int), C.POINTER(C.c_int), C.c_int]),
    "oisat_solve_status_ex": (C.c_int, [_c_ctx, C.POINTER(C.c_int32), C.c_int, C.c_int]),
    "oisat_dense_reserve": (C.c_int, [_c_ctx, _i64, _i64]),
}


class OisatError(RuntimeError):
    """A call into liboisat_hip.so returned an error code."""


class OisatUnavailable(RuntimeError):
    """The HIP backend cannot run here (library missing / no MI355X).  There is no fallback."""


def library_path() -> str:
    env = os.environ.get("OISAT_LIB")
    if env:
        return env
    here = os.path.dirname(os.path.abspath(__file__))
    return os.path.join(os.path.dirname(here), "lib", "liboisat_hip.so")


_lib = None
_lib_lock = threading.Lock()


def load_library():
    global _lib
    with _lib_lock:
        if _lib is not None:
            return _lib
        path = library_path()
        if not os.path.exists(path):
            raise OisatUnavailable(
                f"{path} not found: build it with `python -c 'import __graft_entry__ as g; g.build()'` "
                f"or `make -C oi-sat-gmi_amd/csrc`.  This package has no CPU fallback.")
        os.environ.setdefault("GPU_MAX_HW_QUEUES", "16")
        if "torch" not in sys.modules and os.environ.get("OISAT_PRELOAD_TORCH", "1") != "0":
            try:
                import torch
            except Exception:
                pass
        try:
            lib = C.CDLL(path)
        except OSError as e:
            raise OisatUnavailable(f"cannot load {path}: {e}.  This package has no CPU fallback.") from e
        for name, (res, args) in SIGNATURES.items():
            fn = getattr(lib, name)
            fn.restype = res
            fn.argtypes = args
        _lib = lib
        return lib


def load_test_hooks_library():
    load_library()
    path = os.path.join(os.path.dirname(library_path()), "liboisat_hip_testhooks.so")
    if not os.path.exists(path):
        raise OisatUnavailable(f"{path} not found: `make -C oi-sat-gmi_amd/csrc` builds it next to the product library")
    lib = C.CDLL(path)
    for name, (res, args) in SIGNATURES.items():
        fn = getattr(lib, name)
        fn.restype = res
        fn.argtypes = args
    return lib


def dtype_code(dt) -> int:
    dt = np.dtype(dt)
    if dt == np.float32:
        return F32
    if dt == np.float64:
        return F64
    raise TypeError(f"unsupported field dtype {dt}; float32 or float64 only")


def compute_dtype(*arrays) -> np.dtype:
    env = os.environ.get("OISAT_DTYPE", "").lower()
    if env in ("f32", "float32"):
        return np.dtype(np.float32)
    if env in ("f64", "float64"):
        return np.dtype(np.float64)
    for a in arrays:
        if np.asarray(a).dtype != np.float32:
            return np.dtype(np.float64)
    return np.dtype(np.float32)


class SolveStatus(collections.namedtuple("SolveStatus", "notpd_col notpd_blocks trsv_timeouts unconverged unconverged_member dag_timeouts")):
    __slots__ = ()

    @property
    def clean(self) -> bool:
        return not (self.notpd_col or self.notpd_blocks or self.trsv_timeouts or self.unconverged or self.dag_timeouts)


class DeviceBuffer:

    __slots__ = ("ctx", "ptr", "nbytes", "foreign")

    def __init__(self, ctx: "Context", nbytes: int):
        self.ctx = ctx
        self.nbytes = int(nbytes)
        self.foreign = False
        cached = ctx._take_cached(self.nbytes)
        if cached is not None:
            self.ptr = cached
            return
        p = _ptr()
        ctx.check(ctx.lib.oisat_dmalloc(ctx.h, max(self.nbytes, 16), C.byref(p)))
        self.ptr = p.value

    def shared_with_other_streams(self):
        self.foreign = True
        return self

    def free(self):
        if self.ptr is not None and self.ctx is not None and self.ctx.h is not None:
            if self.foreign or not self.ctx._give_cached(self.nbytes, self.ptr):
                self.ctx.lib.oisat_dfree(self.ctx.h, self.ptr)
        self.ptr = None

    def __del__(self):
        try:
            self.free()
        except Exception:
            pass

    def at(self, byte_offset: int) -> int:
        return self.ptr + int(byte_offset)


class Context:

    def __init__(self, device: int, lib=None):
        self.lib = lib if lib is not None else load_library()
        h = _c_ctx()
        rc = self.lib.oisat_init(int(device), C.byref(h))
        if rc != 0:
            msg = self.lib.oisat_last_error().decode()
            raise OisatUnavailable(f"oisat_init(device={device}) failed: {msg}.  This package has no CPU fallback.")
        self.h = h
        self.device = int(device)
        self._cache = {}
        self._cache_bytes = 0
        self._cache_lock = threading.Lock()

    _CACHE_MAX_BUFFER = 256 << 20
    _CACHE_MAX_TOTAL = 2 << 30

    def _take_cached(self, nbytes):
        with self._cache_lock:
            lst = self._cache.get(nbytes)
            if lst:
                self._cache_bytes -= nbytes
                return lst.pop()
        return None

    def _give_cached(self, nbytes, ptr) -> bool:
        if nbytes <= 0 or nbytes > self._CACHE_MAX_BUFFER or os.environ.get("OISAT_BUFFER_CACHE", "1") == "0":
            return False
        try:
            self.sync()
        except OisatError:
            return False
        with self._cache_lock:
            if self._cache_bytes + nbytes > self._CACHE_MAX_TOTAL:
                return False
            self._cache.setdefault(nbytes, []).append(ptr)
            self._cache_bytes += nbytes
        return True

    def drop_cache(self):
        with self._cache_lock:
            for lst in self._cache.values():
                for ptr in lst:
                    self.lib.oisat_dfree(self.h, ptr)
            self._cache.clear()
            self._cache_bytes = 0

    def check(self, rc: int):
        if rc != 0:
            raise OisatError(f"liboisat_hip error {rc}: {self.lib.oisat_last_error().decode()}")

    def close(self):
        if self.h is not None:
            self.drop_cache()
            self.lib.oisat_shutdown(self.h)
            self.h = None

    def set_stream(self, stream_handle: int | None):
        self.check(self.lib.oisat_set_stream(self.h, stream_handle or None))

    def own_stream(self):
        self.check(self.lib.oisat_stream_create(self.h))
        return self

    def own_stream_masked(self, reserve_per_xcd: int):
        self.check(self.lib.oisat_stream_create_masked(self.h, int(reserve_per_xcd)))
        return self

    def bind_thread(self):
        self.check(self.lib.oisat_bind_thread(self.h))

    def wait_for(self, other: "Context"):
        self.check(self.lib.oisat_wait_for(self.h, other.h))

    def sync(self):
        self.check(self.lib.oisat_sync(self.h))

    def busy(self) -> bool:
        b = C.c_int(0)
        self.check(self.lib.oisat_query(self.h, C.byref(b)))
        return bool(b.value)

    def alloc(self, nbytes: int) -> DeviceBuffer:
        return DeviceBuffer(self, nbytes)

    def upload(self, arr: np.ndarray, dtype=None) -> DeviceBuffer:
        a = np.ascontiguousarray(arr, dtype=dtype)
        buf = DeviceBuffer(self, a.nbytes)
        self.check(self.lib.oisat_h2d(self.h, buf.ptr, a.ctypes.data, a.nbytes))
        self.sync()
        return buf

    def upload_into(self, dev_ptr: int, arr: np.ndarray, dtype=None) -> int:
        a = np.ascontiguousarray(arr, dtype=dtype)
        self.check(self.lib.oisat_h2d(self.h, dev_ptr, a.ctypes.data, a.nbytes))
        self.sync()
        return a.nbytes

    def download(self, dev_ptr: int, shape, dtype) -> np.ndarray:
        out = np.empty(shape, dtype=dtype)
        self.check(self.lib.oisat_d2h(self.h, out.ctypes.data, dev_ptr, out.nbytes))
        return out

    def device_info(self):
        name = C.create_string_buffer(128)
        cu = C.c_int()
        hbm = _i64()
        self.check(self.lib.oisat_device_info(self.h, name, 128, C.byref(cu), C.byref(hbm)))
        return {"name": name.value.decode(), "cu_count": cu.value, "hbm_bytes": hbm.value}

    def solve_status(self, clear=True) -> "SolveStatus":
        w = (C.c_int32 * len(SolveStatus._fields))()
        self.check(self.lib.oisat_solve_status_ex(self.h, w, len(SolveStatus._fields), 1 if clear else 0))
        return SolveStatus(*(int(x) for x in w))

    def check_solves(self, what="dense analysis"):
        st = self.solve_status(clear=True)._asdict()
        msgs = []
        if st["notpd_col"] or st["notpd_blocks"]:
            msgs.append(f"H B H^T + R not positive definite (first bad column {st['notpd_col']}, {st['notpd_blocks']} diagonal block(s))")
        if st["dag_timeouts"]:
            msgs.append(f"{st['dag_timeouts']} task-graph factorization(s) timed out: incomplete factor")
        if st["trsv_timeouts"]:
            msgs.append(f"{st['trsv_timeouts']} triangular-solve workgroup(s) gave up waiting: z holds NaN fill")
        if st["unconverged"]:
            who = f", first: batch member {st['unconverged_member']}" if st["unconverged_member"] >= 0 else ""
# ... 52 lines not shown
```

Before: 13.79 million grid-cells/s.

## Store pre-split bf16 hi/lo shadow of factor panels for far/mid trailing updates

```diff
diff --git a/include/oisat.h b/include/oisat.h
--- a/include/oisat.h
+++ b/include/oisat.h
@@ -183,6 +183,9 @@
 int oisat_factor_mid_corr(int kind, const double* lat_sorted, int64_t m, double g, const int32_t* first, const int32_t* far,
                           int32_t* mid_out);
 int oisat_set_factor_mid(oisat_ctx* h, const int32_t* mid, int64_t nb);
+int oisat_factor_shadow_layout(int nb, const int32_t* first, int64_t* rowoff_out, int64_t* ntiles_out);
+int oisat_set_factor_shadow_cap(oisat_ctx* h, int64_t bytes);
+int oisat_factor_shadow_tile(oisat_ctx* h, int r, int k, uint16_t* hi_out, uint16_t* lo_out);
 int oisat_cov_build_env(oisat_ctx* h, const double* oxyz, const double* osig, const double* ovar, int64_t m,
                         double g, float* S, int64_t ld, const int32_t* env_dev);
 int oisat_potrf_env(oisat_ctx* h, float* S, int64_t m, int64_t ld, const int32_t* first, const int32_t* env_dev,
diff --git a/oi-sat-gmi_amd/csrc/dense_chol.hip b/oi-sat-gmi_amd/csrc/dense_chol.hip
--- a/oi-sat-gmi_amd/csrc/dense_chol.hip
+++ b/oi-sat-gmi_amd/csrc/dense_chol.hip
@@ -1917,10 +1917,20 @@
     return e != nullptr && atoi(e) == 0;
 }
 
+static int factor_shadow_mode() {
+    const char* e = getenv("OISAT_FACTOR_SHADOW");
+    if (!e || !*e || strcmp(e, "1") == 0) return 3;
+    if (strcmp(e, "0") == 0) return 0;
+    if (strcmp(e, "far") == 0) return 1;
+    if (strcmp(e, "mid") == 0) return 2;
+    return -1;
+}
+
 static int potrf_impl(oisat_ctx* h, float* S, int64_t m, int64_t ld, int* info_host, const int32_t* first, const int32_t* env_dev,
                       const double* fwd_d = nullptr, int* schedule_out = nullptr, const int32_t* far = nullptr, const int32_t* mid = nullptr) {
     ARG_CHECK(h && S && m > 0);
     h->factor.fwd_d = nullptr;
+    h->shadow_last = nullptr;
     if (schedule_out) *schedule_out = OISAT_SCHEDULE_OTHER;
     const int64_t mp = cdiv(m, NB) * NB;
     ARG_CHECK(ld >= mp && (ld % 4) == 0 && ((uintptr_t)S % 16) == 0);
@@ -1981,6 +1991,21 @@
         }
         hit->stamp = ++h->dag_clock;
         DagPlan& pl = *(DagPlan*)hit->plan;
+        char* shadow = nullptr;
+        int shadow_use = 0;
+        if (first && (far || mid)) {
+            const int mode = factor_shadow_mode();
+            ARG_CHECK(mode >= 0 && "OISAT_FACTOR_SHADOW is 0, 1, far or mid");
+            bool any = false;
+            for (int64_t b = 0; b < mpb; ++b) any = any || pl.mid[b] > pl.first[b];
+            const size_t bytes = (size_t)pl.sh_tiles * (size_t)kShTile;
+            if (mode > 0 && any && (h->shadow_cap < 0 || bytes <= (size_t)h->shadow_cap)) {
+                shadow = (char*)oisat_ws(h, 10, bytes);
+                if (!shadow) (void)hipGetLastError();
+                shadow_use = shadow ? mode : 0;
+            }
+        }
+        HIP_TRY(dag_plan_shadow(pl, shadow, shadow_use, h->stream));
         if (ride) {
             double* w = (double*)oisat_ws(h, 5, sizeof(double) * (2 + 8) * mp);
             SolveState* st = solve_state(h);
@@ -2003,6 +2028,11 @@
             rc = dag_launch(h, pl, info_dev, (unsigned*)(info_dev + kInfoDagTimeouts));
         }
         if (schedule_out) *schedule_out = !first ? OISAT_SCHEDULE_OTHER : ride ? OISAT_SCHEDULE_ENV_DAG_FWD : OISAT_SCHEDULE_ENV_DAG;
+        if (rc == OISAT_OK && shadow) {
+            h->shadow_last = shadow;
+            h->shadow_first = pl.first;
+            h->shadow_shrow = pl.shrow;
+        }
     } else {
         rc = lookahead ? potrf_lookahead(h, S, ld, mpb, tinv, info_dev, pw) : potrf_rec(h, S, ld, mpb, 0, mpb, tinv, info_dev);
     }
@@ -2220,6 +2250,34 @@
     for (int64_t i = 0; i < nb; ++i)
         if (mid[i] < (far.empty() ? first[i] : far[i]) || mid[i] > i) return false;
     return true;
+}
+
+extern "C" int oisat_factor_shadow_layout(int nb, const int32_t* first, int64_t* rowoff_out, int64_t* ntiles_out) {
+    ARG_CHECK(nb >= 1 && nb <= kDagEnvMaxBlocks && first && rowoff_out && ntiles_out);
+    ARG_CHECK(envelope_table_ok(first, nb));
+    *ntiles_out = dag_shadow_layout(first, nb, rowoff_out);
+    return OISAT_OK;
+}
+
+extern "C" int oisat_set_factor_shadow_cap(oisat_ctx* h, int64_t bytes) {
+    ARG_CHECK(h != nullptr && bytes >= -1);
+    h->shadow_cap = bytes;
+    return OISAT_OK;
+}
+
+extern "C" int oisat_factor_shadow_tile(oisat_ctx* h, int r, int k, uint16_t* hi_out, uint16_t* lo_out) {
+    ARG_CHECK(h != nullptr && hi_out && lo_out);
+    ARG_CHECK(h->shadow_last != nullptr && "the last factorization on this handle filled a shadow");
+    ARG_CHECK(r >= 1 && r < (int)h->shadow_first.size() && k >= h->shadow_first[r] && k < r);
+    std::vector<uint16_t> raw((size_t)kShTile / 2);
+    HIP_TRY(hipMemcpyAsync(raw.data(), h->shadow_last + (h->shadow_shrow[r] + k) * kShTile, (size_t)kShTile, hipMemcpyDeviceToHost, h->stream));
+    HIP_TRY(hipStreamSynchronize(h->stream));
+    for (int plane = 0; plane < 2; ++plane)
+        for (int half = 0; half < 2; ++half)
+            for (int row = 0; row < NB; ++row)
+                memcpy((plane ? lo_out : hi_out) + row * NB + half * 64, raw.data() + (plane * kShPlane + half * kShHalf + row * 128) / 2,
+                       128);
+    return OISAT_OK;
 }
 
 extern "C" int oisat_dag_task_order_env(int nb, const int32_t* first, const int32_t* far, int32_t* tasks_out, int64_t capacity,
diff --git a/oi-sat-gmi_amd/csrc/dense_dag.inc b/oi-sat-gmi_amd/csrc/dense_dag.inc
--- a/oi-sat-gmi_amd/csrc/dense_dag.inc
+++ b/oi-sat-gmi_amd/csrc/dense_dag.inc
@@ -18,6 +18,9 @@
     int nb;
     int which;
     const int* mid;
+    char* shadow;
+    const int64_t* shrow;
+    int shuse;
 };
 
 struct DagCtl {
@@ -232,6 +235,123 @@
 #undef DAG_CHUNK
 }
 
+constexpr int64_t kShTile = 65536;
+constexpr int kShPlane = 32768, kShHalf = 16384;
+__device__ __forceinline__ const char* dag_sh_src_far(const char* tile, const DagLane& L) { return tile + (L.wid * 32 + L.rl) * 128 + 16 * L.lc; }
+__device__ __forceinline__ const char* dag_sh_src_mid(const char* tile, const DagLane& L) {
+    return tile + (L.wid * 32 + L.rl) * 128 + 16 * (L.lc & 3) + (L.lc >> 2) * kShPlane;
+}
+#define DAG_SH_DMA(buf, off)                                                                                       \
+    do {                                                                                                           \
+        _Pragma("unroll") for (int i = 0; i < 4; ++i) {                                                            \
+            __builtin_amdgcn_global_load_lds((gptr_t)(Ad + (off) + 8 * i * 128),                                   \
+                                             (lptr_t)(lds + ((buf) * 2 + 0) * IMG + (L.wid * 32 + 8 * i) * BK), 16, 0, 0); \
+            __builtin_amdgcn_global_load_lds((gptr_t)(Bd + (off) + 8 * i * 128),                                   \
+                                             (lptr_t)(lds + ((buf) * 2 + 1) * IMG + (L.wid * 32 + 8 * i) * BK), 16, 0, 0); \
+        }                                                                                                          \
+    } while (0)
+#define DAG_SH_RD(buf, op, row, q) (*reinterpret_cast<const dag_bf16x8*>(lds + ((buf) * 2 + (op)) * IMG + (row) + 4 * ((q) ^ L.sw)))
+__device__ __forceinline__ void dag_seg_bf16_sh(float* __restrict__ lds, const DagLane& L, const char* Ad, const char* Bd, int nkt,
+                                                f32x16& acc00, f32x16& acc01, f32x16& acc10, f32x16& acc11) {
+    typedef __attribute__((address_space(1))) const void* gptr_t;
+    typedef __attribute__((address_space(3))) void* lptr_t;
+    constexpr int IMG = NB * BK;
+#define DAG_CHUNK(buf, c)                                                                                          \
+    do {                                                                                                           \
+        const dag_bf16x8 a0 = DAG_SH_RD(buf, 0, L.arow, 2 * (c) + L.fh), a1 = DAG_SH_RD(buf, 0, L.arow + 32 * BK, 2 * (c) + L.fh); \
+        const dag_bf16x8 b0 = DAG_SH_RD(buf, 1, L.brow, 2 * (c) + L.fh), b1 = DAG_SH_RD(buf, 1, L.brow + 32 * BK, 2 * (c) + L.fh); \
+        acc00 = __builtin_amdgcn_mfma_f32_32x32x16_bf16(a0, b0, acc00, 0, 0, 0);                                   \
+        acc01 = __builtin_amdgcn_mfma_f32_32x32x16_bf16(a0, b1, acc01, 0, 0, 0);                                   \
+        acc10 = __builtin_amdgcn_mfma_f32_32x32x16_bf16(a1, b0, acc10, 0, 0, 0);                                   \
+        acc11 = __builtin_amdgcn_mfma_f32_32x32x16_bf16(a1, b1, acc11, 0, 0, 0);                                   \
+    } while (0)
+    DAG_SH_DMA(0, 0);
+    asm volatile("s_waitcnt vmcnt(0)" ::: "memory");
+    __syncthreads();
+    for (int kt = 0; kt < nkt; ++kt) {
+        const int cur = kt & 1, nx = kt + 1;
+        if (nx < nkt) DAG_SH_DMA(cur ^ 1, (int64_t)(nx >> 1) * kShTile + (nx & 1) * kShHalf);
+        DAG_CHUNK(cur, 0);
+        DAG_CHUNK(cur, 1);
+        DAG_CHUNK(cur, 2);
+        DAG_CHUNK(cur, 3);
+        asm volatile("s_waitcnt vmcnt(0)" ::: "memory");
+        __syncthreads();
+    }
+#undef DAG_CHUNK
+}
+__device__ __forceinline__ void dag_seg_bf16x2_sh(float* __restrict__ lds, const DagLane& L, const char* Ad, const char* Bd, int nkt,
+                                                  f32x16& acc00, f32x16& acc01, f32x16& acc10, f32x16& acc11) {
+    typedef __attribute__((address_space(1))) const void* gptr_t;
+    typedef __attribute__((address_space(3))) void* lptr_t;
+    constexpr int IMG = NB * BK;
+#define DAG_CHUNK(buf, c)                                                                                          \
+    do {                                                                                                           \
+        const dag_bf16x8 a0 = DAG_SH_RD(buf, 0, L.arow, 2 * (c) + L.fh), a1 = DAG_SH_RD(buf, 0, L.arow + 32 * BK, 2 * (c) + L.fh); \
+        const dag_bf16x8 b0 = DAG_SH_RD(buf, 1, L.brow, 2 * (c) + L.fh), b1 = DAG_SH_RD(buf, 1, L.brow + 32 * BK, 2 * (c) + L.fh); \
+        const dag_bf16x8 a0l = DAG_SH_RD(buf, 0, L.arow, 4 + 2 * (c) + L.fh), a1l = DAG_SH_RD(buf, 0, L.arow + 32 * BK, 4 + 2 * (c) + L.fh); \
+        const dag_bf16x8 b0l = DAG_SH_RD(buf, 1, L.brow, 4 + 2 * (c) + L.fh), b1l = DAG_SH_RD(buf, 1, L.brow + 32 * BK, 4 + 2 * (c) + L.fh); \
+        acc00 = __builtin_amdgcn_mfma_f32_32x32x16_bf16(a0l, b0, acc00, 0, 0, 0);                                  \
+        acc01 = __builtin_amdgcn_mfma_f32_32x32x16_bf16(a0l, b1, acc01, 0, 0, 0);                                  \
+        acc10 = __builtin_amdgcn_mfma_f32_32x32x16_bf16(a1l, b0, acc10, 0, 0, 0);                                  \
+        acc11 = __builtin_amdgcn_mfma_f32_32x32x16_bf16(a1l, b1, acc11, 0, 0, 0);                                  \
+        acc00 = __builtin_amdgcn_mfma_f32_32x32x16_bf16(a0, b0l, acc00, 0, 0, 0);                                  \
+        acc01 = __builtin_amdgcn_mfma_f32_32x32x16_bf16(a0, b1l, acc01, 0, 0, 0);                                  \
+        acc10 = __builtin_amdgcn_mfma_f32_32x32x16_bf16(a1, b0l, acc10, 0, 0, 0);                                  \
+        acc11 = __builtin_amdgcn_mfma_f32_32x32x16_bf16(a1, b1l, acc11, 0, 0, 0);                                  \
+        acc00 = __builtin_amdgcn_mfma_f32_32x32x16_bf16(a0, b0, acc00, 0, 0, 0);                                   \
+        acc01 = __builtin_amdgcn_mfma_f32_32x32x16_bf16(a0, b1, acc01, 0, 0, 0);                                   \
+        acc10 = __builtin_amdgcn_mfma_f32_32x32x16_bf16(a1, b0, acc10, 0, 0, 0);                                   \
+        acc11 = __builtin_amdgcn_mfma_f32_32x32x16_bf16(a1, b1, acc11, 0, 0, 0);                                   \
+    } while (0)
+    DAG_SH_DMA(0, 0);
+    asm volatile("s_waitcnt vmcnt(0)" ::: "memory");
+    __syncthreads();
+    for (int kt = 0; kt < nkt; ++kt) {
+        const int cur = kt & 1, nx = kt + 1;
+        if (nx < nkt) DAG_SH_DMA(cur ^ 1, (int64_t)(nx >> 2) * kShTile + ((nx >> 1) & 1) * kShHalf + (nx & 1) * 64);
+        DAG_CHUNK(cur, 0);
+        DAG_CHUNK(cur, 1);
+        asm volatile("s_waitcnt vmcnt(0)" ::: "memory");
+        __syncthreads();
+    }
+#undef DAG_CHUNK
+}
+#undef DAG_SH_DMA
+#undef DAG_SH_RD
+
+__device__ __forceinline__ void dag_shadow_store(float* __restrict__ lds, const DagLane& L, char* tile, const f32x16& acc00, const f32x16& acc01,
+                                                 const f32x16& acc10, const f32x16& acc11) {
+    constexpr int IMG = NB * BK;
+    unsigned short* hi = reinterpret_cast<unsigned short*>(lds + (L.wc * 2) * IMG + L.wr * (IMG / 2));
+    unsigned short* lo = reinterpret_cast<unsigned short*>(lds + (L.wc * 2 + 1) * IMG + L.wr * (IMG / 2));
+#define DAG_SH_PUT(ACC, i, j)                                                                           \
+    _Pragma("unroll") for (int e = 0; e < 16; ++e) {                                                    \
+        const int at = ((i) * 32 + (e & 3) + 8 * (e >> 2) + 4 * L.fh) * 64 + (j) * 32 + L.frow;         \
+        const float a = ACC[e];                                                                         \
+        const unsigned h = dag_pk_bf16(a, a);                                                           \
+        const float rest = a - __builtin_bit_cast(float, h << 16);                                      \
+        hi[at] = (unsigned short)h;                                                                     \
+        lo[at] = (unsigned short)dag_pk_bf16(rest, rest);                                               \
+    }
+    DAG_SH_PUT(acc00, 0, 0)
+    DAG_SH_PUT(acc01, 0, 1)
+    DAG_SH_PUT(acc10, 1, 0)
+    DAG_SH_PUT(acc11, 1, 1)
+#undef DAG_SH_PUT
+    asm volatile("s_waitcnt lgkmcnt(0)" ::: "memory");
+    const __amdgpu_buffer_rsrc_t rs = __builtin_amdgcn_make_buffer_rsrc((void*)tile, (short)0, (int)kShTile, 0x00020000);
+    const int voff = L.wc * kShHalf + L.wr * (kShHalf / 2) + L.lane * 16;
+#pragma unroll
+    for (int n = 0; n < 8; ++n) {
+        const dag_u32x4 vh = *reinterpret_cast<const dag_u32x4*>(reinterpret_cast<const char*>(hi) + n * 1024 + L.lane * 16);
+        const dag_u32x4 vl = *reinterpret_cast<const dag_u32x4*>(reinterpret_cast<const char*>(lo) + n * 1024 + L.lane * 16);
+        __builtin_amdgcn_raw_buffer_store_b128(vh, rs, voff, n * 1024, 16);
+        __builtin_amdgcn_raw_buffer_store_b128(vl, rs, voff, kShPlane + n * 1024, 16);
+    }
+    asm volatile("s_waitcnt lgkmcnt(0)" ::: "memory");
+}
+
 __device__ __forceinline__ void dag_acc_to_image(float* __restrict__ lds, const DagLane& L, const f32x16& acc00, const f32x16& acc01,
                                                  const f32x16& acc10, const f32x16& acc11) {
     constexpr int IMG = NB * BK;
@@ -306,6 +426,12 @@
     const float* Arow = sy.S + (int64_t)i * NB * sy.ld;
     const float* Brow = sy.S + (int64_t)j * NB * sy.ld;
     f32x16 acc00 = {0}, acc01 = {0}, acc10 = {0}, acc11 = {0};
+    const char* shA = nullptr;
+    const char* shB = nullptr;
+    if (FAR && sy.shadow) {
+        shA = sy.shadow + sy.shrow[i] * kShTile;
+        shB = sy.shadow + sy.shrow[j] * kShTile;
+    }
     int kmid = kfar;
     if (FAR && sy.mid) {
         kmid = sy.mid[i];
@@ -328,12 +454,18 @@
         int kav = *s_kav;
         if (FAR && k < kfar) {
             kav = kav < kfar ? kav : kfar;
-            dag_seg_bf16(lds, L, dag_src(Arow + (int64_t)k * NB, sy.ld, L), sy.ld, dag_src(Brow + (int64_t)k * NB, sy.ld, L), sy.ld,
-                         (kav - k) * (NB / BK), acc00, acc01, acc10, acc11);
+            if (shA && (sy.shuse & 1))
+                dag_seg_bf16_sh(lds, L, dag_sh_src_far(shA + k * kShTile, L), dag_sh_src_far(shB + k * kShTile, L), (kav - k) * 2, acc00, acc01, acc10, acc11);
+            else
+                dag_seg_bf16(lds, L, dag_src(Arow + (int64_t)k * NB, sy.ld, L), sy.ld, dag_src(Brow + (int64_t)k * NB, sy.ld, L), sy.ld,
+                             (kav - k) * (NB / BK), acc00, acc01, acc10, acc11);
         } else if (FAR && k < kmid) {
             kav = kav < kmid ? kav : kmid;
-            dag_seg_bf16x2(lds, L, dag_src(Arow + (int64_t)k * NB, sy.ld, L), sy.ld, dag_src(Brow + (int64_t)k * NB, sy.ld, L), sy.ld,
-                           (kav - k) * (NB / BK), acc00, acc01, acc10, acc11);
+            if (shA && (sy.shuse & 2))
+                dag_seg_bf16x2_sh(lds, L, dag_sh_src_mid(shA + k * kShTile, L), dag_sh_src_mid(shB + k * kShTile, L), (kav - k) * 4, acc00, acc01, acc10, acc11);
+            else
+                dag_seg_bf16x2(lds, L, dag_src(Arow + (int64_t)k * NB, sy.ld, L), sy.ld, dag_src(Brow + (int64_t)k * NB, sy.ld, L), sy.ld,
+                               (kav - k) * (NB / BK), acc00, acc01, acc10, acc11);
         } else {
             dag_seg(lds, L, dag_src(Arow + (int64_t)k * NB, sy.ld, L), sy.ld, dag_src(Brow + (int64_t)k * NB, sy.ld, L), sy.ld, (kav - k) * (NB / BK),
                     acc00, acc01, acc10, acc11);
@@ -368,6 +500,7 @@
     dag_seg(lds, L, dag_src(Ct, sy.ld, L), sy.ld, dag_src(sy.tinv + (int64_t)j * NB * NB, NB, L), NB, NB / BK, acc00, acc01, acc10, acc11);
     if (t == 0) dag_drop_l1();
     dag_epilogue<false>(Cq, sy.ld, L, acc00, acc01, acc10, acc11);
+    if (FAR && sy.shadow) dag_shadow_store(lds, L, sy.shadow + (sy.shrow[i] + j) * kShTile, acc00, acc01, acc10, acc11);
     dag_publish(st + DAG_STATE_HDR + i, j + 1);
     return true;
 }
@@ -400,6 +533,7 @@
     dag_publish(sy.state, j + 1);
 }
 
+template <bool SH >
 __device__ __forceinline__ bool dag_chain_panel(const DagSys& sy, int j, DagCtl* ctl, float* lds, const DagLane& L, int* s_flag, long long* ctr) {
     const int t = threadIdx.x;
     int* const st = sy.state;
@@ -409,6 +543,7 @@
     dag_seg(lds, L, dag_src(Pt, sy.ld, L), sy.ld, dag_src(sy.tinv + (int64_t)j * NB * NB, NB, L), NB, NB / BK, acc00, acc01, acc10, acc11);
     if (t == 0) dag_drop_l1();
     dag_epilogue<false>(Pt + (int64_t)(L.wr * 64) * sy.ld + L.wc * 64, sy.ld, L, acc00, acc01, acc10, acc11);
+    if (SH && sy.shadow) dag_shadow_store(lds, L, sy.shadow + (sy.shrow[j + 1] + j) * kShTile, acc00, acc01, acc10, acc11);
     dag_acc_to_image(lds, L, acc00, acc01, acc10, acc11);
     dag_publish(st + DAG_STATE_HDR + j + 1, j + 1);
     if (ctr && t == 0) ctr[8 * j + 3] = wall_clock64();
@@ -427,6 +562,7 @@
     return true;
 }
 
+template <bool SH>
 __device__ __forceinline__ bool dag_chain_task(const DagSys& sy, DagCtl* ctl, int* info, float* lds, const DagLane& L, int* s_flag,
                                                long long* ctr , const struct DagSolve* sv) {
     const int t = threadIdx.x;
@@ -440,7 +576,7 @@
         if (t == 0 && j >= 1) ok = dag_wait_ge(sy.state + DAG_STATE_HDR + 2 * sy.nb + j, 1, ctl, L.spin);
         if (ctr && t == 0) ctr[8 * j + 2] = wall_clock64();
         if (!dag_join(ok, s_flag)) return false;
-        if (!dag_chain_panel(sy, j, ctl, lds, L, s_flag, ctr)) return false;
+        if (!dag_chain_panel<SH>(sy, j, ctl, lds, L, s_flag, ctr)) return false;
     }
     __builtin_amdgcn_s_setprio(0);
     return true;
@@ -889,7 +1025,7 @@
             dag_lane_coords(L, tt);
             if (ready_task) ok = dag_fwd_row_task(sy, task.z, sv, ctl, lds);
             else if ((task.x & 255) == DAG_CHAIN)
-                ok = dag_chain_task(sy, ctl, info, lds, L, &s_flag, trace ? trace + 4 * (int64_t)(ntasks + sv.qcap) + 8 * (int64_t)task.z : nullptr, &sv);
+                ok = dag_chain_task<true>(sy, ctl, info, lds, L, &s_flag, trace ? trace + 4 * (int64_t)(ntasks + sv.qcap) + 8 * (int64_t)task.z : nullptr, &sv);
             else ok = dag_tile_task<true>(sy, task.x & 255, (task.x >> 8) & 1023, task.x >> 18, task.z, task.w, ctl, lds, L, &s_flag, &s_kav, tr);
         } else if (ready_task) {
             const SolveMember mb = sv.mem[task.y];
@@ -899,7 +1035,7 @@
             else if (sv.dtype == OISAT_F32) ok = dag_inc_task<float>(sy, mb, task.z, task.w, sv, ctl, lds);
             else ok = dag_inc_task<double>(sy, mb, task.z, task.w, sv, ctl, lds);
         } else if ((task.x & 255) == DAG_CHAIN) {
-            ok = dag_chain_task(sy, ctl, info, lds, L, &s_flag, trace ? trace + 4 * (int64_t)(ntasks + (SOLVE ? sv.qcap : 0)) + 8 * (int64_t)task.z : nullptr,
+            ok = dag_chain_task<SOLVE != DAG_SOLVE_ALL>(sy, ctl, info, lds, L, &s_flag, trace ? trace + 4 * (int64_t)(ntasks + (SOLVE ? sv.qcap : 0)) + 8 * (int64_t)task.z : nullptr,
                                 SOLVE ? &sv : (const DagSolve*)nullptr);
         } else {
             ok = dag_tile_task<SOLVE != DAG_SOLVE_ALL>(sy, task.x & 255, (task.x >> 8) & 1023, task.x >> 18, task.z, task.w, ctl, lds, L, &s_flag,
@@ -969,6 +1105,9 @@
     std::vector<int> far;
     std::vector<int> mid;
     int* mid_dev = nullptr;
+    std::vector<int64_t> shrow;
+    int64_t* shrow_dev = nullptr;
+    int64_t sh_tiles = 0;
     size_t tasks_cap = 0;
     long long* trace_dev = nullptr;
 };
@@ -981,6 +1120,7 @@
     if (p->ctl_dev) (void)hipFree(p->ctl_dev);
     if (p->queue_dev) (void)hipFree(p->queue_dev);
     if (p->mid_dev) (void)hipFree(p->mid_dev);
+    if (p->shrow_dev) (void)hipFree(p->shrow_dev);
     if (p->trace_dev) (void)hipFree(p->trace_dev);
     delete p;
 }
@@ -1100,6 +1240,34 @@
     return hipMemcpyAsync(p.sys_dev, p.sys_host.data(), sizeof(DagSys), hipMemcpyHostToDevice, stream);
 }
 
+static int64_t dag_shadow_layout(const int* first, int64_t nb, int64_t* rowoff) {
+    int64_t n = 0;
+    for (int64_t r = 0; r < nb; ++r) {
+        rowoff[r] = n;
+        n += r - first[r];
+    }
+    return n;
+}
+
+static hipError_t dag_plan_shrow(DagPlan& p, hipStream_t stream) {
+    const size_t nb = p.first.size();
+    p.shrow.resize(nb);
+    p.sh_tiles = dag_shadow_layout(p.first.data(), (int64_t)nb, p.shrow.data());
+    for (size_t r = 0; r < nb; ++r) p.shrow[r] -= p.first[r];
+    return hipMemcpyAsync(p.shrow_dev, p.shrow.data(), sizeof(int64_t) * nb, hipMemcpyHostToDevice, stream);
+}
+
+static hipError_t dag_plan_shadow(DagPlan& p, char* shadow, int use, hipStream_t stream) {
+    DagSys& sy = p.sys_host[0];
+    const int64_t* want = shadow ? p.shrow_dev : nullptr;
+    if (sy.shadow == shadow && sy.shrow == want && sy.shuse == use) return hipSuccess;
+    if (hipError_t e = hipStreamSynchronize(stream)) return e;
+    sy.shadow = shadow;
+    sy.shrow = want;
+    sy.shuse = use;
+    return hipMemcpyAsync(p.sys_dev, p.sys_host.data(), sizeof(DagSys), hipMemcpyHostToDevice, stream);
+}
+
 DagPlan* dag_plan_create(const std::vector<BatchMat>& table, hipStream_t stream, const DagSolveShape& shape = DagSolveShape(),
                          const int* first = nullptr, const int* far = nullptr, const int* mid = nullptr) {
     DagPlan* p = new DagPlan();
@@ -1148,6 +1316,7 @@
               hipMalloc((void**)&p->state_dev, sizeof(int) * words) == hipSuccess &&
               hipMalloc((void**)&p->ctl_dev, sizeof(DagCtl)) == hipSuccess &&
               (p->first.empty() || hipMalloc((void**)&p->mid_dev, sizeof(int) * p->first.size()) == hipSuccess) &&
+              (p->first.empty() || hipMalloc((void**)&p->shrow_dev, sizeof(int64_t) * p->first.size()) == hipSuccess) &&
               (p->qcap == 0 || (p->qcap < (int64_t)INT32_MAX / 4 && hipMalloc((void**)&p->queue_dev, 16 * (size_t)p->qcap) == hipSuccess));
     if (ok && p->qcap > 0) ok = hipMemsetAsync(p->queue_dev, 0, 16 * (size_t)p->qcap, stream) == hipSuccess;
     if (ok) {
@@ -1157,7 +1326,7 @@
              hipMemcpy(p->tasks_dev, tasks.data(), sizeof(int4) * tasks.size(), hipMemcpyHostToDevice) == hipSuccess &&
              hipMemsetAsync(p->state_dev, 0, sizeof(int) * words, stream) == hipSuccess &&
              hipMemsetAsync(p->ctl_dev, 0, sizeof(DagCtl), stream) == hipSuccess;
-        if (ok && !p->first.empty()) ok = dag_plan_mid(*p, mid, stream) == hipSuccess;
+        if (ok && !p->first.empty()) ok = dag_plan_mid(*p, mid, stream) == hipSuccess && dag_plan_shrow(*p, stream) == hipSuccess;
     }
     if (!ok) {
         dag_plan_free(p);
@@ -1186,6 +1355,7 @@
     if (p.trace_dev) { (void)hipFree(p.trace_dev); p.trace_dev = nullptr; }
     HIP_TRY(hipMemcpyAsync(p.tasks_dev, p.tasks_host.data(), sizeof(int4) * p.tasks_host.size(), hipMemcpyHostToDevice, stream));
     HIP_TRY(dag_plan_mid(p, mid, stream));
+    HIP_TRY(dag_plan_shrow(p, stream));
     return OISAT_OK;
 }
 
diff --git a/oi-sat-gmi_amd/csrc/oisat_common.h b/oi-sat-gmi_amd/csrc/oisat_common.h
--- a/oi-sat-gmi_amd/csrc/oisat_common.h
+++ b/oi-sat-gmi_amd/csrc/oisat_common.h
@@ -110,8 +110,8 @@
     std::vector<ProfRec> recs;
     std::vector<ProfPending> pending;
     std::vector<hipEvent_t> free_events;
-    void* ws[10] = {nullptr, nullptr, nullptr, nullptr, nullptr, nullptr, nullptr, nullptr, nullptr, nullptr};
-    size_t ws_bytes[10] = {0, 0, 0, 0, 0, 0, 0, 0, 0, 0};
+    void* ws[11] = {nullptr, nullptr, nullptr, nullptr, nullptr, nullptr, nullptr, nullptr, nullptr, nullptr, nullptr};
+    size_t ws_bytes[11] = {0, 0, 0, 0, 0, 0, 0, 0, 0, 0, 0};
     double scales_host[OISAT_MAX_SCALES] = {0};
     int scales_n = 0;
     const void* scales_dev = nullptr;
@@ -132,6 +132,10 @@
     int64_t obs_perm_m = 0;
     std::vector<int32_t> factor_far;
     std::vector<int32_t> factor_mid;
+    int64_t shadow_cap = -1;
+    const char* shadow_last = nullptr;
+    std::vector<int32_t> shadow_first;
+    std::vector<int64_t> shadow_shrow;
     int dag_mode = -1;
     DagSingle dag_cache[8];
     uint64_t dag_clock = 0;
diff --git a/oi-sat-gmi_amd/csrc/oisat_core.hip b/oi-sat-gmi_amd/csrc/oisat_core.hip
--- a/oi-sat-gmi_amd/csrc/oisat_core.hip
+++ b/oi-sat-gmi_amd/csrc/oisat_core.hip
@@ -51,8 +51,8 @@
         (void)hipEventDestroy(p.b);
     }
     for (auto ev : h->free_events) (void)hipEventDestroy(ev);
-    for (int i = 0; i < 10; ++i)
-        if (h->ws[i]) (void)hipFree(h->ws[i]);
+    for (void* w : h->ws)
+        if (w) (void)hipFree(w);
     if (h->pinned) (void)hipHostFree(h->pinned);
     if (h->own_stream) (void)hipStreamDestroy(h->own_stream);
     if (h->aux_stream) (void)hipStreamDestroy(h->aux_stream);
diff --git a/oi-sat-gmi_amd/oisatgmi/_hip.py b/oi-sat-gmi_amd/oisatgmi/_hip.py
--- a/oi-sat-gmi_amd/oisatgmi/_hip.py
+++ b/oi-sat-gmi_amd/oisatgmi/_hip.py
@@ -94,6 +94,9 @@
     "oisat_set_factor_far": (C.c_int, [_ptr, _ptr, _i64]),
     "oisat_factor_mid": (C.c_int, [_ptr, _i64, C.c_double, _ptr, _ptr, _ptr]),
     "oisat_set_factor_mid": (C.c_int, [_ptr, _ptr, _i64]),
+    "oisat_factor_shadow_layout": (C.c_int, [C.c_int, _ptr, _ptr, C.POINTER(_i64)]),
+    "oisat_set_factor_shadow_cap": (C.c_int, [_c_ctx, _i64]),
+    "oisat_factor_shadow_tile": (C.c_int, [_c_ctx, C.c_int, C.c_int, _ptr, _ptr]),
     "oisat_set_correlation": (C.c_int, [_c_ctx, C.c_int]),
     "oisat_corr_eval": (C.c_int, [C.c_int, C.c_double, _ptr, _i64, _ptr]),
     "oisat_corr_cut_chord": (C.c_int, [C.c_int, C.c_double, C.c_double, C.POINTER(C.c_double)]),
```

New measurement: 14.79 million grid-cells/s, median of 6. +7.2%, better.
